# iPERDance/iPERCore

Measured on AMD Instinct MI355X. Metric: synthesized frames/sec at 512x512 (run_imitator), higher is better.
Workload: dtype f32; 1 GPU; run_imitator 512x512 single src/ref pair, 300-frame reference clip frame-sharded over 1 GPU(s), AttLWB-SPADE generator fp32 (BASELINE configs[1] at N = 1, configs[2] at N = 8); poses=imitate, image_size=512, frame_batch=300, frame_batch_requested=384, world_size=1, parallelism=frame-shard x1, batches_in_flight=1, weights=random-init (seeded) of the real architecture, 36,276,992 params

## Files before the change

include/lwg_hip.h:

```cpp
#ifndef LWG_HIP_H
#define LWG_HIP_H

#include <stddef.h>
#include <stdint.h>

#ifdef __cplusplus
extern "C" {
#endif

typedef void* lwg_stream_t;

#define LWG_ABI_VERSION 10
int lwg_abi_version(void);

#define LWG_MAX_TAPS 52
enum { LWG_EPI_NONE = 0, LWG_EPI_RESIDUAL = 1, LWG_EPI_SPADE = 2 };
enum { LWG_ACTIVATION_NONE = 0, LWG_ACTIVATION_RELU = 1, LWG_ACTIVATION_TANH = 2, LWG_ACTIVATION_SIGMOID = 3 };
#define LWG_ACTIVATION_RELU_MASK 5
enum { LWG_DT_F32 = 0, LWG_DT_BF16 = 1,
       LWG_DT_F32_Q4 = 2 };

typedef struct LwgConvArgs {
    const float* x0;
    const float* x1;
    int C0, C1;
    int B, H, W;
    int OH, OW;
    int M;
    int stride;
    int ntaps;
    int cshift;
    const float* w;
    int N;
    const float* bias;
    float* y;
    int YH, YW, YC, ycoff;
    int omul, ooy, oox;
    int epi;
    int act;
    const float* res;
    const float* xn;
    const float* mean;
    const float* rstd;
    int xdt;
    int ydt;
    signed char dy[LWG_MAX_TAPS];
    signed char dx[LWG_MAX_TAPS];
} LwgConvArgs;

int lwg_conv2d_nhwc_f32(const LwgConvArgs* args, lwg_stream_t stream);
size_t lwg_conv2d_ws_floats(const LwgConvArgs* args);
int lwg_conv2d_nhwc_f32_ws(const LwgConvArgs* args, float* ws, lwg_stream_t stream);
int lwg_conv_slice_count(const LwgConvArgs* args);

int lwg_conv2d_nhwc_bf16(const LwgConvArgs* args, lwg_stream_t stream);
int lwg_conv2d_winograd_f32(const LwgConvArgs* args, lwg_stream_t stream);
size_t lwg_conv2d_winograd_ws_floats(const LwgConvArgs* args);
int lwg_conv2d_winograd_f32_ws(const LwgConvArgs* args, float* ws, lwg_stream_t stream);
int lwg_conv2d_winograd_plan(const LwgConvArgs* args, int with_ws, long long* blocks, int* slices, int* nbv, int* workgroups);
int lwg_winograd_panel_f32(const float* wpanel, float* upk, int Cin, int N, const int* tap9, lwg_stream_t stream);
typedef struct LwgWinoDesc {
    const float* wpanel;
    float* upk;
    int Cin, N, first_block;
    int tap9[9];
} LwgWinoDesc;
int lwg_winograd_panels_f32(const LwgWinoDesc* descs_dev, int ndesc, int total_blocks, lwg_stream_t stream);
int lwg_conv2d_winograd4_f32(const LwgConvArgs* args, lwg_stream_t stream);
typedef struct LwgConvLists {
    const int* heavy;
    const int* light;
    const int* counts;
    const float* cal;
} LwgConvLists;
int lwg_conv2d_winograd4_list_f32(const LwgConvArgs* args, const LwgConvLists* lists, lwg_stream_t stream);
int lwg_conv2d_winograd4_list_applies(const LwgConvArgs* args);
int lwg_spade_skip_lists_f32(const float* T, int B, int ns, int h, int w, int d, int* marks, int* heavy, int* light, int* counts, lwg_stream_t stream);
int lwg_conv2d_winograd4_fine_f32(const LwgConvArgs* args, const LwgConvLists* lists, lwg_stream_t stream);
int lwg_spade_skip_fine_lists_f32(const float* T, int B, int ns, int h, int w, int d, int* marks, int* heavy, int* light, int* counts, int* fmarks,
                                  int* fheavy, int* flight, int* fcounts, lwg_stream_t stream);
int lwg_winograd4_panel_f32(const float* wpanel, float* upk, int Cin, int N, const int* tap9, lwg_stream_t stream);
int lwg_conv2d_nhwc_bf16_hr(const LwgConvArgs* args, lwg_stream_t stream);
int lwg_conv2d_winograd_bf16(const LwgConvArgs* args, lwg_stream_t stream);
int lwg_conv2d_nhwc_c8_bf16(const LwgConvArgs* args, lwg_stream_t stream);
int lwg_conv_transpose4_nhwc_bf16(const LwgConvArgs* args, lwg_stream_t stream);
int lwg_conv_transpose4_nhwc_f32(const LwgConvArgs* args, lwg_stream_t stream);
int lwg_conv_transpose4_is_one_grid(const LwgConvArgs* args);
int lwg_conv_transpose4_winograd_f32(const LwgConvArgs* args, lwg_stream_t stream);

int lwg_conv_transpose4_winograd24_f32(const LwgConvArgs* args, lwg_stream_t stream);

int lwg_conv2d_nhwc_f32_split(const LwgConvArgs* args, lwg_stream_t stream);

size_t lwg_conv2d_wgrad_ws_floats(int Ktot, int N, int M);
int lwg_conv2d_wgrad_nhwc_f32(const LwgConvArgs* args, const float* dy, float* dw, float* ws, lwg_stream_t stream);
int lwg_conv2d_wgrad_unpacked_f32(const LwgConvArgs* args, const float* dy, float* ws, float* dw, int D0, int D1, int KH, int KW,
                                  int transposed, const int* kidx, int cin, int nout, float* db, lwg_stream_t stream);
int lwg_colsum_nhwc_f32(const float* x, size_t rows, int C, float* out, float* ws, lwg_stream_t stream);
size_t lwg_conv2d_wgrad_winograd_ws_floats(const LwgConvArgs* args);
int lwg_conv2d_wgrad_winograd_f32(const LwgConvArgs* args, const float* dy, float* ws, float* dw, int cin, int nout, lwg_stream_t stream);

int lwg_act_bwd_f32(const float* dy, const float* y, size_t n, int act, float* out, lwg_stream_t stream);
int lwg_norm_fwd_nhwc_f32(const float* x, const float* mean, const float* rstd, const float* gamma, const float* beta, int gstride,
                          int B, int HW, int C, int act, float* y, lwg_stream_t stream);
int lwg_norm_bwd_nhwc_f32(const float* dy, const float* y, const float* x, const float* mean, const float* rstd,
                          const float* gamma, int gstride, int B, int HW, int C, int act, int nsplit, float* dx, float* dgamma,
                          float* dbeta, float* ws, lwg_stream_t stream);
int lwg_adam_step_f32(float* p, const float* g, float* m, float* v, size_t n, float lr, float beta1, float beta2, float eps, int t,
                      lwg_stream_t stream);
int lwg_adam_step_dev_f32(float* p, const float* g, float* m, float* v, size_t n, float lr, float beta1, float beta2, float eps,
                          int* t_dev, lwg_stream_t stream);
int lwg_pack_panel_f32(const float* w, int D0, int D1, int KH, int KW, int transposed, const int* kidx, int ntaps, int cin,
                       int cin_pad, int nout, int n_pad, float* out, lwg_stream_t stream);
int lwg_unpack_wgrad_f32(const float* dwk, int D0, int D1, int KH, int KW, int transposed, const int* kidx, int ntaps, int cin,
                         int cin_pad, int nout, int n_pad, float* dw, lwg_stream_t stream);
typedef struct LwgPackDesc {
    const float* w;
    float* out;
    int D1, KHW, transposed, ntaps, cin, cin_pad, nout, n_pad, Kp, first_block;
    int kidx[LWG_MAX_TAPS];
} LwgPackDesc;
int lwg_pack_panels_f32(const LwgPackDesc* descs_dev, int ndesc, int total_blocks, lwg_stream_t stream);
int lwg_maxpool2_fwd_nhwc_f32(const float* x, float* y, int B, int H, int W, int C, lwg_stream_t stream);
int lwg_maxpool2_bwd_nhwc_f32(const float* x, const float* dy, float* dx, int B, int H, int W, int C, lwg_stream_t stream);
int lwg_crop_resize_bilinear_f32(const float* x, const long long* box, float* y, float* valid, int N, int C, int H, int W, int OH, int OW,
                                 lwg_stream_t stream);
int lwg_crop_resize_bilinear_bwd_f32(const float* dy, const long long* box, float* dx, int N, int C, int H, int W, int OH, int OW, lwg_stream_t stream);
int lwg_prelu_f32(const float* x, const float* slope, const float* res, size_t rows, int C, float* y, lwg_stream_t stream);
int lwg_prelu_bwd_f32(const float* x, const float* slope, const float* dy, size_t rows, int C, float* dx, lwg_stream_t stream);

int lwg_instnorm_stats_nhwc_f32(const float* x, int B, int HW, int C, float eps, float* mean, float* rstd,
                                float* ws, int nsplit, lwg_stream_t stream);
int lwg_instnorm_stats_nhwc_bf16(const void* x, int B, int HW, int C, float eps, float* mean, float* rstd, float* ws, int nsplit,
                                 lwg_stream_t stream);
int lwg_instnorm_apply_nhwc_f32(const float* x, const float* mean, const float* rstd, const float* res,
                                float* y, int B, int HW, int C, int act, lwg_stream_t stream);

int lwg_flow_resize_f32(const float* T, int n, int S, int h, int w, float* out, lwg_stream_t stream);
int lwg_lwb_attention_f32(const float* q, const float* Ks, const float* Vs, const float* bk, const float* bv,
                          const float* T, float* out, int B, int ns, int h, int w, int C, int S,
                          int src_batched, lwg_stream_t stream);
int lwg_lwb_attention_bf16(const void* q, const void* Ks, const void* Vs, const float* bk, const float* bv, const float* T, void* out,
                           int B, int ns, int h, int w, int C, int S, int src_batched, lwg_stream_t stream);
int lwg_lwb_attention_x_records(int h, int w, int C, int element_size);
int lwg_lwb_attention_x_f32(const float* x, const float* Kq, const float* kappa, const float* Vs, const float* bv, const float* T,
                            float* out, float* stats, int B, int ns, int h, int w, int C, int src_batched, lwg_stream_t stream);
int lwg_lwb_attention_x_bf16(const void* x, const void* Kq, const float* kappa, const void* Vs, const float* bv, const float* T,
                             void* out, float* stats, int B, int ns, int h, int w, int C, int src_batched, lwg_stream_t stream);
size_t lwg_instnorm_finalize_ws_floats(int B, int C, int nrec);
int lwg_instnorm_finalize_f32(float* ws, int B, int C, int nrec, float eps, float* mean, float* rstd, lwg_stream_t stream);
int lwg_lwb_attention_bwd_f32(const float* q, const float* Ks, const float* Vs, const float* bk, const float* bv,
                              const float* T, const float* dout, float* dq, float* dKs, float* dVs, int B, int ns,
                              int h, int w, int C, int S, int src_batched, lwg_stream_t stream);
int lwg_lwb_attention_kv_f32(const float* q, const float* kv, const float* bk, const float* bv, const float* T, float* out,
                             int B, int ns, int h, int w, int C, int S, int src_batched, lwg_stream_t stream);
int lwg_lwb_attention_kv_bwd_f32(const float* q, const float* kv, const float* bk, const float* bv, const float* T,
                                 const float* dout, float* dq, float* dkv, int B, int ns, int h, int w, int C, int S,
                                 int src_batched, lwg_stream_t stream);
int lwg_lwb_fuse_f32(const float* tsf_x, const float* src_x, const float* gate, const float* T, float* out, int B, int ns,
                     int h, int w, int C, int S, int src_batched, float scale_w, float scale_o, lwg_stream_t stream);
int lwg_lwb_fuse_bf16(const void* tsf_x, const void* src_x, const void* gate, const float* T, void* out, int B, int ns, int h, int w,
                      int C, int S, int src_batched, float scale_w, float scale_o, lwg_stream_t stream);
int lwg_lwb_fuse_bwd_f32(const float* src_x, const float* gate, const float* T, const float* dout, float* d_tsf, float* d_src,
                         float* d_gate, int B, int ns, int h, int w, int C, int S, int src_batched, float scale_w, float scale_o,
                         lwg_stream_t stream);

size_t lwg_rasterize_ws_bytes(int B, int nf, int S);
int lwg_project_faces_f32(const float* verts, const float* cam, const int32_t* faces, int B, int nv, int nf,
                          float eye_dist, float* faces_v, float* f2pts, lwg_stream_t stream);
int lwg_rasterize_fim_wim_f32(const float* faces_v, int B, int nf, int S, float near, float far, int32_t* fim,
                              float* wim, void* ws, lwg_stream_t stream);
int lwg_texture_sample_f32(const int32_t* fim, const float* wim, const float* faces_v, const float* textures, int B, int nf,
                           int S, int T, int tex_batched, float eps, const float* bg_color3_host, float* rgb, lwg_stream_t stream);

int lwg_flow_compose_f32(const int32_t* fim, const float* wim, int B, int S, const float* map_fn, int nf,
                         const float* f_uvs2img, const float* uv_img4, int Hu, int Wu, const float* src_f2pts,
                         int ns, float* tsf_inputs, float* Tst, float* cond_nchw, float* Tuv, lwg_stream_t stream);
int lwg_bc_transform_f32(const float* f2pts, const int32_t* fim, const float* wim, int B, int S, int nf, float* T,
                         lwg_stream_t stream);
int lwg_encode_fim_f32(const int32_t* fim, const float* map_fn, int B, int S, int nf, int D, float* out,
                       lwg_stream_t stream);

size_t lwg_smpl_lbs_ws_floats(int B, int nv, int nj);
int lwg_smpl_lbs_f32(const float* pose, int pose_stride, const float* beta, int beta_stride, int nbeta,
                     const float* cam, int cam_stride, const float* v_template, const float* offsets, int off_batched,
                     const float* shapedirs, const float* posedirs, const float* J_regressor, const int32_t* parents,
                     const float* lbs_weights, const int32_t* links, int nlinks, int B, int nv, int nj, float* verts,
                     float* j3d, float* j2d, float* ws, lwg_stream_t stream);

int lwg_head_compose_f32(const float* x, const float* wpk, const float* bg, size_t bg_bstride, int B, int S, int C,
                         float* pred, float* mask, float* img, lwg_stream_t stream);
int lwg_head_compose_q4_f32(const float* x, const float* wpk, const float* bg, size_t bg_bstride, int B, int S, int C,
                            float* pred, float* mask, float* img, lwg_stream_t stream);
int lwg_thin_conv_f32(const float* x, const float* wpk, int B, int S, int C, int ks, float* y, lwg_stream_t stream);
int lwg_head_compose_bf16(const void* x, const void* wb, const float* bg, size_t bg_bstride, int B, int S, int C, float* pred,
                          float* mask, float* img, lwg_stream_t stream);
int lwg_up4_head_compose_bf16(const LwgConvArgs* args, const void* whead, const float* bg, size_t bg_bstride, float* pred, float* mask, float* img,
                              lwg_stream_t stream);
int lwg_frames_to_u8(const float* pred, int B, int S, int bgr, uint8_t* out, lwg_stream_t stream);
int lwg_nchw_to_nhwc_f32(const float* src, float* dst, int B, int C, int Cp, int P, lwg_stream_t stream);
int lwg_nhwc_to_nchw_f32(const float* src, float* dst, int B, int C, int Cs, int P, lwg_stream_t stream);

int lwg_morph_f32(const float* in, float* out, int n, int H, int W, int ks, int mode, float* ws, lwg_stream_t stream);
int lwg_canny_f32(const float* sil, int n, int H, int W, const float* gauss9, const float* sobelx9, float low, float high,
                  float* edges, float* ws, lwg_stream_t stream);
int lwg_boundary_fill_f32(const float* src, const float* confidant, const float* outpad, const float* edges, int n, int H,
                          int W, float* out, int32_t* top3, int32_t* ws, lwg_stream_t stream);
int lwg_grid_sample_nchw_f32(const float* img, size_t img_bstride, const float* grid, int n, int C, int H, int W, int Ho,
                             int Wo, float* out, lwg_stream_t stream);
int lwg_uv_merge_f32(const float* src_warp, const float* vis, int ns, int H, int W, float* out, lwg_stream_t stream);
int lwg_uv_merge_parts_f32(const float* uv_imgs, const float* vis, int n, int H, int W, float* out, lwg_stream_t stream);
int lwg_pack_inputs_f32(const float* a, int Ca, const float* b, int Cb, const float* mask, int n, int H, int W, int Cp,
                        float* out, lwg_stream_t stream);

int lwg_device_cu_count(void);

#ifdef __cplusplus
}
#endif
#endif
```

ipercore_amd/_lib.py:

```python
import ctypes
import os
import re

_HERE = os.path.dirname(os.path.abspath(__file__))
LIB_PATH = os.path.join(_HERE, "liblwg_hip.so")
HEADER_PATH = os.path.join(os.path.dirname(_HERE), "include", "lwg_hip.h")

LWG_MAX_TAPS = 52
EPI_NONE, EPI_RESIDUAL, EPI_SPADE = 0, 1, 2
ACT_NONE, ACT_RELU, ACT_TANH, ACT_SIGMOID, ACT_LRELU = 0, 1, 2, 3, 4
ACT_RELU_MASK = 5
DT_F32, DT_BF16, DT_F32_Q4 = 0, 1, 2

c_f = ctypes.c_void_p
c_i = ctypes.c_int


class LwgConvArgs(ctypes.Structure):
    _fields_ = [
        ("x0", c_f), ("x1", c_f),
        ("C0", c_i), ("C1", c_i),
        ("B", c_i), ("H", c_i), ("W", c_i),
        ("OH", c_i), ("OW", c_i),
        ("M", c_i), ("stride", c_i), ("ntaps", c_i), ("cshift", c_i),
        ("w", c_f), ("N", c_i), ("bias", c_f),
        ("y", c_f), ("YH", c_i), ("YW", c_i), ("YC", c_i), ("ycoff", c_i),
        ("omul", c_i), ("ooy", c_i), ("oox", c_i),
        ("epi", c_i), ("act", c_i),
        ("res", c_f), ("xn", c_f), ("mean", c_f), ("rstd", c_f),
        ("xdt", c_i), ("ydt", c_i),
        ("dy", ctypes.c_byte * LWG_MAX_TAPS), ("dx", ctypes.c_byte * LWG_MAX_TAPS),
    ]


class LwgWinoDesc(ctypes.Structure):
    _fields_ = [("wpanel", ctypes.c_void_p), ("upk", ctypes.c_void_p), ("Cin", c_i), ("N", c_i), ("first_block", c_i), ("tap9", c_i * 9)]


class LwgConvLists(ctypes.Structure):
    _fields_ = [("heavy", c_f), ("light", c_f), ("counts", c_f), ("cal", c_f)]


class LwgPackDesc(ctypes.Structure):
    _fields_ = [("w", c_f), ("out", c_f)] + [(n, c_i) for n in ("D1", "KHW", "transposed", "ntaps", "cin", "cin_pad", "nout", "n_pad", "Kp",
                                                               "first_block")] + [("kidx", c_i * LWG_MAX_TAPS)]


_SIGS = {
    "lwg_abi_version": (c_i, []),
    "lwg_device_cu_count": (c_i, []),
    "lwg_conv2d_nhwc_f32": (c_i, [ctypes.POINTER(LwgConvArgs), c_f]),
    "lwg_conv2d_ws_floats": (ctypes.c_size_t, [ctypes.POINTER(LwgConvArgs)]),
    "lwg_conv2d_nhwc_f32_ws": (c_i, [ctypes.POINTER(LwgConvArgs), c_f, c_f]),
    "lwg_conv2d_nhwc_bf16": (c_i, [ctypes.POINTER(LwgConvArgs), c_f]),
    "lwg_conv2d_winograd_f32": (c_i, [ctypes.POINTER(LwgConvArgs), c_f]),
    "lwg_conv2d_winograd_ws_floats": (ctypes.c_size_t, [ctypes.POINTER(LwgConvArgs)]),
    "lwg_conv2d_winograd_f32_ws": (c_i, [ctypes.POINTER(LwgConvArgs), c_f, c_f]),
    "lwg_conv2d_winograd_plan": (c_i, [ctypes.POINTER(LwgConvArgs), c_i, ctypes.POINTER(ctypes.c_longlong), ctypes.POINTER(c_i), ctypes.POINTER(c_i),
                                       ctypes.POINTER(c_i)]),
    "lwg_winograd_panel_f32": (c_i, [c_f, c_f, c_i, c_i, ctypes.POINTER(c_i), c_f]),
    "lwg_winograd_panels_f32": (c_i, [c_f, c_i, c_i, c_f]),
    "lwg_conv2d_winograd4_f32": (c_i, [ctypes.POINTER(LwgConvArgs), c_f]),
    "lwg_conv2d_winograd4_list_f32": (c_i, [ctypes.POINTER(LwgConvArgs), ctypes.POINTER(LwgConvLists), c_f]),
    "lwg_conv2d_winograd4_list_applies": (c_i, [ctypes.POINTER(LwgConvArgs)]),
    "lwg_spade_skip_lists_f32": (c_i, [c_f, c_i, c_i, c_i, c_i, c_i, c_f, c_f, c_f, c_f, c_f]),
    "lwg_conv2d_winograd4_fine_f32": (c_i, [ctypes.POINTER(LwgConvArgs), ctypes.POINTER(LwgConvLists), c_f]),
    "lwg_spade_skip_fine_lists_f32": (c_i, [c_f, c_i, c_i, c_i, c_i, c_i, c_f, c_f, c_f, c_f, c_f, c_f, c_f, c_f, c_f]),
    "lwg_winograd4_panel_f32": (c_i, [c_f, c_f, c_i, c_i, ctypes.POINTER(c_i), c_f]),
    "lwg_conv2d_nhwc_bf16_hr": (c_i, [ctypes.POINTER(LwgConvArgs), c_f]),
    "lwg_conv2d_winograd_bf16": (c_i, [ctypes.POINTER(LwgConvArgs), c_f]),
    "lwg_conv2d_nhwc_c8_bf16": (c_i, [ctypes.POINTER(LwgConvArgs), c_f]),
    "lwg_conv_transpose4_nhwc_bf16": (c_i, [ctypes.POINTER(LwgConvArgs), c_f]),
    "lwg_conv_transpose4_nhwc_f32": (c_i, [ctypes.POINTER(LwgConvArgs), c_f]),
    "lwg_conv_transpose4_winograd_f32": (c_i, [ctypes.POINTER(LwgConvArgs), c_f]),
    "lwg_conv_transpose4_winograd24_f32": (c_i, [ctypes.POINTER(LwgConvArgs), c_f]),
    "lwg_conv_transpose4_is_one_grid": (c_i, [ctypes.POINTER(LwgConvArgs)]),
    "lwg_conv_slice_count": (c_i, [ctypes.POINTER(LwgConvArgs)]),
    "lwg_conv2d_nhwc_f32_split": (c_i, [ctypes.POINTER(LwgConvArgs), c_f]),
    "lwg_conv2d_wgrad_ws_floats": (ctypes.c_size_t, [c_i, c_i, c_i]),
    "lwg_conv2d_wgrad_nhwc_f32": (c_i, [ctypes.POINTER(LwgConvArgs), c_f, c_f, c_f, c_f]),
    "lwg_conv2d_wgrad_unpacked_f32": (c_i, [ctypes.POINTER(LwgConvArgs), c_f, c_f, c_f] + [c_i] * 5 + [ctypes.POINTER(ctypes.c_int), c_i, c_i, c_f, c_f]),
    "lwg_colsum_nhwc_f32": (c_i, [c_f, ctypes.c_size_t, c_i, c_f, c_f, c_f]),
    "lwg_conv2d_wgrad_winograd_ws_floats": (ctypes.c_size_t, [ctypes.POINTER(LwgConvArgs)]),
    "lwg_conv2d_wgrad_winograd_f32": (c_i, [ctypes.POINTER(LwgConvArgs), c_f, c_f, c_f, c_i, c_i, c_f]),
    "lwg_act_bwd_f32": (c_i, [c_f, c_f, ctypes.c_size_t, c_i, c_f, c_f]),
    "lwg_norm_fwd_nhwc_f32": (c_i, [c_f, c_f, c_f, c_f, c_f, c_i, c_i, c_i, c_i, c_i, c_f, c_f]),
    "lwg_norm_bwd_nhwc_f32": (c_i, [c_f, c_f, c_f, c_f, c_f, c_f, c_i, c_i, c_i, c_i, c_i, c_i, c_f, c_f, c_f, c_f, c_f]),
    "lwg_adam_step_f32": (c_i, [c_f, c_f, c_f, c_f, ctypes.c_size_t, ctypes.c_float, ctypes.c_float, ctypes.c_float, ctypes.c_float, c_i, c_f]),
    "lwg_adam_step_dev_f32": (c_i, [c_f, c_f, c_f, c_f, ctypes.c_size_t, ctypes.c_float, ctypes.c_float, ctypes.c_float, ctypes.c_float, c_f, c_f]),
    "lwg_pack_panel_f32": (c_i, [c_f] + [c_i] * 5 + [ctypes.POINTER(ctypes.c_int)] + [c_i] * 5 + [c_f, c_f]),
    "lwg_pack_panels_f32": (c_i, [c_f, c_i, c_i, c_f]),
    "lwg_unpack_wgrad_f32": (c_i, [c_f] + [c_i] * 5 + [ctypes.POINTER(ctypes.c_int)] + [c_i] * 5 + [c_f, c_f]),
    "lwg_maxpool2_fwd_nhwc_f32": (c_i, [c_f, c_f, c_i, c_i, c_i, c_i, c_f]),
    "lwg_maxpool2_bwd_nhwc_f32": (c_i, [c_f, c_f, c_f, c_i, c_i, c_i, c_i, c_f]),
    "lwg_crop_resize_bilinear_f32": (c_i, [c_f, c_f, c_f, c_f, c_i, c_i, c_i, c_i, c_i, c_i, c_f]),
    "lwg_crop_resize_bilinear_bwd_f32": (c_i, [c_f, c_f, c_f, c_i, c_i, c_i, c_i, c_i, c_i, c_f]),
    "lwg_prelu_f32": (c_i, [c_f, c_f, c_f, ctypes.c_size_t, c_i, c_f, c_f]),
    "lwg_prelu_bwd_f32": (c_i, [c_f, c_f, c_f, ctypes.c_size_t, c_i, c_f, c_f]),
    "lwg_instnorm_stats_nhwc_f32": (c_i, [c_f, c_i, c_i, c_i, ctypes.c_float, c_f, c_f, c_f, c_i, c_f]),
    "lwg_instnorm_apply_nhwc_f32": (c_i, [c_f, c_f, c_f, c_f, c_f, c_i, c_i, c_i, c_i, c_f]),
    "lwg_lwb_attention_f32": (c_i, [c_f, c_f, c_f, c_f, c_f, c_f, c_f, c_i, c_i, c_i, c_i, c_i, c_i, c_i, c_f]),
    "lwg_lwb_attention_bf16": (c_i, [c_f, c_f, c_f, c_f, c_f, c_f, c_f, c_i, c_i, c_i, c_i, c_i, c_i, c_i, c_f]),
    "lwg_instnorm_stats_nhwc_bf16": (c_i, [c_f, c_i, c_i, c_i, ctypes.c_float, c_f, c_f, c_f, c_i, c_f]),
    "lwg_head_compose_bf16": (c_i, [c_f, c_f, c_f, ctypes.c_size_t, c_i, c_i, c_i, c_f, c_f, c_f, c_f]),
    "lwg_up4_head_compose_bf16": (c_i, [ctypes.POINTER(LwgConvArgs), c_f, c_f, ctypes.c_size_t, c_f, c_f, c_f, c_f]),
    "lwg_flow_resize_f32": (c_i, [c_f, c_i, c_i, c_i, c_i, c_f, c_f]),
    "lwg_lwb_fuse_f32": (c_i, [c_f] * 5 + [c_i] * 7 + [ctypes.c_float, ctypes.c_float, c_f]),
    "lwg_lwb_fuse_bf16": (c_i, [c_f] * 5 + [c_i] * 7 + [ctypes.c_float, ctypes.c_float, c_f]),
    "lwg_lwb_fuse_bwd_f32": (c_i, [c_f] * 7 + [c_i] * 7 + [ctypes.c_float, ctypes.c_float, c_f]),
    "lwg_lwb_attention_x_f32": (c_i, [c_f] * 8 + [c_i] * 6 + [c_f]),
    "lwg_lwb_attention_x_bf16": (c_i, [c_f] * 8 + [c_i] * 6 + [c_f]),
    "lwg_lwb_attention_x_records": (c_i, [c_i, c_i, c_i, c_i]),
    "lwg_instnorm_finalize_ws_floats": (ctypes.c_size_t, [c_i, c_i, c_i]),
    "lwg_instnorm_finalize_f32": (c_i, [c_f, c_i, c_i, c_i, ctypes.c_float, c_f, c_f, c_f]),
    "lwg_lwb_attention_bwd_f32": (c_i, [c_f] * 10 + [c_i] * 7 + [c_f]),
    "lwg_lwb_attention_kv_f32": (c_i, [c_f] * 6 + [c_i] * 7 + [c_f]),
    "lwg_lwb_attention_kv_bwd_f32": (c_i, [c_f] * 8 + [c_i] * 7 + [c_f]),
    "lwg_rasterize_ws_bytes": (ctypes.c_size_t, [c_i, c_i, c_i]),
    "lwg_project_faces_f32": (c_i, [c_f, c_f, c_f, c_i, c_i, c_i, ctypes.c_float, c_f, c_f, c_f]),
    "lwg_rasterize_fim_wim_f32": (c_i, [c_f, c_i, c_i, c_i, ctypes.c_float, ctypes.c_float, c_f, c_f, c_f, c_f]),
    "lwg_texture_sample_f32": (c_i, [c_f, c_f, c_f, c_f, c_i, c_i, c_i, c_i, c_i, ctypes.c_float, ctypes.POINTER(ctypes.c_float), c_f, c_f]),
    "lwg_flow_compose_f32": (c_i, [c_f, c_f, c_i, c_i, c_f, c_i, c_f, c_f, c_i, c_i, c_f, c_i, c_f, c_f, c_f, c_f, c_f]),
    "lwg_bc_transform_f32": (c_i, [c_f, c_f, c_f, c_i, c_i, c_i, c_f, c_f]),
    "lwg_encode_fim_f32": (c_i, [c_f, c_f, c_i, c_i, c_i, c_i, c_f, c_f]),
    "lwg_smpl_lbs_ws_floats": (ctypes.c_size_t, [c_i, c_i, c_i]),
    "lwg_smpl_lbs_f32": (c_i, [c_f, c_i, c_f, c_i, c_i, c_f, c_i, c_f, c_f, c_i, c_f, c_f, c_f, c_f, c_f, c_f, c_i, c_i, c_i,
                               c_i, c_f, c_f, c_f, c_f, c_f]),
    "lwg_head_compose_f32": (c_i, [c_f, c_f, c_f, ctypes.c_size_t, c_i, c_i, c_i, c_f, c_f, c_f, c_f]),
    "lwg_head_compose_q4_f32": (c_i, [c_f, c_f, c_f, ctypes.c_size_t, c_i, c_i, c_i, c_f, c_f, c_f, c_f]),
    "lwg_thin_conv_f32": (c_i, [c_f, c_f, c_i, c_i, c_i, c_i, c_f, c_f]),
    "lwg_nchw_to_nhwc_f32": (c_i, [c_f, c_f, c_i, c_i, c_i, c_i, c_f]),
    "lwg_nhwc_to_nchw_f32": (c_i, [c_f, c_f, c_i, c_i, c_i, c_i, c_f]),
    "lwg_frames_to_u8": (c_i, [c_f, c_i, c_i, c_i, c_f, c_f]),
    "lwg_morph_f32": (c_i, [c_f, c_f, c_i, c_i, c_i, c_i, c_i, c_f, c_f]),
    "lwg_canny_f32": (c_i, [c_f, c_i, c_i, c_i, ctypes.POINTER(ctypes.c_float), ctypes.POINTER(ctypes.c_float),
                            ctypes.c_float, ctypes.c_float, c_f, c_f, c_f]),
    "lwg_boundary_fill_f32": (c_i, [c_f, c_f, c_f, c_f, c_i, c_i, c_i, c_f, c_f, c_f, c_f]),
    "lwg_grid_sample_nchw_f32": (c_i, [c_f, ctypes.c_size_t, c_f, c_i, c_i, c_i, c_i, c_i, c_i, c_f, c_f]),
    "lwg_uv_merge_f32": (c_i, [c_f, c_f, c_i, c_i, c_i, c_f, c_f]),
    "lwg_uv_merge_parts_f32": (c_i, [c_f, c_f, c_i, c_i, c_i, c_f, c_f]),
    "lwg_pack_inputs_f32": (c_i, [c_f, c_i, c_f, c_i, c_f, c_i, c_i, c_i, c_i, c_f, c_f]),
}

_lib = None


def header_symbols():
    with open(HEADER_PATH) as fp:
        src = re.sub(r"/\*.*?\*/", "", fp.read(), flags=re.S)
    return sorted(set(re.findall(r"\b(lwg_[a-z0-9_]+)\s*\(", src)))


def lib():
    global _lib
    if _lib is None:
        if not os.path.exists(LIB_PATH):
            raise RuntimeError(
                f"{LIB_PATH} not found: the HIP kernels are not built (run `python -c 'import __graft_entry__ as g; "
                "g.build()'` or `make -C ipercore_amd/csrc`).  There is no CPU fallback.")
        import torch
        handle = ctypes.CDLL(LIB_PATH)
        for name, (res, args) in _SIGS.items():
            fn = getattr(handle, name)
            fn.restype = res
            fn.argtypes = args
        if handle.lwg_abi_version() != 10:
            raise RuntimeError("liblwg_hip.so ABI version mismatch")
        _lib = handle
    return _lib


def check(err, what):
    if err != 0:
        raise RuntimeError(f"{what} failed with hipError_t {err}")
```

ipercore_amd/csrc/lwb_attn_x.hip:

```cpp
#include "lwg_common.h"
#include "lwg_conv_args.h"
#include "lwg_lwb_taps.h"

typedef unsigned int uintx4 __attribute__((ext_vector_type(4)));

template <typename ST> struct AttnXTraits;
template <> struct AttnXTraits<float> {
    static constexpr int CPL = 4;
    __device__ static __forceinline__ void unpack(const uintx4 v, float (&f)[4]) {
#pragma unroll
        for (int k = 0; k < 4; ++k) {
            const unsigned u = v[k];
            f[k] = __builtin_bit_cast(float, u);
        }
    }
    __device__ static __forceinline__ uintx4 pack(const float (&f)[4]) {
        uintx4 v;
#pragma unroll
        for (int k = 0; k < 4; ++k) v[k] = __builtin_bit_cast(unsigned, f[k]);
        return v;
    }
};
template <> struct AttnXTraits<__bf16> {
    static constexpr int CPL = 8;
    __device__ static __forceinline__ void unpack(const uintx4 v, float (&f)[8]) {
#pragma unroll
        for (int k = 0; k < 4; ++k) {
            f[2 * k] = __builtin_bit_cast(float, v[k] << 16);
            f[2 * k + 1] = __builtin_bit_cast(float, v[k] & 0xffff0000u);
        }
    }
    __device__ static __forceinline__ uintx4 pack(const float (&f)[8]) {
        typedef __bf16 bf16x2 __attribute__((ext_vector_type(2)));
        uintx4 v;
#pragma unroll
        for (int k = 0; k < 4; ++k) {
            bf16x2 p;
            p[0] = (__bf16)f[2 * k];
            p[1] = (__bf16)f[2 * k + 1];
            v[k] = __builtin_bit_cast(unsigned, p);
        }
        return v;
    }
};

template <typename ST, int LPP, bool STATS, int NSU, int PW, int OCC, bool PIPE = false>
__global__ __launch_bounds__(256 * PW, PW == 1 ? OCC : 1) void lwg_lwb_attnx_kernel(const ST* __restrict__ x, const ST* __restrict__ Kq,
                                                                 const float* __restrict__ kappa, const ST* __restrict__ Vs,
                                                                 const float* __restrict__ bv, const float* __restrict__ T,
                                                                 ST* __restrict__ out, float* __restrict__ stats, int B, int ns, int h, int w,
                                                                 int src_batched) {
    using TR = AttnXTraits<ST>;
    constexpr int CPL = TR::CPL;
    constexpr int C = CPL * LPP;
    constexpr int PPW = 64 / LPP;
    constexpr int PPP = 4 * PPW;
    constexpr int NPASS = 64 / PPP;
    constexpr int NIT = NPASS / PW;
    static_assert(NPASS % PW == 0, "PW must divide the tile's pass count");
    constexpr int NT = NSU > 0 ? NSU : 1;
    constexpr unsigned ROWB = (unsigned)C * sizeof(ST);
    const int lane = threadIdx.x & 63, wid = threadIdx.x >> 6;
    const int wq = wid & 3, pl = wid >> 2;
    const int cl = lane % LPP, pg = lane / LPP;
    const int tiles_x = (w + 7) >> 3;
    int tile, b;
    if (LWG_ATTNX_INTERLEAVE) {
        const int xcd = blockIdx.x & 7;
        const long idx = blockIdx.x >> 3;
        const long grp = idx / B;
        tile = (int)(grp * 8 + xcd);
        b = (int)(idx - grp * B);
        if (tile >= tiles_x * ((h + 7) >> 3)) return;
    } else {
        const long L = lwg_xcd_remap(blockIdx.x, gridDim.x);
        tile = (int)(L / B);
        b = (int)(L - (long)tile * B);
    }
    const int ty = tile / tiles_x, tx = tile - ty * tiles_x;
    const int hw = h * w;
    const unsigned nsrc = (unsigned)(src_batched ? B * ns : ns);
    __amdgpu_buffer_rsrc_t rK = __builtin_amdgcn_make_buffer_rsrc(const_cast<ST*>(Kq), 0, (int)(nsrc * (unsigned)hw * ROWB), 0x00020000);
    __amdgpu_buffer_rsrc_t rV = __builtin_amdgcn_make_buffer_rsrc(const_cast<ST*>(Vs), 0, (int)(nsrc * (unsigned)hw * ROWB), 0x00020000);
    __amdgpu_buffer_rsrc_t rA = __builtin_amdgcn_make_buffer_rsrc(const_cast<float*>(kappa), 0, (int)(nsrc * (unsigned)hw * 4u), 0x00020000);
    const float inv_sqrt_c = 1.0f / sqrtf((float)C);
    constexpr bool BV_REG = CPL == 4 || LWG_ATTNX_BVREG16;
    float bvr[CPL];
    if (BV_REG) {
#pragma unroll
        for (int k = 0; k < CPL; ++k) bvr[k] = bv[CPL * cl + k];
    }
    const float2* Tb = reinterpret_cast<const float2*>(T) + (size_t)b * ns * hw;

    auto pixel_of = [&](int pass, int& yc, int& xc) -> bool {
        const int p = pass * PPP + wq * PPW + pg;
        const int y = ty * 8 + (p >> 3), xx = tx * 8 + (p & 7);
        const bool live = y < h && xx < w;
        yc = live ? y : ty * 8;
        xc = live ? xx : tx * 8;
        return live;
    };
    extern __shared__ __attribute__((aligned(16))) char smem_ax[];
    char* xs = smem_ax;
    float2* Tl = reinterpret_cast<float2*>(smem_ax + NPASS * 4096);
    {
        __amdgpu_buffer_rsrc_t rX = __builtin_amdgcn_make_buffer_rsrc(const_cast<ST*>(x) + (size_t)b * hw * C, 0, (int)((unsigned)hw * ROWB), 0x00020000);
#pragma unroll
        for (int it = 0; it < NIT; ++it) {
            const int pass = it * PW + pl;
            int yc, xc;
            pixel_of(pass, yc, xc);
            const unsigned voff = (unsigned)(yc * w + xc) * ROWB + (unsigned)(CPL * cl) * (unsigned)sizeof(ST);
            __builtin_amdgcn_raw_ptr_buffer_load_lds(rX, (__attribute__((address_space(3))) void*)(xs + (pass * 4 + wq) * 1024), 16, (int)voff, 0, 0, 0);
        }
        for (int i = threadIdx.x; i < ns * 64; i += 256 * PW) {
            const int s = i >> 6, p = i & 63;
            const int y = ty * 8 + (p >> 3), xx = tx * 8 + (p & 7);
            const bool in = y < h && xx < w;
            Tl[i] = Tb[(size_t)s * hw + (size_t)(in ? y : ty * 8) * w + (in ? xx : tx * 8)];
        }
        asm volatile("s_waitcnt vmcnt(0)" ::: "memory");
        __syncthreads();
    }
    auto x_row = [&](int pass) -> uintx4 { return *reinterpret_cast<const uintx4*>(xs + ((pass * 4 + wq) * 64 + lane) * 16); };

    float shift[CPL], s1[CPL], s2[CPL];
    if (STATS) {
        TR::unpack(*reinterpret_cast<const uintx4*>(xs + cl * 16), shift);
#pragma unroll
        for (int k = 0; k < CPL; ++k) s1[k] = s2[k] = 0.f;
    }
    int nlive = 0;
    auto stats_add = [&](const float (&xv)[CPL]) {
        ++nlive;
        if (PW == 1) {
#pragma unroll
            for (int k = 0; k < CPL; ++k) {
                const float d = xv[k] - shift[k];
                s1[k] += d;
                s2[k] = __builtin_fmaf(d, d, s2[k]);
            }
        }
    };
    auto taps_of = [&](const float2 t, float (&wt)[4], int& tx0, int& ty0) { lwb_taps_of(t, w, h, wt, tx0, ty0); };
    auto fold = [&](const float (&ka)[CPL], const float (&va)[CPL], float kap, const float (&xv)[CPL], float& mrun, float& lrun, float (&o)[CPL]) {
        float dot = 0.f;
#pragma unroll
        for (int k = 0; k < CPL; ++k) dot = __builtin_fmaf(ka[k], xv[k], dot);
#pragma unroll
        for (int off = LPP >> 1; off > 0; off >>= 1) dot += __shfl_xor(dot, off, 64);
        const float logit = (dot + kap) * inv_sqrt_c;
        const float mnew = fmaxf(mrun, logit);
        const float corr = expf(mrun - mnew);
        const float pr = expf(logit - mnew);
        lrun = __builtin_fmaf(lrun, corr, pr);
#pragma unroll
        for (int k = 0; k < CPL; ++k) o[k] = __builtin_fmaf(o[k], corr, pr * va[k]);
        mrun = mnew;
    };
    auto finish = [&](long gp, float lrun, const float (&o)[CPL]) {
        const float invl = 1.f / lrun;
        float r[CPL];
        if (!BV_REG) {
#pragma unroll
            for (int k = 0; k < CPL; k += 4) {
                const floatx4 b4 = *reinterpret_cast<const floatx4*>(bv + CPL * cl + k);
#pragma unroll
                for (int j = 0; j < 4; ++j) bvr[k + j] = b4[j];
            }
        }
#pragma unroll
        for (int k = 0; k < CPL; ++k) r[k] = __builtin_fmaf(o[k], invl, bvr[k]);
        *reinterpret_cast<uintx4*>(out + gp * C + CPL * cl) = TR::pack(r);
    };

    if constexpr (PIPE) {
        static_assert(NSU == 2 && PW == 1 && (NIT % 2) == 0, "the pipelined form is the ns = 2 frame-batch form");
        bool mine = false;
#pragma unroll 1
        for (int it = 0; it < NIT; ++it) {
            int yc, xc;
            const bool live = pixel_of(it, yc, xc);
            const int ptile = it * PPP + wq * PPW + pg;
#pragma unroll
            for (int s = 0; s < 2; ++s) {
                const float2 t = Tl[s * 64 + ptile];
                float wt[4];
                int tx0, ty0;
                taps_of(t, wt, tx0, ty0);
                mine |= live && lwb_tap_in_image(tx0, ty0, w, h);
            }
        }
        if (__syncthreads_or(mine ? 1 : 0) == 0) {
#pragma unroll 1
            for (int it = 0; it < NIT; ++it) {
                int yc, xc;
                const bool live = pixel_of(it, yc, xc);
                float xv[CPL];
                TR::unpack(x_row(it), xv);
                if (live) {
                    if (STATS) stats_add(xv);
                    float o[CPL];
#pragma unroll
                    for (int k = 0; k < CPL; ++k) o[k] = 0.f;
                    finish(((long)b * h + yc) * w + xc, 2.f, o);
                }
            }
        } else {
            struct Taps { uintx4 kr[2][4], vr[2][4]; float ar[2][4], wt[2][4]; };
            auto issue = [&](int pass, Taps& g) {
                int yc, xc;
                const bool live = pixel_of(pass, yc, xc);
                const int ptile = pass * PPP + wq * PPW + pg;
#pragma unroll
                for (int s = 0; s < 2; ++s) {
                    int tx0, ty0;
                    taps_of(Tl[s * 64 + ptile], g.wt[s], tx0, ty0);
                    const unsigned pbase = (unsigned)(src_batched ? b * ns + s : s) * (unsigned)hw;
#pragma unroll
                    for (int tp = 0; tp < 4; ++tp) {
                        const int tyy = ty0 + (tp >> 1), txx = tx0 + (tp & 1);
                        const bool ok = live && tyy >= 0 && tyy < h && txx >= 0 && txx < w;
                        const unsigned pix = pbase + (unsigned)(tyy * w + txx);
                        const unsigned voff = ok ? pix * ROWB + (unsigned)(CPL * cl) * (unsigned)sizeof(ST) : 0xC0000000u;
                        g.kr[s][tp] = __builtin_bit_cast(uintx4, __builtin_amdgcn_raw_buffer_load_b128(rK, (int)voff, 0, 0));
                        g.vr[s][tp] = __builtin_bit_cast(uintx4, __builtin_amdgcn_raw_buffer_load_b128(rV, (int)voff, 0, 0));
                        g.ar[s][tp] = __builtin_bit_cast(float, __builtin_amdgcn_raw_buffer_load_b32(rA, ok ? (int)(pix * 4u) : (int)0xC0000000u, 0, 0));
                    }
                }
            };
            auto consume = [&](int pass, const Taps& g) {
                int yc, xc;
                const bool live = pixel_of(pass, yc, xc);
                float xv[CPL];
                TR::unpack(x_row(pass), xv);
                if (STATS && live) stats_add(xv);
                float mrun = -INFINITY, lrun = 0.f;
                float o[CPL];
#pragma unroll
                for (int k = 0; k < CPL; ++k) o[k] = 0.f;
#pragma unroll
                for (int s = 0; s < 2; ++s) {
                    float ka[CPL], va[CPL], kap = 0.f;
#pragma unroll
                    for (int k = 0; k < CPL; ++k) ka[k] = va[k] = 0.f;
#pragma unroll
                    for (int tp = 0; tp < 4; ++tp) {
                        float k8[CPL], v8[CPL];
                        TR::unpack(g.kr[s][tp], k8);
                        TR::unpack(g.vr[s][tp], v8);
#pragma unroll
                        for (int k = 0; k < CPL; ++k) {
                            ka[k] = __builtin_fmaf(k8[k], g.wt[s][tp], ka[k]);
                            va[k] = __builtin_fmaf(v8[k], g.wt[s][tp], va[k]);
                        }
                        kap = __builtin_fmaf(g.ar[s][tp], g.wt[s][tp], kap);
                    }
                    fold(ka, va, kap, xv, mrun, lrun, o);
                }
                if (live) finish(((long)b * h + yc) * w + xc, lrun, o);
            };
            Taps g0, g1;
            issue(0, g0);
#pragma unroll 1
            for (int it = 0; it < NIT; it += 2) {
                issue(it + 1, g1);
                consume(it, g0);
                issue(it + 2 < NIT ? it + 2 : it + 1, g0);
                consume(it + 1, g1);
            }
        }
    } else {
#pragma unroll 1
    for (int it = 0; it < NIT; ++it) {
        const int pass = it * PW + pl;
        int yc, xc;
        const bool live = pixel_of(pass, yc, xc);
        const long gp = ((long)b * h + yc) * w + xc;
        const int ptile = pass * PPP + wq * PPW + pg;
        float xv[CPL];
        TR::unpack(x_row(pass), xv);
        if (STATS && live) stats_add(xv);
        float mrun = -INFINITY, lrun = 0.f;
        float o[CPL];
#pragma unroll
        for (int k = 0; k < CPL; ++k) o[k] = 0.f;

        auto source = [&](int s, const float2 t) {
            float wt[4];
            int tx0, ty0;
            taps_of(t, wt, tx0, ty0);
            const bool any_tap = live && lwb_tap_in_image(tx0, ty0, w, h);
            float ka[CPL], va[CPL], kap = 0.f;
#pragma unroll
            for (int k = 0; k < CPL; ++k) ka[k] = va[k] = 0.f;
            if (__builtin_amdgcn_ballot_w64(any_tap) != 0ull) {
                const unsigned sidx = (unsigned)(src_batched ? b * ns + s : s);
                const unsigned pbase = sidx * (unsigned)hw;
                uintx4 kr[4], vr[4];
                float ar[4];
#pragma unroll
                for (int tp = 0; tp < 4; ++tp) {
                    const int tyy = ty0 + (tp >> 1), txx = tx0 + (tp & 1);
                    const bool ok = live && tyy >= 0 && tyy < h && txx >= 0 && txx < w;
                    const unsigned pix = pbase + (unsigned)(tyy * w + txx);
                    const unsigned voff = ok ? pix * ROWB + (unsigned)(CPL * cl) * (unsigned)sizeof(ST) : 0xC0000000u;
                    kr[tp] = __builtin_bit_cast(uintx4, __builtin_amdgcn_raw_buffer_load_b128(rK, (int)voff, 0, 0));
                    vr[tp] = __builtin_bit_cast(uintx4, __builtin_amdgcn_raw_buffer_load_b128(rV, (int)voff, 0, 0));
                    ar[tp] = __builtin_bit_cast(float, __builtin_amdgcn_raw_buffer_load_b32(rA, ok ? (int)(pix * 4u) : (int)0xC0000000u, 0, 0));
                }
#pragma unroll
                for (int tp = 0; tp < 4; ++tp) {
                    float k8[CPL], v8[CPL];
                    TR::unpack(kr[tp], k8);
                    TR::unpack(vr[tp], v8);
#pragma unroll
                    for (int k = 0; k < CPL; ++k) {
                        ka[k] = __builtin_fmaf(k8[k], wt[tp], ka[k]);
                        va[k] = __builtin_fmaf(v8[k], wt[tp], va[k]);
                    }
                    kap = __builtin_fmaf(ar[tp], wt[tp], kap);
                }
            }
            fold(ka, va, kap, xv, mrun, lrun, o);
        };
        if (NSU > 0) {
#pragma unroll
            for (int s = 0; s < NT; ++s) source(s, Tl[s * 64 + ptile]);
        } else {
#pragma unroll 1
            for (int s = 0; s < ns; ++s) source(s, Tl[s * 64 + ptile]);
        }
        if (live) finish(gp, lrun, o);
    }
    }

    if (STATS) {
        if (PW > 1) {
            __shared__ float acc[4][64][2 * CPL];
            if (pl == 0) {
#pragma unroll
                for (int k = 0; k < 2 * CPL; ++k) acc[wq][lane][k] = 0.f;
            }
            __syncthreads();
#pragma unroll 1
            for (int p = 0; p < NPASS; ++p) {
                if (pl == p % PW) {
                    int yc, xc;
                    if (pixel_of(p, yc, xc)) {
                        float xv[CPL];
                        TR::unpack(x_row(p), xv);
#pragma unroll
                        for (int k = 0; k < CPL; ++k) {
                            const float d = xv[k] - shift[k];
                            acc[wq][lane][k] += d;
                            acc[wq][lane][CPL + k] = __builtin_fmaf(d, d, acc[wq][lane][CPL + k]);
                        }
                    }
                }
                __syncthreads();
            }
            if (pl == 0) {
#pragma unroll
                for (int k = 0; k < CPL; ++k) {
                    s1[k] = acc[wq][lane][k];
                    s2[k] = acc[wq][lane][CPL + k];
                }
            }
        }
        __syncthreads();
        float (*sh)[2][C] = reinterpret_cast<float (*)[2][C]>(smem_ax);
        float* shn = reinterpret_cast<float*>(smem_ax + 4 * 2 * C * sizeof(float));
        float fn = (float)nlive;
#pragma unroll
        for (int off = LPP; off < 64; off <<= 1) {
#pragma unroll
            for (int k = 0; k < CPL; ++k) {
                s1[k] += __shfl_xor(s1[k], off, 64);
                s2[k] += __shfl_xor(s2[k], off, 64);
            }
            fn += __shfl_xor(fn, off, 64);
        }
        if (pg == 0) {
            if (pl == 0) {
#pragma unroll
                for (int k = 0; k < CPL; ++k) {
                    sh[wq][0][CPL * cl + k] = s1[k];
                    sh[wq][1][CPL * cl + k] = s2[k];
                }
            }
            if (cl == 0) shn[wid] = fn;
        }
        __syncthreads();
        if (wid == 0 && pg == 0) {
            float tn = 0.f;
#pragma unroll
            for (int k = 0; k < 4 * PW; ++k) tn += shn[k];
            const int nrec = tiles_x * ((h + 7) >> 3);
#pragma unroll
            for (int k = 0; k < CPL; ++k) {
                const int c = CPL * cl + k;
                const float t1 = ((sh[0][0][c] + sh[1][0][c]) + sh[2][0][c]) + sh[3][0][c];
                const float t2 = ((sh[0][1][c] + sh[1][1][c]) + sh[2][1][c]) + sh[3][1][c];
                const float mean = shift[k] + t1 / tn;
                const float m2 = t2 - t1 * t1 / tn;
                float* rec = stats + (((size_t)b * nrec + tile) * C + c) * 3;
                rec[0] = tn;
                rec[1] = mean;
                rec[2] = m2 > 0.f ? m2 : 0.f;
            }
        }
    }
}

extern "C" int lwg_lwb_attention_x_records(int h, int w, int C, int esz) {
    if (h <= 0 || w <= 0 || C <= 0 || (esz != 2 && esz != 4)) return 0;
    const int lpp = C / (16 / esz);
    if (lpp < 8 || lpp > 64 || (lpp & (lpp - 1)) != 0) return 0;
    return ((w + 7) >> 3) * ((h + 7) >> 3);
}

template <typename ST>
static int lwg_attnx_launch(const ST* x, const ST* Kq, const float* kappa, const ST* Vs, const float* bv, const float* T, ST* out, float* stats,
                            int B, int ns, int h, int w, int C, int src_batched, hipStream_t stream) {
    if (!x || !Kq || !kappa || !Vs || !bv || !T || !out || B <= 0 || ns <= 0 || ns > 64 || h <= 0 || w <= 0) return (int)hipErrorInvalidValue;
    const unsigned long long nsrc = (unsigned long long)(src_batched ? B * ns : ns);
    if (nsrc * (unsigned long long)h * w * (unsigned long long)C * sizeof(ST) >= 0xC0000000ull) return (int)hipErrorInvalidValue;
    const long tiles = (long)((w + 7) >> 3) * ((h + 7) >> 3);
    constexpr int CPL = AttnXTraits<ST>::CPL;
    const int npass = (C / CPL) / 4;
    const dim3 grid((unsigned)((LWG_ATTNX_INTERLEAVE ? (tiles + 7) / 8 * 8 : tiles) * B));
    const bool wide = LWG_ATTNX_WIDE && tiles * B < 512 && npass >= 4;
#define LWG_ATTNX_GO(LPP, ST_, NSU, PW)                                                                                              \
    {                                                                                                                                \
             \
        constexpr bool pipe = LWG_ATTNX_PIPE && CPL == 4 && (LPP) == 64 && (NSU) == 2 && (PW) == 1;                                  \
        auto kern = lwg_lwb_attnx_kernel<ST, LPP, ST_, NSU, PW, (pipe ? 2 : CPL == 4 ? LWG_ATTNX_OCC : LWG_ATTNX_OCC16), pipe>;        \
        const size_t lds = (size_t)((LPP) / 4) * 4096 + (size_t)ns * 512;                         \
        static unsigned long long lds_ok = 0;                                                                                        \
        if (lds > 65536) {                                                                                                           \
            const hipError_t e = lwg_allow_dynamic_lds(reinterpret_cast<const void*>(kern), lds, lds_ok);                            \
            if (e != hipSuccess) return (int)e;                                                                                      \
        }                                                                                                                            \
        hipLaunchKernelGGL(kern, grid, dim3(256 * PW), lds, stream, x, Kq, kappa, Vs, bv, T, out, stats, B, ns, h, w, src_batched);   \
    }
#define LWG_ATTNX_PW(LPP, ST_, NSU)                                                                                                  \
    {                                                                                                                                \
        if constexpr ((LPP) / 4 >= 4) {                                                                                              \
            if (wide) LWG_ATTNX_GO(LPP, ST_, NSU, 4) else LWG_ATTNX_GO(LPP, ST_, NSU, 1)                                             \
        } else {                                                                                                                     \
            LWG_ATTNX_GO(LPP, ST_, NSU, 1)                                                                                           \
        }                                                                                                                            \
    }
#define LWG_ATTNX_LAUNCH(LPP)                                                                                                        \
    if (stats) { if (LWG_ATTNX_NSU2 && ns == 2) LWG_ATTNX_PW(LPP, true, 2) else LWG_ATTNX_PW(LPP, true, 0) }                         \
    else { if (LWG_ATTNX_NSU2 && ns == 2) LWG_ATTNX_PW(LPP, false, 2) else LWG_ATTNX_PW(LPP, false, 0) }
    switch (C / CPL) {
        case 8: LWG_ATTNX_LAUNCH(8) break;
        case 16: LWG_ATTNX_LAUNCH(16) break;
        case 32: LWG_ATTNX_LAUNCH(32) break;
        case 64: if constexpr (CPL == 4) { LWG_ATTNX_LAUNCH(64) break; }
                 return (int)hipErrorInvalidValue;
        default: return (int)hipErrorInvalidValue;
    }
#undef LWG_ATTNX_LAUNCH
#undef LWG_ATTNX_PW
#undef LWG_ATTNX_GO
    return (int)hipGetLastError();
}

extern "C" int lwg_lwb_attention_x_f32(const float* x, const float* Kq, const float* kappa, const float* Vs, const float* bv, const float* T,
                                       float* out, float* stats, int B, int ns, int h, int w, int C, int src_batched, lwg_stream_t stream_) {
    if (C != 32 && C != 64 && C != 128 && C != 256) return (int)hipErrorInvalidValue;
    return lwg_attnx_launch<float>(x, Kq, kappa, Vs, bv, T, out, stats, B, ns, h, w, C, src_batched, reinterpret_cast<hipStream_t>(stream_));
}

extern "C" int lwg_lwb_attention_x_bf16(const void* x, const void* Kq, const float* kappa, const void* Vs, const float* bv, const float* T,
                                        void* out, float* stats, int B, int ns, int h, int w, int C, int src_batched, lwg_stream_t stream_) {
    if (C != 64 && C != 128 && C != 256) return (int)hipErrorInvalidValue;
    return lwg_attnx_launch<__bf16>(static_cast<const __bf16*>(x), static_cast<const __bf16*>(Kq), kappa, static_cast<const __bf16*>(Vs), bv, T,
                                    static_cast<__bf16*>(out), stats, B, ns, h, w, C, src_batched, reinterpret_cast<hipStream_t>(stream_));
}

__global__ __launch_bounds__(1024) void lwg_in_stats_merge_seg(const float* __restrict__ ws, int C, int nrec, int nseg, float eps,
                                                              float* __restrict__ part, float* __restrict__ mean, float* __restrict__ rstd) {
    const int lane = threadIdx.x & 63, wid = threadIdx.x >> 6;
    const int c = blockIdx.x * 64 + lane, b = blockIdx.y, seg = blockIdx.z;
    const bool cok = c < C;
    const float* base = ws + ((size_t)b * nrec * C + (cok ? c : 0)) * 3;
    const float r = base[1];
    const int per = (nrec + nseg - 1) / nseg;
    const int r0 = seg * per, r1 = min(nrec, r0 + per);
    float sa = 0.f, ss = 0.f, sq = 0.f;
    if (cok) {
        for (int i = r0 + wid; i < r1; i += 16) {
            const float* o = base + (size_t)i * C * 3;
            const float n = o[0], d = o[1] - r;
            sa += n;
            ss = __builtin_fmaf(n, d, ss);
            sq += __builtin_fmaf(n * d, d, o[2]);
        }
    }
    __shared__ float sh[16][3][64];
    sh[wid][0][lane] = sa;
    sh[wid][1][lane] = ss;
    sh[wid][2][lane] = sq;
    __syncthreads();
    if (wid == 0 && cok) {
        float ta = 0.f, ts = 0.f, tq = 0.f;
#pragma unroll
        for (int k = 0; k < 16; ++k) { ta += sh[k][0][lane]; ts += sh[k][1][lane]; tq += sh[k][2][lane]; }
        if (nseg == 1) {
            const float m2 = tq - ts * ts / ta;
            mean[(size_t)b * C + c] = r + ts / ta;
            rstd[(size_t)b * C + c] = 1.0f / sqrtf((m2 > 0.f ? m2 : 0.f) / ta + eps);
        } else {
            float* o = part + (((size_t)b * nseg + seg) * C + c) * 3;
            o[0] = ta; o[1] = ts; o[2] = tq;
        }
    }
}

__global__ __launch_bounds__(256) void lwg_in_stats_merge_fin(const float* __restrict__ ws, const float* __restrict__ part, int BC, int C, int nrec,
                                                             int nseg, float eps, float* __restrict__ mean, float* __restrict__ rstd) {
    const int i = blockIdx.x * 256 + threadIdx.x;
    if (i >= BC) return;
    const int b = i / C, c = i - b * C;
    const float r = ws[((size_t)b * nrec * C + c) * 3 + 1];
    float ta = 0.f, ts = 0.f, tq = 0.f;
    for (int s = 0; s < nseg; ++s) {
        const float* o = part + (((size_t)b * nseg + s) * C + c) * 3;
        ta += o[0]; ts += o[1]; tq += o[2];
    }
    const float m2 = tq - ts * ts / ta;
    mean[i] = r + ts / ta;
    rstd[i] = 1.0f / sqrtf((m2 > 0.f ? m2 : 0.f) / ta + eps);
}

extern "C" size_t lwg_instnorm_finalize_ws_floats(int B, int C, int nrec) {
    if (B <= 0 || C <= 0 || nrec <= 0) return 0;
    const size_t nseg = nrec > 512 ? (size_t)(nrec + 255) / 256 : 0;
    return (size_t)B * nrec * C * 3 + (size_t)B * nseg * C * 3;
}
extern "C" int lwg_instnorm_finalize_f32(float* ws, int B, int C, int nrec, float eps, float* mean, float* rstd, lwg_stream_t stream_) {
    if (!ws || !mean || !rstd || B <= 0 || C <= 0 || nrec <= 0 || B > 65535) return (int)hipErrorInvalidValue;
    hipStream_t stream = reinterpret_cast<hipStream_t>(stream_);
    const int nseg = nrec > 512 ? (nrec + 255) / 256 : 1;
    if (nseg > 65535) return (int)hipErrorInvalidValue;
    float* part = ws + (size_t)B * nrec * C * 3;
    hipLaunchKernelGGL(lwg_in_stats_merge_seg, dim3((C + 63) / 64, B, nseg), dim3(1024), 0, stream, ws, C, nrec, nseg, eps, part, mean, rstd);
    if (nseg > 1)
        hipLaunchKernelGGL(lwg_in_stats_merge_fin, dim3((B * C + 255) / 256), dim3(256), 0, stream, ws, part, B * C, C, nrec, nseg, eps, mean, rstd);
    return (int)hipGetLastError();
}
```

ipercore_amd/csrc/lwg_conv_wino.h:

```cpp
#pragma once
#include <stddef.h>
#include "lwg_conv_args.h"

#ifdef __HIPCC__
#define CW_FN __host__ __device__ __forceinline__
#else
#define CW_FN static inline
#endif
#ifdef __HIP_DEVICE_COMPILE__
#define CW_UNIFORM(v) __builtin_amdgcn_readfirstlane(v)
#else
#define CW_UNIFORM(v) (v)
#endif
#define CW_OOB 0xC0000000u
#define CW_KS 8
#define CW_NB 64
struct CwGrid { int bx, by, tiles, total; };
CW_FN CwGrid cw_grid(int B, int H, int W, int N, int ex, int ey, int nbv) {
    const int bx = (W + ex - 1) / ex, by = (H + ey - 1) / ey, tiles = bx * by * B;
    return CwGrid{bx, by, tiles, tiles * (N / nbv)};
}
CW_FN long long cw_total_blocks(int B, int H, int W, int N, int ex, int ey, int nbv) {
    return (long long)((W + ex - 1) / ex) * ((H + ey - 1) / ey) * B * (N / nbv);
}

enum { CW_COLMAJOR = 0, CW_CHUNK = 1, CW_XCD = 2 };
struct CwOrder { int kind, nwg, wg, ncb, tiles, total, xg, xr; };

CW_FN int cw4_order_kind(int xcd_sw, int chunk_sw, bool sm, unsigned nwg, int ncb, int Cin, int N, int tiles, int total) {
    const bool xcd = xcd_sw && !sm && (nwg & 7u) == 0 && (ncb == 4 || ncb == 8 || (ncb == 2 && (Cin >= 192 || xcd_sw == 2))) && (int)nwg < total && tiles >= (int)nwg / ncb;
    return xcd ? CW_XCD : chunk_sw == 2 || (chunk_sw == 1 && 144u * (unsigned)Cin * (unsigned)N <= (5u << 20)) ? CW_CHUNK : CW_COLMAJOR;
}
CW_FN CwOrder cw_order(int kind, unsigned nwg, unsigned wg, int ncb, const CwGrid& g) {
    return CwOrder{kind, (int)nwg, (int)wg, ncb, g.tiles, g.total, (int)nwg / ncb, (int)(((wg & 7u) / (unsigned)ncb) * (nwg >> 3) + (wg >> 3))};
}
CW_FN bool cw_has_block(const CwOrder& o, int id) {
    return o.kind == CW_XCD ? (id / o.nwg) * o.xg + o.xr < o.tiles : id < o.total;
}
CW_FN void cw_block(const CwOrder& o, int id, int& cb, int& t) {
    if (o.kind == CW_XCD) {
        cb = (int)((unsigned)o.wg & 7u) & (o.ncb - 1);
        t = CW_UNIFORM((id / o.nwg) * o.xg + o.xr);
    } else if (o.kind == CW_CHUNK) {
        const int G = o.nwg, per = G * o.ncb;
        const int ch = CW_UNIFORM(id / per);
        const int r = id - ch * per, base = ch * G;
        const int nt = o.tiles - base < G ? o.tiles - base : G;
        cb = CW_UNIFORM(r / nt);
        t = CW_UNIFORM(base + r - cb * nt);
    } else {
        cb = CW_UNIFORM(id / o.tiles);
        t = CW_UNIFORM(id - cb * o.tiles);
    }
}
CW_FN int cw_image(const CwGrid& g, int t) { return t / (g.bx * g.by); }
CW_FN void cw_corner(const CwGrid& g, int t_in_image, int ex, int ey, int& x0, int& y0) { x0 = (t_in_image % g.bx) * ex, y0 = (t_in_image / g.bx) * ey; }
CW_FN int cw_n0(int cb, int nbv) { return cb * nbv; }
CW_FN int cw4_n0_spade_small(int cb) { return (cb >> 1) * 64 + (cb & 1) * 16; }
CW_FN int cw_halo_pixel(int i, int hw, int nel, int lgp, int x0, int y0, int H, int W) {
    const int pix = i >> lgp, hy = pix / hw, hx = pix - hy * hw;
    const int gy = y0 - 1 + hy, gx = x0 - 1 + hx;
    return i < nel && gy >= 0 && gy < H && gx >= 0 && gx < W ? gy * W + gx : -1;
}
CW_FN unsigned cw_halo_pixel_voff(int lin, int i, int lgp, int C, int ebytes) {
    return lin >= 0 ? (unsigned)(lin * C + (16 / ebytes) * (i & ((1 << lgp) - 1))) * (unsigned)ebytes : CW_OOB;
}
CW_FN unsigned cw_halo_voff(int i, int hw, int nel, int lgp, int x0, int y0, int H, int W, int C, int ebytes) {
    return cw_halo_pixel_voff(cw_halo_pixel(i, hw, nel, lgp, x0, y0, H, W), i, lgp, C, ebytes);
}
CW_FN bool cw_stage_second(int c, int C0, bool two) { return two && c >= C0; }
CW_FN unsigned cw_stage_soff(int c, int C0, bool two, int ebytes) { return (unsigned)(cw_stage_second(c, C0, two) ? c - C0 : c) * (unsigned)ebytes; }
CW_FN unsigned cw4_out_voff(int ox, int oy, int H, int W, int YC, int chan) {
    return ox < W && oy < H ? (unsigned)((oy * W + ox) * YC + chan) * 4u : CW_OOB;
}
CW_FN unsigned cw4_out_group(unsigned vo, int h, bool grouped) { return vo + (grouped ? 128u * (unsigned)h : 0u); }

struct CwWindow { int x0, y0, x1, y1; };
CW_FN CwWindow cw_block_window(int x0, int y0, int ex, int ey, int d, int H, int W) {
    return CwWindow{x0 - d > 0 ? x0 - d : 0, y0 - d > 0 ? y0 - d : 0, x0 + ex + d < W ? x0 + ex + d : W, y0 + ey + d < H ? y0 + ey + d : H};
}
CW_FN void cw_list_entry(int e, int ncb, int& slot, int& cb) { slot = e / ncb, cb = e - slot * ncb; }
CW_FN int cw_list_first_light(int wg, int nwg, int nhe) { return wg >= nhe ? wg : wg + (nhe - wg + nwg - 1) / nwg * nwg; }
CW_FN void cw4_light_elem(int tid, int it, int nth, int nq, int& px, int& py, int& q4) {
    const int e = it * nth + tid, p = e / nq;
    q4 = e - p * nq, px = p & 31, py = p >> 5;
}

#define CW4F_SX 16
#define CW4F_SY 8
#define CW4F_NSX (32 / CW4F_SX)
#define CW4F_NS (CW4F_NSX * (16 / CW4F_SY))
#define CW4F_HW (CW4F_SX + 2)
#define CW4F_HH (CW4F_SY + 2)
#define CW4F_NEL (CW4F_HW * CW4F_HH * 2)
#define CW4F_ROUNDS ((CW4F_NEL + 63) / 64)
CW_FN int cw4f_slot_of_patch(int pty, int ptx) { return (pty / (CW4F_SY / 4)) * CW4F_NSX + ptx / (CW4F_SX / 4); }
CW_FN void cw4f_patch_in_slot(int pty, int ptx, int& ly, int& lx) { ly = pty % (CW4F_SY / 4), lx = ptx % (CW4F_SX / 4); }
CW_FN void cw4f_corner(const CwGrid& g, int u, int& b, int& x0, int& y0) {
    const int t = u / CW4F_NS, s = u - t * CW4F_NS;
    b = cw_image(g, t);
    cw_corner(g, t - b * g.bx * g.by, 32, 16, x0, y0);
    x0 += (s % CW4F_NSX) * CW4F_SX, y0 += (s / CW4F_NSX) * CW4F_SY;
}
CW_FN bool cw4f_in_image(int x0, int y0, int H, int W) { return x0 < W && y0 < H; }
CW_FN int cw4f_in_image_total(int B, int H, int W) { return B * ((W + CW4F_SX - 1) / CW4F_SX) * ((H + CW4F_SY - 1) / CW4F_SY); }
CW_FN int cw4f_groups(int nh) { return (nh + CW4F_NS - 1) / CW4F_NS; }
CW_FN int cw4f_slot_index(int grp, int k, int nh) { return grp * CW4F_NS + k < nh ? grp * CW4F_NS + k : -1; }
CW_FN unsigned cw4f_reached(int x, int y, int x0, int y0, int d) {
    unsigned m = 0;
    for (int s = 0; s < CW4F_NS; ++s) {
        const int sx = x0 + (s % CW4F_NSX) * CW4F_SX, sy = y0 + (s / CW4F_NSX) * CW4F_SY;
        m |= (x >= sx - d && x < sx + CW4F_SX + d && y >= sy - d && y < sy + CW4F_SY + d ? 1u : 0u) << s;
    }
    return m;
}
CW_FN void cw4f_halo_elem(int i, int& slot, int& j) {
    const int wave = (i >> 6) & 7, k = i >> 9, per = CW4F_ROUNDS / 3, wr = 3 * wave + k;
    slot = wave / per, j = (wr - slot * CW4F_ROUNDS) * 64 + (i & 63);
}
CW_FN void cw4f_halo_place(int j, int& hy, int& hx, int& hq) {
    const int pix = j >> 1;
    hq = j & 1, hy = pix / CW4F_HW, hx = pix - hy * CW4F_HW;
}
CW_FN unsigned cw4f_halo_voff(bool present, int j, int x0, int y0, int H, int W, int C) {
    int hy, hx, hq;
    cw4f_halo_place(j, hy, hx, hq);
    const int gy = y0 - 1 + hy, gx = x0 - 1 + hx;
    return present && j < CW4F_NEL && gy >= 0 && gy < H && gx >= 0 && gx < W ? (unsigned)((gy * W + gx) * C + 4 * hq) * 4u : CW_OOB;
}
CW_FN void cw4f_light_pixel(int& px, int& py) {
    const int p = py * 32 + px;
    py = p / CW4F_SX, px = p - py * CW4F_SX;
}

#define CW_NO_OUT_BUFFER (-1ll)
CW_FN bool cw_contract_ok(const LwgConvArgs& a, unsigned long long pair_bytes, long long out_slack) {
    if (!a.x0 || !a.w || !a.y || a.M <= 0 || a.ntaps != 9 || a.stride != 1 || a.omul != 1 || a.C0 <= 0 || (a.C0 % CW_KS) != 0 || a.C1 < 0 ||
        (a.C1 % CW_KS) != 0 || ((a.C0 + a.C1) % (2 * CW_KS)) != 0 || (a.C1 > 0 && !a.x1) || a.N <= 0 || (a.N % CW_NB) != 0 || a.OH != a.H ||
        a.OW != a.W || a.YH != a.H || a.YW != a.W || a.xdt != LWG_DT_F32 || a.ydt != LWG_DT_F32 || (long long)a.M != (long long)a.B * a.H * a.W ||
        a.ycoff < 0 || (a.ycoff % 4) != 0 || (a.YC % 4) != 0 || (a.act == LWG_ACTIVATION_RELU_MASK && a.epi != LWG_EPI_RESIDUAL))
        return false;
    if (a.epi == LWG_EPI_SPADE) {
        if (!a.xn || !a.mean || !a.rstd || !a.bias || a.YC * 2 != a.N || a.ycoff != 0) return false;
    } else {
        if (a.ycoff + a.N > a.YC) return false;
        if (a.epi != LWG_EPI_NONE && (a.epi != LWG_EPI_RESIDUAL || !a.res)) return false;
    }
    const unsigned long long cmax = (unsigned long long)(a.C0 > a.C1 ? a.C0 : a.C1);
    if ((unsigned long long)a.H * a.W * cmax * 4ull >= (unsigned long long)CW_OOB || pair_bytes * (a.C0 + a.C1) * a.N >= 0xffffffffull) return false;
    if (out_slack >= 0 && (unsigned long long)a.H * a.W * a.YC * 4ull + (unsigned long long)out_slack >= (unsigned long long)CW_OOB) return false;
    return true;
}
CW_FN bool cw_contract_calib_ok(const LwgConvArgs& a) {
    return (unsigned long long)a.H * a.W * (unsigned long long)(a.epi == LWG_EPI_SPADE ? a.N : a.YC) * 4ull + 256ull < (unsigned long long)CW_OOB;
}
CW_FN bool cwb_contract_ok(const LwgConvArgs& a) {
    if (!a.x0 || !a.w || !a.y || a.B <= 0 || a.H <= 0 || a.W <= 0 || a.C0 <= 0 || a.C1 < 0 || a.N <= 0 || a.xdt != LWG_DT_BF16 || a.ydt != LWG_DT_BF16 ||
        a.ntaps != 9 || a.stride != 1 || a.omul != 1 || a.ooy != 0 || a.oox != 0 || a.OH != a.H || a.OW != a.W || a.YH != a.H || a.YW != a.W ||
        (long long)a.M != (long long)a.B * a.H * a.W)
        return false;
    for (int t = 0; t < 9; ++t)
        if (a.dy[t] != t / 3 - 1 || a.dx[t] != t % 3 - 1) return false;
    const int Cin = a.C0 + a.C1;
    if (a.N % 64 != 0 || Cin % 64 != 0 || (a.YC & 7) != 0 || (a.ycoff & 7) != 0 || a.ycoff < 0 || (a.C1 != 0 && (a.C0 % 64 != 0 || !a.x1))) return false;
    if (a.act != LWG_ACTIVATION_NONE && a.act != LWG_ACTIVATION_RELU && a.act != LWG_ACTIVATION_TANH && a.act != LWG_ACTIVATION_SIGMOID) return false;
    if ((unsigned long long)a.H * a.W * (unsigned long long)(a.C0 > a.C1 ? a.C0 : a.C1) * 2ull >= (unsigned long long)CW_OOB ||
        32ull * (unsigned long long)Cin * (unsigned long long)a.N >= (unsigned long long)CW_OOB || cw_total_blocks(a.B, a.H, a.W, a.N, 16, 16, 64) >= 0x7fffffffll)
        return false;
    if (a.epi == LWG_EPI_SPADE) return a.xn && a.mean && a.rstd && a.bias && a.YC * 2 == a.N && a.ycoff == 0;
    return a.ycoff + a.N <= a.YC && (a.epi == LWG_EPI_NONE || (a.epi == LWG_EPI_RESIDUAL && a.res));
}

struct LwgWinoTaps { int t[9]; };
CW_FN bool cw_panel_args_ok(const float* wpanel, const float* upk, int Cin, int N, const int* tap9, LwgWinoTaps& taps) {
    if (!wpanel || !upk || !tap9 || Cin <= 0 || (Cin % 32) != 0 || N <= 0) return false;
    for (int i = 0; i < 9; ++i) {
        if (tap9[i] < 0 || tap9[i] > 8) return false;
        taps.t[i] = tap9[i];
    }
    return true;
}

#ifdef __HIPCC__
#include "lwg_common.h"

template <int V> struct IntC { static constexpr int value = V; };
template <int POLICY = 0>
__device__ __forceinline__ floatx4 cw_buf_load(__amdgpu_buffer_rsrc_t r, unsigned voff, unsigned soff) {
    return __builtin_bit_cast(floatx4, __builtin_amdgcn_raw_buffer_load_b128(r, (int)voff, (int)soff, POLICY));
}
__device__ __forceinline__ __amdgpu_buffer_rsrc_t cw_image_rsrc(const void* x, int b, int H, int W, int C, unsigned ebytes) {
    const unsigned img = (unsigned)(H * W);
    return __builtin_amdgcn_make_buffer_rsrc(const_cast<char*>(static_cast<const char*>(x)) + (size_t)b * img * C * ebytes, 0, (int)(img * (unsigned)C * ebytes), 0x00020000);
}

template <int NQ, bool TWO>
struct CwBlock {
    int b, x0, y0, n0;
    __amdgpu_buffer_rsrc_t rx0, rx1;
    unsigned voff0[NQ], voff1[NQ];

    __device__ __forceinline__ void locate(const LwgConvArgs& a, const CwGrid& g, int t, int ex, int ey, int n) {
        b = __builtin_amdgcn_readfirstlane(cw_image(g, t));
        cw_corner(g, t - b * g.bx * g.by, ex, ey, x0, y0);
        n0 = n;
        rx0 = cw_image_rsrc(a.x0, b, a.H, a.W, a.C0, 4u);
        if constexpr (TWO) rx1 = cw_image_rsrc(a.x1, b, a.H, a.W, a.C1, 4u);
    }
    __device__ __forceinline__ void halo(const LwgConvArgs& a, int tid, int nth, int hw, int nel) {
#pragma unroll
        for (int k = 0; k < NQ; ++k) {
            voff0[k] = cw_halo_voff(tid + nth * k, hw, nel, 1, x0, y0, a.H, a.W, a.C0, 4);
            if constexpr (TWO) voff1[k] = cw_halo_voff(tid + nth * k, hw, nel, 1, x0, y0, a.H, a.W, a.C1, 4);
        }
    }
    template <int POLICY = 0>
    __device__ __forceinline__ floatx4 rld1(const LwgConvArgs& a, int c, int k) const {
        if constexpr (!TWO) {
            return cw_buf_load<POLICY>(rx0, voff0[k], cw_stage_soff(c, a.C0, false, 4));
        } else {
            const bool second = cw_stage_second(c, a.C0, true);
            const __amdgpu_buffer_rsrc_t r = second ? rx1 : rx0;
            const unsigned v = second ? voff1[k] : voff0[k];
            return cw_buf_load<POLICY>(r, v, cw_stage_soff(c, a.C0, true, 4));
        }
    }
};
__device__ __forceinline__ void cw_rst1(float* dst, int plane, floatx4 v) {
#pragma unroll
    for (int k = 0; k < 4; ++k) dst[k * plane] = v[k];
}

template <void (*KERNEL)(const LwgConvArgs)>
static inline int cw_launch(dim3 grid, unsigned threads, size_t lds, hipStream_t stream, const LwgConvArgs& a) {
    static unsigned long long done = 0ull;
    if (hipError_t e = lwg_allow_dynamic_lds(reinterpret_cast<const void*>(KERNEL), lds, done); e != hipSuccess) return (int)e;
    hipLaunchKernelGGL(KERNEL, grid, dim3(threads), lds, stream, a);
    return (int)hipGetLastError();
}
template <void (*KERNEL)(const LwgConvArgs, const LwgConvLists)>
static inline int cw_launch_lists(dim3 grid, unsigned threads, size_t lds, hipStream_t stream, const LwgConvArgs& a, const LwgConvLists& l) {
    static unsigned long long done = 0ull;
    if (hipError_t e = lwg_allow_dynamic_lds(reinterpret_cast<const void*>(KERNEL), lds, done); e != hipSuccess) return (int)e;
    hipLaunchKernelGGL(KERNEL, grid, dim3(threads), lds, stream, a, l);
    return (int)hipGetLastError();
}
static inline dim3 cw_persistent_grid(long long total, int cus) { return dim3((unsigned)(LWG_WINO_PERSIST && total > cus ? cus : total)); }
#endif
```

ipercore_amd/csrc/spade_skip.hip:

```cpp
#include <hip/hip_runtime.h>
#include "lwg_common.h"
#include "lwg_conv_wino.h"
#include "lwg_lwb_taps.h"

#define SK_EX 32
#define SK_EY 16

__global__ __launch_bounds__(256) void lwg_spade_skip_mark_kernel(const float2* __restrict__ T, int B, int ns, int h, int w, int d, int* __restrict__ marks) {
    const CwGrid g = cw_grid(B, h, w, CW_NB, SK_EX, SK_EY, CW_NB);
    const int t = blockIdx.x, b = cw_image(g, t);
    int x0, y0;
    cw_corner(g, t - b * g.bx * g.by, SK_EX, SK_EY, x0, y0);
    const CwWindow win = cw_block_window(x0, y0, SK_EX, SK_EY, d, h, w);
    const int ww = win.x1 - win.x0, n = ww * (win.y1 - win.y0);
    bool mine = false;
    for (int s = 0; s < ns; ++s) {
        const float2* Ts = T + ((size_t)b * ns + s) * h * w;
        for (int i = threadIdx.x; i < n; i += 256) {
            const int yy = i / ww, y = win.y0 + yy, x = win.x0 + (i - yy * ww);
            float wt[4];
            int tx0, ty0;
            lwb_taps_of(Ts[(size_t)y * w + x], w, h, wt, tx0, ty0);
            mine |= lwb_tap_in_image(tx0, ty0, w, h);
        }
    }
    const int any = __syncthreads_or(mine ? 1 : 0);
    if (threadIdx.x == 0) marks[t] = any ? 1 : 0;
}

__global__ __launch_bounds__(1024) void lwg_spade_skip_scan_kernel(const int* __restrict__ marks, int n, int* __restrict__ heavy, int* __restrict__ light,
                                                                   int* __restrict__ counts) {
    __shared__ int part[1024];
    const int tid = threadIdx.x, per = (n + 1023) / 1024;
    const int i0 = tid * per < n ? tid * per : n, i1 = i0 + per < n ? i0 + per : n;
    int c = 0;
    for (int i = i0; i < i1; ++i) c += marks[i] != 0;
    part[tid] = c;
    __syncthreads();
    for (int off = 1; off < 1024; off <<= 1) {
        const int v = tid >= off ? part[tid - off] : 0;
        __syncthreads();
        part[tid] += v;
        __syncthreads();
    }
    int hv = part[tid] - c;
    for (int i = i0; i < i1; ++i) {
        if (marks[i] != 0) heavy[hv++] = i;
        else light[i - hv] = i;
    }
    if (tid == 1023) {
        counts[0] = part[1023];
        counts[1] = n - part[1023];
    }
}

__global__ __launch_bounds__(256) void lwg_spade_skip_mark_fine_kernel(const float2* __restrict__ T, int B, int ns, int h, int w, int d, int* __restrict__ marks,
                                                                       int* __restrict__ fmarks) {
    const CwGrid g = cw_grid(B, h, w, CW_NB, SK_EX, SK_EY, CW_NB);
    const int t = blockIdx.x, b = cw_image(g, t);
    int x0, y0;
    cw_corner(g, t - b * g.bx * g.by, SK_EX, SK_EY, x0, y0);
    const CwWindow win = cw_block_window(x0, y0, SK_EX, SK_EY, d, h, w);
    const int ww = win.x1 - win.x0, n = ww * (win.y1 - win.y0);
    unsigned mine = 0;
    for (int s = 0; s < ns; ++s) {
        const float2* Ts = T + ((size_t)b * ns + s) * h * w;
        for (int i = threadIdx.x; i < n; i += 256) {
            const int yy = i / ww, y = win.y0 + yy, x = win.x0 + (i - yy * ww);
            float wt[4];
            int tx0, ty0;
            lwb_taps_of(Ts[(size_t)y * w + x], w, h, wt, tx0, ty0);
            if (lwb_tap_in_image(tx0, ty0, w, h)) mine |= (1u << CW4F_NS) | cw4f_reached(x, y, x0, y0, d);
        }
    }
    unsigned all = 0;
    for (int s = 0; s <= CW4F_NS; ++s) all |= __syncthreads_or((int)((mine >> s) & 1u)) ? 1u << s : 0u;
    if (threadIdx.x < CW4F_NS) {
        const int s = threadIdx.x;
        const bool in = cw4f_in_image(x0 + (s % CW4F_NSX) * CW4F_SX, y0 + (s / CW4F_NSX) * CW4F_SY, h, w);
        fmarks[CW4F_NS * t + s] = in ? (int)((all >> s) & 1u) : 2;
    } else if (threadIdx.x == CW4F_NS) {
        marks[t] = (int)((all >> CW4F_NS) & 1u);
    }
}

struct SkScanJob { const int* marks; int n; int* heavy; int* light; int* counts; };
template <typename F>
__device__ __forceinline__ void sk_for_marks(const int* __restrict__ marks, int i0, int i1, bool vec, F f) {
    int i = i0;
    if (vec)
        for (; i + 4 <= i1; i += 4) {
            const int4 m = *reinterpret_cast<const int4*>(marks + i);
            f(i, m.x), f(i + 1, m.y), f(i + 2, m.z), f(i + 3, m.w);
        }
    for (; i < i1; ++i) f(i, marks[i]);
}
__global__ __launch_bounds__(1024) void lwg_spade_skip_scan2_kernel(SkScanJob j0, SkScanJob j1) {
    __shared__ int ph[1024], pl[1024];
    const SkScanJob j = blockIdx.x == 0 ? j0 : j1;
    const int tid = threadIdx.x, n = j.n, per = ((n + 1023) / 1024 + 3) & ~3;
    const int i0 = tid * per < n ? tid * per : n, i1 = i0 + per < n ? i0 + per : n;
    const bool vec = (reinterpret_cast<size_t>(j.marks) & 15) == 0;
    int ch = 0, cl = 0;
    sk_for_marks(j.marks, i0, i1, vec, [&](int, int m) { ch += m == 1, cl += m == 0; });
    ph[tid] = ch, pl[tid] = cl;
    __syncthreads();
    for (int off = 1; off < 1024; off <<= 1) {
        const int vh = tid >= off ? ph[tid - off] : 0, vl = tid >= off ? pl[tid - off] : 0;
        __syncthreads();
        ph[tid] += vh, pl[tid] += vl;
        __syncthreads();
    }
    int hv = ph[tid] - ch, lt = pl[tid] - cl;
    sk_for_marks(j.marks, i0, i1, vec, [&](int i, int m) {
        if (m == 1) j.heavy[hv++] = i;
        else if (m == 0) j.light[lt++] = i;
    });
    if (tid == 1023) {
        j.counts[0] = ph[1023];
        j.counts[1] = pl[1023];
    }
}

extern "C" int lwg_spade_skip_fine_lists_f32(const float* T, int B, int ns, int h, int w, int d, int* marks, int* heavy, int* light, int* counts,
                                             int* fmarks, int* fheavy, int* flight, int* fcounts, lwg_stream_t stream_) {
    if (!T || !marks || !heavy || !light || !counts || !fmarks || !fheavy || !flight || !fcounts || B <= 0 || ns <= 0 || h <= 0 || w <= 0 || d < 0 || d > 64)
        return (int)hipErrorInvalidValue;
    const long long tiles = cw_total_blocks(B, h, w, CW_NB, SK_EX, SK_EY, CW_NB);
    if (tiles * CW4F_NS >= (1ll << 30) || (long long)h * w >= (1ll << 30)) return (int)hipErrorInvalidValue;
    hipStream_t stream = reinterpret_cast<hipStream_t>(stream_);
    hipLaunchKernelGGL(lwg_spade_skip_mark_fine_kernel, dim3((unsigned)tiles), dim3(256), 0, stream, reinterpret_cast<const float2*>(T), B, ns, h, w, d, marks, fmarks);
    hipLaunchKernelGGL(lwg_spade_skip_scan2_kernel, dim3(2), dim3(1024), 0, stream, SkScanJob{marks, (int)tiles, heavy, light, counts},
                       SkScanJob{fmarks, (int)tiles * CW4F_NS, fheavy, flight, fcounts});
    return (int)hipGetLastError();
}

extern "C" int lwg_spade_skip_lists_f32(const float* T, int B, int ns, int h, int w, int d, int* marks, int* heavy, int* light, int* counts,
                                        lwg_stream_t stream_) {
    if (!T || !marks || !heavy || !light || !counts || B <= 0 || ns <= 0 || h <= 0 || w <= 0 || d < 0 || d > 64) return (int)hipErrorInvalidValue;
    const long long tiles = cw_total_blocks(B, h, w, CW_NB, SK_EX, SK_EY, CW_NB);
    if (tiles >= (1ll << 30) || (long long)h * w >= (1ll << 30)) return (int)hipErrorInvalidValue;
    hipStream_t stream = reinterpret_cast<hipStream_t>(stream_);
    hipLaunchKernelGGL(lwg_spade_skip_mark_kernel, dim3((unsigned)tiles), dim3(256), 0, stream, reinterpret_cast<const float2*>(T), B, ns, h, w, d, marks);
    hipLaunchKernelGGL(lwg_spade_skip_scan_kernel, dim3(1), dim3(1024), 0, stream, marks, (int)tiles, heavy, light, counts);
    return (int)hipGetLastError();
}
```

ipercore_amd/networks/generator.py:

```python
import math

import torch
import torch.nn as nn

from .. import ops
from . import packing
from .params import generator_param_shapes


class _Node(nn.Module):

    def __init__(self):
        super().__init__()


class ParamTree(nn.Module):
    def __init__(self, shapes):
        super().__init__()
        self._shapes = dict(shapes)
        for name, shape in shapes.items():
            parts = name.split(".")
            node = self
            for p in parts[:-1]:
                if not hasattr(node, p):
                    node.add_module(p, _Node())
                node = getattr(node, p)
            node.register_parameter(parts[-1], nn.Parameter(torch.empty(*shape)))
        self.reset_parameters()

    @torch.no_grad()
    def reset_parameters(self):
        named = dict(self.named_parameters())
        for name, p in named.items():
            if name.endswith(".weight"):
                fan_in = p.shape[1] * p.shape[2] * p.shape[3]
                bound = 1.0 / math.sqrt(fan_in)
                p.uniform_(-bound, bound)
                b = named.get(name[:-len("weight")] + "bias")
                if b is not None:
                    b.uniform_(-bound, bound)


class _Packed:

    def __init__(self, gen):
        sd = {k: v for k, v in gen.named_parameters()}
        dev = next(gen.parameters()).device
        self.device = dev
        self.version = _param_version(gen)
        nf, n_res, n_down = gen.num_filters, gen.n_res_block, len(gen.num_filters)
        P = packing

        def conv(name, stride=1, pad=None, cin_pad=None, n_pad=None):
            return P.spec_to(P.pack_conv(sd[name + ".weight"], sd.get(name + ".bias"), stride, pad, cin_pad, n_pad), dev)

        def convT(name, n_pad=None):
            return [P.spec_to(s, dev) for s in P.pack_conv_transpose(sd[name + ".weight"], sd.get(name + ".bias"), n_pad)]

        def site(p):
            Wq = sd[p + ".fq.weight"].detach()[:, :, 0, 0].double()
            Wk = sd[p + ".fk.weight"].detach()[:, :, 0, 0].double()
            bq = sd[p + ".fq.bias"].detach().double()
            Wkq = (Wq.t() @ Wk).float()[:, :, None, None].contiguous()
            wkap = (Wk.t() @ bq).float()[None, :, None, None].contiguous()
            d = {
                "fkq": P.spec_to(P.pack_conv(Wkq, None, 1, 0), dev),
                "fkap": P.spec_to(P.pack_conv(wkap, None, 1, 0, None, 64), dev),
                "fv": P.spec_to(P.pack_conv(sd[p + ".fv.weight"], None, 1, 0), dev),
                "bv": sd[p + ".fv.bias"].detach().float().contiguous(),
                "shared": conv(p + ".spade.mlp_shared.0"),
                "gb": P.spec_to(P.pack_spade_gamma_beta(sd[p + ".spade.mlp_gamma.weight"], sd[p + ".spade.mlp_gamma.bias"],
                                                        sd[p + ".spade.mlp_beta.weight"], sd[p + ".spade.mlp_beta.bias"]), dev),
            }
            return d

        cin_pad = 8
        self.tsf_enc = [conv(f"tsf_net_enc.layers.{i}.0", stride=2, cin_pad=cin_pad if i == 0 else None) for i in range(n_down)]
        self.src_enc = [conv(f"src_net.encoders.layers.{i}.0", stride=2, cin_pad=cin_pad if i == 0 else None) for i in range(n_down)]
        self.src_res = [(conv(f"src_net.res_blocks.{i}.main.0"), conv(f"src_net.res_blocks.{i}.main.2")) for i in range(n_res)]
        self.src_dec = [convT(f"src_net.decoders.layers.{i}.0") for i in range(n_down)]
        self.src_head = P.pack_head(sd["src_net.img_reg.0.weight"], sd["src_net.att_reg.0.weight"]).to(dev)
        self.res = [(conv(f"res_blocks.{i}.main.0"), conv(f"res_blocks.{i}.main.2")) for i in range(n_res)]
        if gen.lwb_kind == "att":
            pass
        elif gen.lwb_kind in ("sg_add", "sg_avg"):
            site = lambda p: {"g0": conv(p + ".gate_conv.0"), "g2": conv(p + ".gate_conv.2")}
        else:
            site = lambda p: {}
        self.enc_sites = [site(f"enc_attlwbs.{i}") for i in range(n_down)]
        self.res_sites = [site(f"res_attlwbs.{i}") for i in range(n_res)]
        self.upconvs = [convT(f"tsf_net_dec.upconvs.{i}.0") for i in range(n_down)]
        self.skippers = [conv(f"tsf_net_dec.skippers.{i}.0") for i in range(n_down - 1)]
        self.head = P.pack_head(sd["tsf_img_reg.0.weight"], sd["tsf_att_reg.0.weight"]).to(dev)
        self.head16 = P.pack_head_bf16(sd["tsf_img_reg.0.weight"], sd["tsf_att_reg.0.weight"]).to(dev) if nf[0] == 64 else None
        self.bg = pack_bg_layers(sd, gen.bg_filters, n_res, dev) if gen.has_bg else None


def pack_bg_layers(sd, bgf, n_res, dev):
    P = packing

    def conv(name, stride=1, pad=None, cin_pad=None, n_pad=None):
        return P.spec_to(P.pack_conv(sd[name + ".weight"], sd.get(name + ".bias"), stride, pad, cin_pad, n_pad), dev)

    def convT(name, n_pad=None):
        return [P.spec_to(s, dev) for s in P.pack_conv_transpose(sd[name + ".weight"], sd.get(name + ".bias"), n_pad)]
    i = 0
    layers = [("conv", conv(f"bg_net.main.{i}", stride=1, pad=3, cin_pad=4))]
    i += 3
    for d in range(1, len(bgf)):
        layers.append(("conv", conv(f"bg_net.main.{i}", stride=2)))
        i += 3
    for _ in range(n_res):
        layers.append(("res", (conv(f"bg_net.main.{i}.main.0"), conv(f"bg_net.main.{i}.main.3"))))
        i += 1
    for d in range(len(bgf) - 1, 0, -1):
        layers.append(("convT", convT(f"bg_net.main.{i}")))
        i += 3
    layers.append(("out", conv(f"bg_net.main.{i}", stride=1, pad=3, n_pad=64)))
    return layers


def run_bg_layers(layers, bg4):
    scratch = _Scratch()
    x = bg4

    def norm(t, act, res=None):
        B, h, w, C = t.shape
        mean, rstd = t.new_empty(B, C), t.new_empty(B, C)
        nsplit = max(1, min(64, (h * w) // 64))
        ops.instnorm_stats(t, mean, rstd, scratch.get(B * C * nsplit * 3, t.device), eps=1e-5, nsplit=nsplit)
        return ops.instnorm_apply(t, mean, rstd, torch.empty_like(t), act=act, res=res)

    for kind, spec in layers:
        B, H, W, _ = x.shape
        if kind == "conv":
            y = ops.conv2d(x, spec, x.new_empty(B, H // spec.stride, W // spec.stride, spec.N))
            x = norm(y, ops.ACT_RELU)
        elif kind == "res":
            h = norm(ops.conv2d(x, spec[0], torch.empty_like(x)), ops.ACT_RELU)
            x = norm(ops.conv2d(h, spec[1], torch.empty_like(x)), ops.ACT_NONE, res=x)
        elif kind == "convT":
            y = x.new_empty(B, 2 * H, 2 * W, spec[0].N)
            x = norm(ops.conv_transpose2d(x, spec, y, act=ops.ACT_NONE), ops.ACT_RELU)
        else:
            y = ops.conv2d(x, spec, x.new_empty(B, H, W, spec.N), act=ops.ACT_TANH)
            return ops.nhwc_to_nchw(y, channels=3)


def _skip_lists(lists, cal):
    return (lists, cal) if isinstance(lists, ops.SkipLists) else tuple(lists) + (cal,)


def spade_calibration(st, x):
    _, h, w, C = x.shape
    cal = st.setdefault("cal", {})
    if (h, w) not in cal:
        hook, ops.CONV_HOOK = ops.CONV_HOOK, None
        try:
            z = x.new_zeros(1, h, w, C)
            T = x.new_full((1, 1, h, w, 2), -2.0)
            att = ops.lwb_attention_x(z, z, x.new_zeros(1, h, w), z, st["bv"], T, torch.empty_like(z))
            actv = ops.conv2d(att, st["shared"], x.new_empty(1, h, w, st["shared"].N), act=ops.ACT_RELU)
            gb = ops.conv2d(actv, st["gb"], x.new_empty(1, h, w, st["gb"].N))
        finally:
            ops.CONV_HOOK = hook
        cal[(h, w)] = (actv, gb)
    return cal[(h, w)]


def _param_version(gen):
    return tuple((p.data_ptr(), p._version) for p in gen.parameters())


class SourceFeatures:

    def __init__(self, enc, res, kv, ns, batched=False):
        self.enc, self.res, self.kv, self.ns, self.batched = enc, res, kv, ns, batched


class AttentionLWBGenerator(nn.Module):
    has_bg = True
    lwb_kind = "att"

    def __init__(self, cfg, temporal=False):
        super().__init__()
        self._name = _get(cfg, "name", "AttLWB-SPADE")
        tsf = _get(cfg, "TSFNet")
        sid = _get(cfg, "SIDNet")
        self.num_filters = [int(c) for c in _get(tsf, "num_filters")]
        self.n_res_block = int(_get(tsf, "n_res_block"))
        if [int(c) for c in _get(sid, "num_filters")] != self.num_filters or int(_get(sid, "n_res_block")) != self.n_res_block:
            raise ValueError("SIDNet and TSFNet must share num_filters / n_res_block (the LWB sites pair them up)")
        for c in self.num_filters:
            if c not in (64, 128, 256):
                raise ValueError(f"num_filters entries must be in {{64,128,256}} for the HIP kernels, got {c}")
        self.cond_nc = int(_get(tsf, "cond_nc"))
        self.temporal = temporal
        self.bg_filters, bg_cond = None, 4
        if self.has_bg:
            bgc = _get(cfg, "BGNet")
            self.bg_filters = [int(c) for c in _get(bgc, "num_filters")]
            bg_cond = int(_get(bgc, "cond_nc"))
        shapes = generator_param_shapes(self.num_filters, self.n_res_block, self.bg_filters or (), cond_nc=self.cond_nc,
                                        bg_cond_nc=bg_cond, with_bg=self.has_bg,
                                        lwb={"att": "att", "add": "plain", "avg": "plain"}.get(self.lwb_kind, "softgate"))
        tree = ParamTree(shapes)
        for name, child in tree.named_children():
            self.add_module(name, child)
        self._packed = None
        self.conv_precision = "winograd"

    def packed(self):
        if self._packed is None or self._packed.version != _param_version(self):
            self._packed = _Packed(self)
        return self._packed

    def _check(self, *tensors):
        if torch.is_grad_enabled() and any(p.requires_grad for p in self.parameters()) and self.training:
            raise NotImplementedError("these methods are the no_grad inference engine: call under torch.no_grad() / .eval(), or train "
                                      "through ipercore_amd.networks.training.TrainableGenerator (trainers.LWGTrainer; all five LWB generators)")
        for t in tensors:
            if t is not None and not t.is_cuda:
                raise RuntimeError("ipercore_amd generator runs on the MI355X only: got a CPU tensor (no fallback)")

    @staticmethod
    def _check_square(t):
        if t.shape[-1] != t.shape[-2]:
            raise ValueError(f"square images only (got {t.shape[-2]} x {t.shape[-1]}): the reference's image_size is one number and the "
                             "attention blocks' flow fields are resized to square feature maps")

    @torch.no_grad()
    def _encode_sources_impl(self, src8, batched=False, ns=None):
        pk = self.packed()
        x = src8
        adt = self._act_dtype()
        enc, res = [], []
        for i, spec in enumerate(pk.src_enc):
            n, H, W, _ = x.shape
            y = x.new_empty(n, H // 2, W // 2, spec.N, dtype=adt)
            x = ops.conv2d(x, spec, y, act=ops.ACT_RELU)
            enc.append(x)
        for c0, c1 in pk.src_res:
            h = ops.conv2d(x, c0, torch.empty_like(x), act=ops.ACT_RELU)
            x = ops.conv2d(h, c1, torch.empty_like(x), epi=ops.EPI_RESIDUAL, res=x)
            res.append(x)
        return SourceFeatures(enc, res, self._project_sources(pk, enc, res), ns if ns is not None else src8.shape[0], batched)

    def _project_sources(self, pk, enc, res):
        kv = []
        for feats, sites in ((enc, pk.enc_sites), (res, pk.res_sites)):
            for f, st in zip(feats, sites):
                if self.lwb_kind == "att":
                    n, h, w, _ = f.shape
                    with ops.conv_precision("fp32" if self.conv_precision in ("bf16", "bf16_winograd") else self.conv_precision):
                        kap = ops.conv2d(f.float(), st["fkap"], f.new_empty(n, h, w, 64, dtype=torch.float32))[..., 0].contiguous()
                    kv.append((ops.conv2d(f, st["fkq"], torch.empty_like(f)), ops.conv2d(f, st["fv"], torch.empty_like(f)), kap))
                else:
                    kv.append((f, None, None))
        return kv

    def _attlwb(self, st, tsf_x, kv, Tst, batched, scratch):
        B, h, w, C = tsf_x.shape
        if self.lwb_kind != "att":
            ns = Tst.shape[1]
            Tst = scratch.flow(Tst, h, w)
            if self.lwb_kind == "add":
                return ops.lwb_fuse(tsf_x, kv[0], Tst, torch.empty_like(tsf_x), src_batched=batched)
            if self.lwb_kind == "avg":
                return ops.lwb_fuse(tsf_x, kv[0], Tst, torch.empty_like(tsf_x), scale_o=1.0 / (ns + 1), src_batched=batched)
            g = ops.conv2d(tsf_x, st["g0"], torch.empty_like(tsf_x), act=ops.ACT_RELU)
            g = ops.conv2d(g, st["g2"], torch.empty_like(tsf_x), act=ops.ACT_SIGMOID)
            return ops.lwb_fuse(tsf_x, kv[0], Tst, torch.empty_like(tsf_x), gate=g,
                                scale_w=1.0 if self.lwb_kind == "sg_add" else 1.0 / ns, src_batched=batched)
        mean = tsf_x.new_empty(B, C, dtype=torch.float32)
        rstd = tsf_x.new_empty(B, C, dtype=torch.float32)
        nrec = ops.attn_records(h, w, C, tsf_x.dtype)
        ws = scratch.get(ops.instnorm_finalize_ws(B, C, nrec), tsf_x.device)
        flow = scratch.flow(Tst, h, w)
        if tuple(flow.shape[2:4]) != (h, w):
            raise NotImplementedError("the attention block takes flows resized to its feature size: non-square feature maps are not built "
                                      "(image_size is one number throughout the reference)")
        att = ops.lwb_attention_x(tsf_x, kv[0], kv[2], kv[1], st["bv"], flow, torch.empty_like(tsf_x), stats=ws,
                                  src_batched=batched)
        ops.instnorm_finalize(ws, B, C, nrec, mean, rstd, eps=1e-5)
        actv, out = tsf_x.new_empty(B, h, w, st["shared"].N), torch.empty_like(tsf_x)
        l1 = l5 = None
        if ops.conv2d_lists_apply(att, st["shared"], actv, act=ops.ACT_RELU):
            l1 = _skip_lists(scratch.lists(flow, ops.SPADE_SKIP_D[0]), spade_calibration(st, tsf_x)[0])
        if ops.conv2d_lists_apply(actv, st["gb"], out, epi=ops.EPI_SPADE, xn=tsf_x, mean=mean, rstd=rstd):
            l5 = _skip_lists(scratch.lists(flow, ops.SPADE_SKIP_D[1]), spade_calibration(st, tsf_x)[1])
        ops.conv2d(att, st["shared"], actv, act=ops.ACT_RELU, **({} if l1 is None else {"lists": l1}))
        return ops.conv2d(actv, st["gb"], out, epi=ops.EPI_SPADE, xn=tsf_x, mean=mean, rstd=rstd, **({} if l5 is None else {"lists": l5}))

    @staticmethod
    def _upconv(x, specs, act, q4=False):
        B, H, W, _ = x.shape
        if q4:
            return ops.conv_transpose2d(x, specs, x.new_empty(B, specs[0].N // 4, 2 * H, 2 * W, 4), act=act, q4=True)
        y = x.new_empty(B, 2 * H, 2 * W, specs[0].N)
        return ops.conv_transpose2d(x, specs, y, act=act)

    @torch.no_grad()
    def _run_tsf_impl(self, tsf8, feats, Tst, bg=None, want_pred=True, want_mask=True, want_img=False):
        pk = self.packed()
        scratch = _Scratch()
        n_down = len(pk.tsf_enc)
        x = tsf8
        adt = self._act_dtype()
        if feats.kv[0][0].dtype != adt:
            raise RuntimeError(f"source features are {feats.kv[0][0].dtype} but the generator runs in {self.conv_precision} mode: "
                               "rebuild them (Imitator.set_source / forward_src) after changing conv_precision")
        enc = []
        site = 0
        for i, spec in enumerate(pk.tsf_enc):
            B, H, W, _ = x.shape
            x = ops.conv2d(x, spec, x.new_empty(B, H // 2, W // 2, spec.N, dtype=adt), act=ops.ACT_RELU)
            x = self._attlwb(pk.enc_sites[i], x, feats.kv[site], Tst, feats.batched, scratch)
            site += 1
            enc.append(x)
        for i, (c0, c1) in enumerate(pk.res):
            h = ops.conv2d(x, c0, torch.empty_like(x), act=ops.ACT_RELU)
            x = ops.conv2d(h, c1, torch.empty_like(x), epi=ops.EPI_RESIDUAL, res=x)
            x = self._attlwb(pk.res_sites[i], x, feats.kv[site], Tst, feats.batched, scratch)
            site += 1
        q4 = adt == torch.float32 and self.conv_precision in ("fp32", "winograd", "winograd2x2")
        for i in range(n_down):
            if i == n_down - 1 and pk.head16 is not None and ops.up4_head_eligible(x, pk.upconvs[i], ops.ACT_RELU):
                return ops.up4_head_compose_bf16(x, pk.upconvs[i], pk.head16, bg, want_pred=want_pred and bg is not None, want_mask=want_mask,
                                                 want_img=want_img)
            x = self._upconv(x, pk.upconvs[i], ops.ACT_RELU, q4=q4 and i == n_down - 1)
            if i != n_down - 1:
                skip = enc[n_down - 2 - i]
                sp = pk.skippers[i]
                x = ops.conv2d(skip, sp, x.new_empty(x.shape[0], x.shape[1], x.shape[2], sp.N), x1=x, act=ops.ACT_RELU)
        head = pk.head
        if x.dtype == torch.bfloat16:
            if pk.head16 is not None:
                head = pk.head16
            else:
                x = x.float()
        return ops.head_compose(x, head, bg, want_pred=want_pred and bg is not None, want_mask=want_mask, want_img=want_img, q4=q4)

    def _act_dtype(self):
        return torch.bfloat16 if self.conv_precision in ("bf16", "bf16_winograd") else torch.float32

    @torch.no_grad()
    def _run_bg_impl(self, bg4):
        return run_bg_layers(self.packed().bg, bg4)

    @torch.no_grad()
    def _run_src_decode_impl(self, x):
        pk = self.packed()
        for specs in pk.src_dec:
            x = self._upconv(x, specs, ops.ACT_RELU)
        _, mask, img = ops.head_compose(x.float(), pk.src_head, None, want_pred=False, want_mask=True, want_img=True)
        return img, mask

    def encode_sources(self, *a, **k):
        with ops.conv_precision(self.conv_precision):
            return self._encode_sources_impl(*a, **k)

    def run_tsf(self, *a, **k):
        with ops.conv_precision(self.conv_precision):
            return self._run_tsf_impl(*a, **k)

    def run_bg(self, *a, **k):
        with ops.conv_precision("fp32" if self.conv_precision in ("bf16", "bf16_winograd") else self.conv_precision):
            return self._run_bg_impl(*a, **k)

    def run_src_decode(self, *a, **k):
        with ops.conv_precision(self.conv_precision):
            return self._run_src_decode_impl(*a, **k)

    @torch.no_grad()
    def forward_bg(self, bg_inputs):
        if not self.has_bg:
            raise AttributeError("this generator has no background network")
        self._check(bg_inputs)
        bs, ns, c, h, w = bg_inputs.shape
        x = ops.nchw_to_nhwc(bg_inputs.reshape(bs * ns, c, h, w).contiguous().float(), c_pad=4)
        return self.run_bg(x).view(bs, ns, 3, h, w)

    @torch.no_grad()
    def forward_src(self, src_inputs, only_enc=True):
        self._check(src_inputs)
        self._check_square(src_inputs)
        bs, ns, c, h, w = src_inputs.shape
        src8 = ops.nchw_to_nhwc(src_inputs.reshape(bs * ns, c, h, w).contiguous().float(), c_pad=8)
        feats = self.encode_sources(src8, batched=bs > 1, ns=ns)
        enc = _FeatList(ops.nhwc_to_nchw(t.float()) for t in feats.enc)
        res = _FeatList(ops.nhwc_to_nchw(t.float()) for t in feats.res)
        enc.lwg_cache = res.lwg_cache = feats
        if only_enc:
            return enc, res
        img, mask = self.run_src_decode(feats.res[-1])
        return enc, res, img.view(bs, ns, 3, h, w), mask.view(bs, ns, 1, h, w)

    def _features_from_api(self, src_enc_outs, src_res_outs, bs):
        cache = getattr(src_enc_outs, "lwg_cache", None)
        if cache is not None and getattr(src_res_outs, "lwg_cache", None) is cache:
            return cache
        pk = self.packed()
        adt = self._act_dtype()
        enc = [ops.nchw_to_nhwc(t.contiguous().float()).to(adt) for t in src_enc_outs]
        res = [ops.nchw_to_nhwc(t.contiguous().float()).to(adt) for t in src_res_outs]
        n = enc[0].shape[0]
        return SourceFeatures(enc, res, self._project_sources(pk, enc, res), n // bs, batched=bs > 1)

    @torch.no_grad()
    def forward_tsf(self, tsf_inputs, src_enc_outs, src_res_outs, Tst, temp_enc_outs=None, temp_res_outs=None, Ttt=None):
        self._check(tsf_inputs, Tst)
        self._check_square(tsf_inputs)
        bs = tsf_inputs.shape[0]
        feats = self._features_from_api(src_enc_outs, src_res_outs, bs)
        T = Tst.contiguous().float()
        if temp_enc_outs is not None and Ttt is not None and self.lwb_kind == "att":
            if bs != 1:
                raise NotImplementedError("temporal attention runs one clip per process (bs = 1), as Imitator.inference does")
            tfe = self._features_from_api(temp_enc_outs, temp_res_outs, bs)
            feats = SourceFeatures(feats.enc, feats.res, [tuple(torch.cat([a, ta], dim=0) for a, ta in zip(site, tsite))
                                                          for site, tsite in zip(feats.kv, tfe.kv)],
                                   feats.ns + Ttt.shape[1], batched=False)
            T = torch.cat([T, Ttt.contiguous().float()], dim=1).contiguous()
        tsf8 = ops.nchw_to_nhwc(tsf_inputs.contiguous().float(), c_pad=8)
        _, mask, img = self.run_tsf(tsf8, feats, T, bg=None, want_pred=False, want_mask=True, want_img=True)
        return img, mask

    @torch.no_grad()
    def _forward_streams(self, src_inputs, tsf_inputs, Tst, only_tsf):
        bs, nt = Tst.shape[0], Tst.shape[1]
        if only_tsf:
            enc, res = self.forward_src(src_inputs, only_enc=True)
            src_imgs = src_masks = None
        else:
            enc, res, src_imgs, src_masks = self.forward_src(src_inputs, only_enc=False)
        imgs, masks = [], []
        for t in range(nt):
            if t != 0 and self.temporal:
                raise NotImplementedError("multi-step temporal training forward (Ttt inside forward()) is not built; "
                                          "temporal INFERENCE goes through Imitator(temporal=True) / forward_tsf(temp_*)")
            img, mask = self.forward_tsf(tsf_inputs[:, t], enc, res, Tst[:, t].contiguous())
            imgs.append(img)
            masks.append(mask)
        return src_imgs, src_masks, torch.stack(imgs, dim=1), torch.stack(masks, dim=1)

    @torch.no_grad()
    def forward(self, bg_inputs, src_inputs, tsf_inputs, Tst, Ttt=None, only_tsf=True):
        bg_img = self.forward_bg(bg_inputs)
        src_imgs, src_masks, imgs, masks = self._forward_streams(src_inputs, tsf_inputs, Tst, only_tsf)
        if only_tsf:
            return bg_img, imgs, masks
        return bg_img, src_imgs, src_masks, imgs, masks


class AttentionLWBFrontGenerator(AttentionLWBGenerator):
    has_bg = False

    @torch.no_grad()
    def forward(self, src_inputs, tsf_inputs, Tst, Ttt=None, only_tsf=True):
        src_imgs, src_masks, imgs, masks = self._forward_streams(src_inputs, tsf_inputs, Tst, only_tsf)
        if only_tsf:
            return imgs, masks
        return src_imgs, src_masks, imgs, masks


class AddLWBGenerator(AttentionLWBGenerator):
    lwb_kind = "add"


class AvgLWBGenerator(AttentionLWBGenerator):
    lwb_kind = "avg"


class SoftGateAddLWBGenerator(AttentionLWBGenerator):
    lwb_kind = "sg_add"


class SoftGateAvgLWBGenerator(AttentionLWBGenerator):
    lwb_kind = "sg_avg"


class _FeatList(list):
    """A list that can carry the engine's cache as an attribute (plain lists cannot)."""


class _Scratch:
    def __init__(self):
        self.buf = None
        self.flows = {}

    def flow(self, Tst, h, w):
        if Tst.shape[2] == h and Tst.shape[3] == w:
            return Tst
        if h != w:
            return Tst
        key = (h, w, Tst.data_ptr())
        if key not in self.flows:
            self.flows[key] = ops.flow_resize(Tst, h, w)
        return self.flows[key]

    def lists(self, flow, d):
        key = ("lists", flow.shape[2], flow.shape[3], d, flow.data_ptr())
        if key not in self.flows:
            self.flows[key] = ops.spade_skip_lists(flow, d)
        return self.flows[key]

    def get(self, n, device):
        if self.buf is None or self.buf.numel() < n or self.buf.device != device:
            self.buf = torch.empty(max(n, 1 << 16), device=device, dtype=torch.float32)
        return self.buf


def _get(cfg, key, default=None):
    if isinstance(cfg, dict):
        if key in cfg:
            return cfg[key]
    elif hasattr(cfg, key):
        return getattr(cfg, key)
    if default is not None:
        return default
    raise KeyError(key)


class _ConcatPacked:

    def __init__(self, gen):
        sd = {k: v for k, v in gen.named_parameters()}
        dev = next(gen.parameters()).device
        self.version = _param_version(gen)
        P = packing
        nf, n_down = gen.num_filters, len(gen.num_filters)

        def conv(name, stride=1, pad=None, cin_pad=None):
            return P.spec_to(P.pack_conv(sd[name + ".weight"], sd.get(name + ".bias"), stride, pad, cin_pad, None), dev)
        self.enc = [conv(f"tsf_net.encoders.layers.{i}.0", stride=2, cin_pad=gen.cin_pad if i == 0 else None) for i in range(n_down)]
        self.res = [(conv(f"tsf_net.res_blocks.{i}.main.0"), conv(f"tsf_net.res_blocks.{i}.main.2")) for i in range(gen.n_res_block)]
        self.dec = [[P.spec_to(sp, dev) for sp in P.pack_conv_transpose(sd[f"tsf_net.decoders.layers.{i}.0.weight"],
                                                                       sd[f"tsf_net.decoders.layers.{i}.0.bias"], None)] for i in range(n_down)]
        self.head = P.pack_head(sd["tsf_net.img_reg.0.weight"], sd["tsf_net.att_reg.0.weight"]).to(dev)
        self.bg = pack_bg_layers(sd, gen.bg_filters, gen.bg_n_res_block, dev)


class InputConcatGenerator(nn.Module):
    has_bg = True

    def __init__(self, cfg, temporal=False):
        super().__init__()
        self._name = _get(cfg, "name", "InputConcat")
        tsf, bgc = _get(cfg, "TSFNet"), _get(cfg, "BGNet")
        self.num_filters = [int(c) for c in _get(tsf, "num_filters")]
        self.n_res_block = int(_get(tsf, "n_res_block"))
        self.cond_nc = int(_get(tsf, "cond_nc"))
        self.num_source = int(_get(tsf, "num_source", 4)) if self._uses_sources() else None
        self.bg_filters = [int(c) for c in _get(bgc, "num_filters")]
        self.bg_n_res_block = int(_get(bgc, "n_res_block"))
        self.temporal = temporal
        if self.num_filters[0] != 64 or any(c not in (64, 128, 256) for c in self.num_filters):
            raise ValueError(f"num_filters must start with 64 and stay in {{64,128,256}} for the HIP kernels, got {self.num_filters}")
        self.cin_pad = 8 if self.cond_nc <= 8 else (16 if self.cond_nc <= 16 else (self.cond_nc + 31) // 32 * 32)
        from .params import concat_generator_param_shapes
        tree = ParamTree(concat_generator_param_shapes(self.num_filters, self.n_res_block, self.bg_filters, self.cond_nc,
                                                        int(_get(bgc, "cond_nc", 4)), self.bg_n_res_block))
        for name, child in tree.named_children():
            self.add_module(name, child)
        self._packed = None

    def _uses_sources(self):
        return True

    def packed(self):
        if self._packed is None or self._packed.version != _param_version(self):
            self._packed = _ConcatPacked(self)
        return self._packed

    @staticmethod
    def _check(*tensors):
        for t in tensors:
            if t is not None and not t.is_cuda:
                raise RuntimeError("ipercore_amd generator runs on the MI355X only: got a CPU tensor (no fallback)")

    @torch.no_grad()
    def forward_bg(self, bg_inputs):
        self._check(bg_inputs)
        bs, ns, c, h, w = bg_inputs.shape
        x = ops.nchw_to_nhwc(bg_inputs.reshape(bs * ns, c, h, w).contiguous().float(), c_pad=4)
        return run_bg_layers(self.packed().bg, x).view(bs, ns, 3, h, w)

    def forward_src(self, src_inputs, only_enc=True):
        bs, ns, _, h, w = src_inputs.shape
        need = self.num_source
        if ns > need:
            src_inputs = src_inputs[:, 0:need]
        elif ns < need:
            src_inputs = torch.cat([src_inputs, torch.stack([src_inputs[:, s % ns] for s in range(need - ns)], dim=1)], dim=1)
        enc = src_inputs.reshape(bs, -1, h, w)
        return (enc, enc) if only_enc else (enc, enc, None, None)

    @torch.no_grad()
    def _autoencode(self, inputs):
        self._check(inputs)
        pk = self.packed()
        x = ops.nchw_to_nhwc(inputs.contiguous().float(), c_pad=self.cin_pad)
        for spec in pk.enc:
            n, H, W, _ = x.shape
            x = ops.conv2d(x, spec, x.new_empty(n, H // 2, W // 2, spec.N), act=ops.ACT_RELU)
        for c0, c1 in pk.res:
            t = ops.conv2d(x, c0, torch.empty_like(x), act=ops.ACT_RELU)
            x = ops.conv2d(t, c1, torch.empty_like(x), epi=ops.EPI_RESIDUAL, res=x)
        for specs in pk.dec:
            n, H, W, _ = x.shape
            x = ops.conv_transpose2d(x, specs, x.new_empty(n, 2 * H, 2 * W, specs[0].N), act=ops.ACT_RELU)
        _, mask, img = ops.head_compose(x, pk.head, None, want_pred=False, want_mask=True, want_img=True)
        return img, mask

    @torch.no_grad()
    def forward_tsf(self, tsf_inputs, src_enc_outs, src_res_outs=None, Tst=None, temp_enc_outs=None, temp_res_outs=None, Ttt=None):
        return self._autoencode(torch.cat([src_enc_outs, tsf_inputs[:, -3:]], dim=1))

    @torch.no_grad()
    def forward(self, bg_inputs, src_inputs, tsf_inputs, Tst=None, Ttt=None, only_tsf=True):
        bg_img = self.forward_bg(bg_inputs)
        enc, _ = self.forward_src(src_inputs, only_enc=True)
        outs = [self.forward_tsf(tsf_inputs[:, t], enc) for t in range(tsf_inputs.shape[1])]
        return bg_img, torch.stack([o[0] for o in outs], dim=1), torch.stack([o[1] for o in outs], dim=1)


class TextureWarpingGenerator(InputConcatGenerator):

    def __init__(self, cfg, temporal=False):
        super().__init__(cfg, temporal)
        self._name = _get(cfg, "name", "TextureWarping")

    def _uses_sources(self):
        return False

    def forward_src(self, src_inputs, only_enc=True):
        bs, ns, _, h, w = src_inputs.shape
        enc = src_inputs.reshape(bs, -1, h, w)
        return (enc, enc) if only_enc else (enc, enc, None, None)

    @torch.no_grad()
    def forward_tsf(self, tsf_inputs, src_enc_outs=None, src_res_outs=None, Tst=None, temp_enc_outs=None, temp_res_outs=None, Ttt=None):
        return self._autoencode(tsf_inputs)

    @torch.no_grad()
    def forward(self, bg_inputs, src_inputs, tsf_inputs, Tst=None, Ttt=None, only_tsf=True):
        bg_img = self.forward_bg(bg_inputs)
        bs, nt, c, h, w = tsf_inputs.shape
        img, mask = self._autoencode(tsf_inputs.reshape(bs * nt, c, h, w))
        return bg_img, img.view(bs, nt, 3, h, w), mask.view(bs, nt, 1, h, w)
```

ipercore_amd/ops.py:

```python
import ctypes

import torch

from . import _lib
from ._lib import ACT_LRELU, ACT_NONE, ACT_RELU, ACT_RELU_MASK, ACT_SIGMOID, ACT_TANH, EPI_NONE, EPI_RESIDUAL, EPI_SPADE

EYE_DIST = 2.7320508075688776


def _ptr(t, dtype=torch.float32):
    if t is None:
        return None
    if not t.is_cuda:
        raise RuntimeError("ipercore_amd ops need CUDA (HIP) tensors: the MI355X path has no CPU fallback")
    if t.dtype != dtype:
        raise TypeError(f"expected {dtype}, got {t.dtype}")
    if not t.is_contiguous():
        raise ValueError("tensor must be contiguous")
    return t.data_ptr()


CONV_PRECISION = "fp32"


class conv_precision(object):

    def __init__(self, mode):
        assert mode in ("fp32", "bf16", "bf16_winograd", "split", "winograd", "winograd2x2")
        self.mode = mode

    def __enter__(self):
        global CONV_PRECISION, _MODE_WINO4
        self.prev = CONV_PRECISION, _MODE_WINO4
        CONV_PRECISION, _MODE_WINO4 = ("winograd", False) if self.mode == "winograd2x2" else (self.mode, True)

    def __exit__(self, *exc):
        global CONV_PRECISION, _MODE_WINO4
        CONV_PRECISION, _MODE_WINO4 = self.prev


_MODE_WINO4 = True


CONV_HOOK = None


def _stream():
    return torch.cuda.current_stream().cuda_stream


class ConvSpec:
    __slots__ = ("w", "bias", "N", "Cin", "ntaps", "dy", "dx", "stride", "cshift", "omul", "ooy", "oox", "algo_kn", "_panels")

    def __init__(self, w, bias, N, Cin, taps, stride=1, omul=1, ooy=0, oox=0, algo_kn=None):
        self.w, self.bias, self.N, self.Cin = w, bias, int(N), int(Cin)
        self.algo_kn = int(algo_kn) if algo_kn is not None else len(taps) * int(Cin) * int(N)
        self.ntaps = len(taps)
        self.dy = [int(t[0]) for t in taps]
        self.dx = [int(t[1]) for t in taps]
        self.stride, self.omul, self.ooy, self.oox = stride, omul, ooy, oox
        self._panels = {}
        self.cshift = 0
        if self.Cin % 32 != 0:
            q = self.Cin // 4
            assert q in (1, 2, 4), "small-Cin path handles Cin in {4, 8, 16}"
            self.cshift = q.bit_length() - 1


def _derived(specs, key, build, bias=False):
    specs = specs if isinstance(specs, (list, tuple)) else (specs,)
    src = [s.w for s in specs] + ([specs[0].bias] if bias else [])
    hit = specs[0]._panels.get(key)
    if hit is None or len(hit[0]) != len(src) or any(a is not b for a, b in zip(hit[0], src)):
        hit = specs[0]._panels[key] = (src, build())
    return hit[1]


def _tap_order9(spec):
    order = [0] * 9
    for t in range(spec.ntaps):
        order[3 * (spec.dy[t] + 1) + spec.dx[t] + 1] = t
    return order


def _spade_columns(N, blk, device):
    j = torch.arange(N, device=device)
    ch, beta = blk * (j // (2 * blk)) + j % blk, (j % (2 * blk)) // blk
    return 64 * (ch // 32) + (ch % 32) + 32 * beta


def _w16v2(spec):
    def build():
        K4, N, _ = spec.w.shape
        cin, nt = spec.Cin, spec.ntaps
        assert cin % 64 == 0 and K4 * 4 == nt * cin, (cin, nt, K4)
        wk = spec.w.permute(0, 2, 1).reshape(cin // 64, 2, nt, 32, N)
        wk = wk.permute(0, 2, 1, 3, 4).reshape(cin // 64 * nt, 64, N)
        rows = wk.permute(0, 2, 1).reshape(cin // 64 * nt, N, 8, 8)
        n = torch.arange(N, device=spec.w.device)
        slot = torch.arange(8, device=spec.w.device)
        src = slot[None, :] ^ ((n[:, None] >> 1) & 7)
        rows = torch.gather(rows, 2, src[None, :, :, None].expand(rows.shape[0], N, 8, 8))
        return rows.reshape(cin // 64 * nt, N, 64).contiguous().to(torch.bfloat16)
    return _derived(spec, "w16v2", build)


def _hr_eligible(spec, x0, y, out_hw):
    if not BF16_HR or spec.stride != 1 or spec.ntaps not in (9, 4) or spec.N % 64 != 0 or spec.Cin % 64 != 0:
        return False
    if any(abs(d) > 1 for d in spec.dy) or any(abs(d) > 1 for d in spec.dx):
        return False
    OH, OW = ((y.shape[1], y.shape[2]) if spec.omul == 1 else (y.shape[1] // spec.omul, y.shape[2] // spec.omul)) if out_hw is None else out_hw
    return (OH, OW) == (x0.shape[1], x0.shape[2])


def _hr_tap_order(spec):
    return sorted(range(spec.ntaps), key=lambda t: (spec.dy[t], spec.dx[t]))


def _w16hr(spec, spade):
    def build():
        K4, N, _ = spec.w.shape
        cin, nt = spec.Cin, spec.ntaps
        wk = spec.w.permute(0, 2, 1).reshape(cin // 64, 2, nt, 32, N).permute(0, 2, 1, 3, 4).reshape(cin // 64, nt, 64, N)
        wk = wk[:, _hr_tap_order(spec)].reshape(cin // 64 * nt, 64, N)
        bias = spec.bias
        if spade:
            old = _spade_columns(N, 16, spec.w.device)
            wk = wk[:, :, old]
            bias = None if bias is None else bias[old].contiguous()
        return wk.reshape(cin // 64 * nt, 4, 16, N).permute(0, 1, 3, 2).contiguous().to(torch.bfloat16), bias
    return _derived(spec, ("w16hr", bool(spade)), build, bias=True)


BF16_WINO_MIN_CIN = 64
_WINO_G = ((1.0, 0.0, 0.0), (0.5, 0.5, 0.5), (0.5, -0.5, 0.5), (0.0, 0.0, 1.0))


def _bf16_wino_eligible(spec, x0, y, x1, epi, act, out_hw, ycoff=0):
    if spec.ntaps != 9 or spec.stride != 1 or spec.omul != 1 or spec.N % 64 != 0 or spec.Cin % 64 != 0 or spec.Cin < BF16_WINO_MIN_CIN:
        return False
    if (y.shape[1], y.shape[2]) != (x0.shape[1], x0.shape[2]) or (out_hw is not None and tuple(out_hw) != (x0.shape[1], x0.shape[2])):
        return False
    if sorted(zip(spec.dy, spec.dx)) != _WINO_TAPS or epi not in (EPI_NONE, EPI_RESIDUAL, EPI_SPADE):
        return False
    if act not in (ACT_NONE, ACT_RELU, ACT_TANH, ACT_SIGMOID) or y.dtype != torch.bfloat16:
        return False
    if x1 is not None and (x1.dtype != torch.bfloat16 or x0.shape[3] % 64 != 0):
        return False
    if epi == EPI_SPADE:
        return y.shape[3] * 2 == spec.N and ycoff == 0
    return y.shape[3] % 8 == 0 and ycoff % 8 == 0 and ycoff + spec.N <= y.shape[3]


def wwino16_index(ks, p, n, e, N):
    return ((ks * 16 + p) * N + n) * 16 + e


def wwino16_spade_column(j):
    return 4 * (j // 8) + j % 4, (j % 8) // 4


def _wwino16(spec, spade):
    def build():
        K4, N, _ = spec.w.shape
        cin, nt = spec.Cin, spec.ntaps
        assert nt == 9 and cin % 64 == 0 and N % 64 == 0 and K4 * 4 == nt * cin, (cin, nt, K4, N)
        dev = spec.w.device
        wk = spec.w.permute(0, 2, 1).reshape(cin // 32, nt, 32, N).permute(1, 0, 2, 3).reshape(nt, cin, N)
        w33 = wk[_tap_order9(spec)].reshape(3, 3, cin, N).to(torch.float64)
        G = torch.tensor(_WINO_G, dtype=torch.float64, device=dev)
        U = torch.einsum("ar,rscn,bs->abcn", G, w33, G)
        bias = spec.bias
        if spade:
            old = _spade_columns(N, 4, dev)
            U = U[:, :, :, old]
            bias = None if bias is None else bias[old].contiguous()
        return U.reshape(16, cin // 16, 16, N).permute(1, 0, 3, 2).contiguous().to(torch.bfloat16), bias
    return _derived(spec, ("wwino16", bool(spade)), build, bias=True)


BF16_HR = True
BF16_PW = True
BF16_C8 = True


def _pw_eligible(spec, x0, y, x1, epi, out_hw):
    if not BF16_PW or spec.ntaps != 1 or spec.stride != 1 or spec.omul != 1 or x1 is not None or epi != EPI_NONE:
        return False
    if spec.dy[0] != 0 or spec.dx[0] != 0 or spec.N != spec.Cin or spec.N not in (64, 128, 256):
        return False
    OH, OW = (y.shape[1], y.shape[2]) if out_hw is None else out_hw
    return (OH, OW) == (x0.shape[1], x0.shape[2])


def _w16c8(spec):
    def build():
        K4, N, _ = spec.w.shape
        nks = (spec.ntaps + 1) // 2
        wk = spec.w.permute(0, 2, 1).reshape(K4 * 4, N)
        if wk.shape[0] < nks * 16:
            wk = torch.cat([wk, wk.new_zeros(nks * 16 - wk.shape[0], N)], dim=0)
        return wk[:nks * 16].reshape(nks, 16, N).permute(0, 2, 1).contiguous().to(torch.bfloat16)
    return _derived(spec, "w16c8", build)


def _w16x3(spec):
    def build():
        K4, N, _ = spec.w.shape
        wk = spec.w.permute(0, 2, 1).reshape(K4 * 4, N)
        hi = wk.to(torch.bfloat16)
        r1 = wk - hi.float()
        mid = r1.to(torch.bfloat16)
        lo = (r1 - mid.float()).to(torch.bfloat16)
        return torch.stack([hi, mid, lo]).view(3, K4 // 2, 8, N).permute(0, 1, 3, 2).contiguous()
    return _derived(spec, "w16x3", build)


_WINO_TAPS = sorted((dy, dx) for dy in (-1, 0, 1) for dx in (-1, 0, 1))


def _wino_eligible(spec, x0, y, x1, epi, act, out_hw, q4, ycoff=0):
    if q4 or x0.dtype != torch.float32 or y.dtype != torch.float32 or epi not in (EPI_NONE, EPI_RESIDUAL, EPI_SPADE) or \
            (act == ACT_RELU_MASK and epi != EPI_RESIDUAL):
        return False
    if x1 is not None and (x1.dtype != torch.float32 or x0.shape[3] % 8 != 0 or x1.shape[3] % 8 != 0):
        return False
    if spec.ntaps != 9 or spec.stride != 1 or spec.omul != 1 or spec.Cin % 32 != 0 or spec.N % 64 != 0:
        return False
    if epi == EPI_SPADE and (y.shape[3] * 2 != spec.N or ycoff != 0):
        return False
    if sorted(zip(spec.dy, spec.dx)) != _WINO_TAPS:
        return False
    hw = (y.shape[1], y.shape[2]) if out_hw is None else tuple(out_hw)
    return hw == (x0.shape[1], x0.shape[2]) == (y.shape[1], y.shape[2])


WINO_MIN_GRID = 128
WINO_SPLITK = True


def _wino_plan(a, spec, y, splitk):
    if not splitk:
        return 0
    blocks, slices, nbv = ctypes.c_longlong(0), ctypes.c_int(0), ctypes.c_int(0)
    if _lib.lib().lwg_conv2d_winograd_plan(a, 1 if WINO_SPLITK else 0, ctypes.byref(blocks), ctypes.byref(slices), ctypes.byref(nbv), None) != 0:
        return None
    units32 = blocks.value * (nbv.value // 32)
    return slices.value * a.M * spec.N if units32 >= WINO_MIN_GRID else None


def _wwino(spec):
    def build():
        cin, N, tap9 = _wino_panel_source(spec)
        if PANEL_CACHE is not None:
            U = PANEL_CACHE.winograd(spec, list(tap9))
            if U is not None:
                return U
        U = torch.empty(16, cin // 8, 2, N, 4, device=spec.w.device, dtype=torch.float32)
        _lib.check(_lib.lib().lwg_winograd_panel_f32(_ptr(spec.w), _ptr(U), cin, N, tap9, _stream()), "lwg_winograd_panel_f32")
        return U
    return _derived(spec, "wwino", build)


def _wino_panel_source(spec):
    K4, N, _ = spec.w.shape
    cin, nt = spec.Cin, spec.ntaps
    assert nt == 9 and cin % 32 == 0 and K4 * 4 == nt * cin, (cin, nt, K4)
    if not spec.w.is_cuda:
        raise RuntimeError("ipercore_amd ops need CUDA (HIP) tensors: the MI355X path has no CPU fallback")
    return cin, N, (ctypes.c_int * 9)(*_tap_order9(spec))


WINO4 = True
WINO4_MIN_CIN = 64


def _wino4_use(spec, splitk):
    return WINO4 and _MODE_WINO4 and not splitk and spec.Cin >= WINO4_MIN_CIN


def _wwino4(spec):
    def build():
        cin, N, tap9 = _wino_panel_source(spec)
        U = torch.empty(4, cin // 8, 4, 2, 9 * N, device=spec.w.device, dtype=torch.float32)
        _lib.check(_lib.lib().lwg_winograd4_panel_f32(_ptr(spec.w), _ptr(U), cin, N, tap9, _stream()), "lwg_winograd4_panel_f32")
        return U
    return _derived(spec, "wwino4", build)


SPADE_SKIP = True
SPADE_SKIP_D = (1, 5)


SPADE_SKIP_FINE = True

_LISTS_APPLY = {}


class SkipLists(tuple):
    fine = None


def spade_skip_fine_apply(x0):
    return SPADE_SKIP_FINE


def spade_skip_lists(flow, d):
    B, ns, h, w, two = flow.shape
    assert two == 2 and flow.dtype == torch.float32
    tiles = B * ((h + 15) // 16) * ((w + 31) // 32)
    buf = torch.empty(15 * tiles + 4, device=flow.device, dtype=torch.int32)
    fmarks, fheavy, flight = buf[:4 * tiles], buf[4 * tiles:8 * tiles], buf[8 * tiles:12 * tiles]
    bb = buf[12 * tiles:]
    marks, heavy, light, counts, fcounts = bb[:tiles], bb[tiles:2 * tiles], bb[2 * tiles:3 * tiles], bb[3 * tiles:3 * tiles + 2], bb[3 * tiles + 2:]
    i32 = torch.int32
    _lib.check(_lib.lib().lwg_spade_skip_fine_lists_f32(_ptr(flow), B, ns, h, w, int(d), _ptr(marks, i32), _ptr(heavy, i32), _ptr(light, i32),
                                                        _ptr(counts, i32), _ptr(fmarks, i32), _ptr(fheavy, i32), _ptr(flight, i32), _ptr(fcounts, i32),
                                                        _stream()), "lwg_spade_skip_fine_lists_f32")
    out = SkipLists((heavy, light, counts))
    out.fine = (fheavy, flight, fcounts)
    return out


def conv2d_lists_apply(x0, spec, y, epi=EPI_NONE, act=ACT_NONE, xn=None, mean=None, rstd=None):
    if not SPADE_SKIP or CONV_PRECISION != "winograd" or not x0.is_cuda or x0.dtype != torch.float32 or not _wino4_use(spec, False) or \
            not _wino_eligible(spec, x0, y, None, epi, act, None, False):
        return False
    key = (x0.shape, y.shape, spec.Cin, spec.N, epi, act)
    if key not in _LISTS_APPLY:
        a = conv_args(x0, spec, y, None, epi, act, None, xn, mean, rstd)
        a.w = _ptr(_wwino4(spec))
        _LISTS_APPLY[key] = bool(_lib.lib().lwg_conv2d_winograd4_list_applies(a))
    return _LISTS_APPLY[key]


def conv_args(x0, spec, y, x1=None, epi=EPI_NONE, act=ACT_NONE, res=None, xn=None, mean=None, rstd=None,
              out_hw=None, ycoff=0, q4=False):
    B, H, W, C0 = x0.shape
    C1 = 0 if x1 is None else x1.shape[3]
    assert C0 + C1 == spec.Cin, (C0, C1, spec.Cin)
    if q4:
        YB, YCq, YH, YW, four = y.shape
        assert four == 4 and y.dtype == torch.float32 and x0.dtype == torch.float32 and epi == EPI_NONE and y.is_contiguous()
        YC = 4 * YCq
    else:
        YB, YH, YW, YC = y.shape
    if out_hw is None:
        OH, OW = (YH, YW) if spec.omul == 1 else (YH // spec.omul, YW // spec.omul)
    else:
        OH, OW = out_hw
    a = _lib.LwgConvArgs()
    xdt, ydt = x0.dtype, y.dtype
    a.xdt = _lib.DT_BF16 if xdt == torch.bfloat16 else _lib.DT_F32
    a.ydt = _lib.DT_F32_Q4 if q4 else (_lib.DT_BF16 if ydt == torch.bfloat16 else _lib.DT_F32)
    a.x0, a.x1 = _ptr(x0, xdt), _ptr(x1, xdt)
    a.C0, a.C1 = C0, C1
    a.B, a.H, a.W = B, H, W
    a.OH, a.OW, a.M = OH, OW, B * OH * OW
    a.stride, a.ntaps, a.cshift = spec.stride, spec.ntaps, spec.cshift
    a.w, a.N, a.bias = _ptr(spec.w), spec.N, _ptr(spec.bias)
    a.y, a.YH, a.YW, a.YC, a.ycoff = _ptr(y, ydt), YH, YW, YC, ycoff
    a.omul, a.ooy, a.oox = spec.omul, spec.ooy, spec.oox
    a.epi, a.act = epi, act
    a.res, a.xn, a.mean, a.rstd = _ptr(res, ydt), _ptr(xn, ydt), _ptr(mean), _ptr(rstd)
    for i in range(spec.ntaps):
        a.dy[i] = spec.dy[i]
        a.dx[i] = spec.dx[i]
    return a


def _hook_end(a, spec, epi, kind, slices=True, extra=0):
    n = (max(1, int(_lib.lib().lwg_conv_slice_count(a))) if slices else 1) + extra
    CONV_HOOK(False, a.M, spec, epi, {"kernels": n, "kind": kind})


def conv2d(x0, spec, y, x1=None, epi=EPI_NONE, act=ACT_NONE, res=None, xn=None, mean=None, rstd=None,
           out_hw=None, ycoff=0, splitk=False, q4=False, lists=None):
    a = conv_args(x0, spec, y, x1, epi, act, res, xn, mean, rstd, out_hw, ycoff, q4)
    if q4 and (splitk or CONV_PRECISION not in ("fp32", "winograd") or x0.dtype != torch.float32):
        raise ValueError("channel-quad-plane outputs: fp32 activations on the fp32 MFMA path, no split-K")
    if CONV_HOOK is not None:
        CONV_HOOK(True, a.M, spec, epi, None)
    if lists is not None and not (x0.dtype == torch.float32 and y.dtype == torch.float32 and CONV_PRECISION == "winograd" and _wino4_use(spec, splitk)):
        raise ValueError("lists: the F(4x4, 3x3) launches of the \"winograd\" mode only (conv2d_lists_apply)")
    kind, sliced, extra = "direct", True, 0
    if x0.dtype == torch.bfloat16:
        kind = "bf16"
        if y.dtype != torch.bfloat16 or spec.Cin % 64 != 0:
            raise ValueError("bf16 convolutions need bf16 outputs and Cin % 64 == 0")
        if CONV_PRECISION == "bf16_winograd" and _bf16_wino_eligible(spec, x0, y, x1, epi, act, out_hw, ycoff):
            kind, sliced = "bf16_winograd", False
            panel, bias = _wwino16(spec, epi == EPI_SPADE)
            a.w, a.bias = _ptr(panel, torch.bfloat16), _ptr(bias)
            for i, (dy, dx) in enumerate(_WINO_TAPS):
                a.dy[i], a.dx[i] = dy, dx
            _lib.check(_lib.lib().lwg_conv2d_winograd_bf16(a, _stream()), "lwg_conv2d_winograd_bf16")
        elif _hr_eligible(spec, x0, y, out_hw) or _pw_eligible(spec, x0, y, x1, epi, out_hw):
            panel, bias = _w16hr(spec, epi == EPI_SPADE)
            a.w, a.bias = _ptr(panel, torch.bfloat16), _ptr(bias)
            for i, t in enumerate(_hr_tap_order(spec)):
                a.dy[i], a.dx[i] = spec.dy[t], spec.dx[t]
            _lib.check(_lib.lib().lwg_conv2d_nhwc_bf16_hr(a, _stream()), "lwg_conv2d_nhwc_bf16_hr")
        else:
            a.w = _ptr(_w16v2(spec), torch.bfloat16)
            _lib.check(_lib.lib().lwg_conv2d_nhwc_bf16(a, _stream()), "lwg_conv2d_nhwc_bf16")
    elif y.dtype == torch.bfloat16:
        if BF16_C8 and spec.Cin == 8 and spec.N == 64 and spec.ntaps <= 10 and x1 is None and epi == EPI_NONE and spec.omul == 1:
            a.w = _ptr(_w16c8(spec), torch.bfloat16)
            _lib.check(_lib.lib().lwg_conv2d_nhwc_c8_bf16(a, _stream()), "lwg_conv2d_nhwc_c8_bf16")
        else:
            _lib.check(_lib.lib().lwg_conv2d_nhwc_f32(a, _stream()), "lwg_conv2d_nhwc_f32")
    elif CONV_PRECISION == "winograd" and _wino_eligible(spec, x0, y, x1, epi, act, out_hw, q4, ycoff) and \
            (nws := _wino_plan(a, spec, y, splitk)) is not None:
        kind, sliced = "winograd", False
        if _wino4_use(spec, splitk):
            a.w = _ptr(_wwino4(spec))
            kind = "winograd4"
            if lists is not None:
                i32 = torch.int32
                fine = len(lists) == 2 and isinstance(lists[0], SkipLists)
                if fine:
                    sl, cal = lists
                    fine = sl.fine is not None and spade_skip_fine_apply(x0)
                    lists = tuple(sl.fine if fine else sl) + (cal,)
                ld = _lib.LwgConvLists(_ptr(lists[0], i32), _ptr(lists[1], i32), _ptr(lists[2], i32), _ptr(lists[3]))
                if fine:
                    _lib.check(_lib.lib().lwg_conv2d_winograd4_fine_f32(a, ctypes.byref(ld), _stream()), "lwg_conv2d_winograd4_fine_f32")
                else:
                    _lib.check(_lib.lib().lwg_conv2d_winograd4_list_f32(a, ctypes.byref(ld), _stream()), "lwg_conv2d_winograd4_list_f32")
            else:
                _lib.check(_lib.lib().lwg_conv2d_winograd4_f32(a, _stream()), "lwg_conv2d_winograd4_f32")
        elif nws:
            a.w = _ptr(_wwino(spec))
            ws, extra = torch.empty(nws, device=x0.device, dtype=torch.float32), 1
            _lib.check(_lib.lib().lwg_conv2d_winograd_f32_ws(a, _ptr(ws), _stream()), "lwg_conv2d_winograd_f32_ws")
        else:
            a.w = _ptr(_wwino(spec))
            _lib.check(_lib.lib().lwg_conv2d_winograd_f32(a, _stream()), "lwg_conv2d_winograd_f32")
    elif CONV_PRECISION == "split" and spec.Cin % 32 == 0:
        a.w = _ptr(_w16x3(spec), torch.bfloat16)
        kind = "split"
        _lib.check(_lib.lib().lwg_conv2d_nhwc_f32_split(a, _stream()), "lwg_conv2d_nhwc_f32_split")
    else:
        nws = _lib.lib().lwg_conv2d_ws_floats(a) if splitk else 0
        if nws:
            ws = torch.empty(nws, device=x0.device, dtype=torch.float32)
            _lib.check(_lib.lib().lwg_conv2d_nhwc_f32_ws(a, _ptr(ws), _stream()), "lwg_conv2d_nhwc_f32_ws")
        else:
            _lib.check(_lib.lib().lwg_conv2d_nhwc_f32(a, _stream()), "lwg_conv2d_nhwc_f32")
    if CONV_HOOK is not None:
        _hook_end(a, spec, epi, kind, sliced, extra)
    return y


WINO_UP4 = True
F32_UP4 = True
BF16_UP4 = True


def _parity_specs_ok(specs):
    s0 = specs[0]
    return (len(specs) == 4 and all(s.ntaps == 4 and s.omul == 2 and s.stride == 1 and (s.ooy, s.oox) == (i >> 1, i & 1) and s.N == s0.N and s.Cin == s0.Cin
                                    and [(dy - (i >> 1), dx - (i & 1)) for dy, dx in zip(s.dy, s.dx)] == list(zip(s0.dy, s0.dx)) for i, s in enumerate(specs)))


def _wwino_t(specs):
    def build():
        Cin, N = specs[0].Cin, specs[0].N
        G = torch.tensor([[1.0, 0.0], [1.0, 1.0], [0.0, 1.0]], dtype=torch.float64, device=specs[0].w.device)
        parts = []
        for par, g in enumerate(_parity_subkernels(specs)):
            u = torch.einsum("ar,rqcn,bq->abcn", G, g, G)
            if par >> 1:
                u[0] = -u[0]
            if par & 1:
                u[:, 0] = -u[:, 0]
            parts.append(u.reshape(9, Cin, N))
        U9 = torch.stack(parts).float()
        U = torch.cat([U9[:, 0:4].permute(0, 2, 3, 1).reshape(4, Cin, 4 * N), U9[:, 4:8].permute(0, 2, 3, 1).reshape(4, Cin, 4 * N), U9[:, 8]], dim=2)
        return U.view(4, Cin // 8, 4, 2, 9 * N).contiguous()
    return _derived(specs, "wwino_t", build)


def _parity_subkernels(specs):
    Cin, N = specs[0].Cin, specs[0].N
    out = []
    for par, sp in enumerate(specs):
        py, px = par >> 1, par & 1
        W = sp.w.double().permute(0, 2, 1).reshape(4 * Cin, N)
        W = W.view(Cin // 32, 4, 32, N).permute(1, 0, 2, 3).reshape(4, Cin, N)
        g = torch.zeros(2, 2, Cin, N, dtype=torch.float64, device=W.device)
        for t, (dy, dx) in enumerate(zip(sp.dy, sp.dx)):
            g[dy - (py - 1), dx - (px - 1)] = W[t]
        out.append(g)
    return out


_G_X24 = ((1.0, 0.0), (0.5, 0.5), (-1.0 / 6.0, 1.0 / 6.0), (-8.0 / 3.0, -4.0 / 3.0), (0.0, 0.5))


def _wwino_t24(specs):
    def build():
        Cin, N = specs[0].Cin, specs[0].N
        Gy = torch.tensor([[1.0, 0.0], [1.0, 1.0], [0.0, 1.0]], dtype=torch.float64, device=specs[0].w.device)
        Gx = torch.tensor(_G_X24, dtype=torch.float64, device=specs[0].w.device)
        parts = []
        for par, g in enumerate(_parity_subkernels(specs)):
            u = torch.einsum("ar,rqcn,bq->abcn", Gy, g, Gx)
            if par >> 1:
                u[0] = -u[0]
            parts.append(torch.cat([u[:, :3].reshape(9, Cin, N), u[:, 3:].reshape(6, Cin, N)]))
        U15 = torch.stack(parts).float()
        quad = lambda lo, hi: U15[:, lo:hi].permute(0, 2, 3, 1).reshape(4, Cin, (hi - lo) * N)
        U = torch.cat([quad(0, 4), quad(4, 8), U15[:, 8], quad(9, 13), U15[:, 13], U15[:, 14]], dim=2)
        return U.view(4, Cin // 8, 4, 2, 15 * N).contiguous()
    return _derived(specs, "wwino_t24", build)


WINO_UP4_24 = True
WINO_UP4_24_MIN_HW = 64 * 64


def _up4_24(x):
    return WINO_UP4_24 and x.shape[1] * x.shape[2] >= WINO_UP4_24_MIN_HW


class _FusedTransposeSpec(object):

    def __init__(self, s0, panel):
        self.N, self.Cin, self.ntaps, self.stride, self.omul = 4 * s0.N, s0.Cin, 16, 1, 2
        self.algo_kn, self.w = 4 * s0.algo_kn, panel


def _fused_transpose_launch(a, s0, panel, entry, kind, sliced=True, extra=(), kernels=None):
    a.w = _ptr(panel, panel.dtype)
    if CONV_HOOK is not None:
        whole = _FusedTransposeSpec(s0, panel)
        CONV_HOOK(True, a.M, whole, EPI_NONE, None)
    _lib.check(getattr(_lib.lib(), entry)(a, *extra, _stream()), entry)
    if CONV_HOOK is not None:
        if kernels is None:
            _hook_end(a, whole, EPI_NONE, kind, sliced)
        else:
            CONV_HOOK(False, a.M, whole, EPI_NONE, {"kernels": kernels, "kind": kind})


def _w16up(specs):
    return _derived(specs, "w16up", lambda: torch.stack([_w16hr(s, False)[0] for s in specs]).contiguous())


def _w32up(specs):
    return _derived(specs, "w32up", lambda: torch.stack([s.w.reshape(-1) for s in specs]).contiguous())


def conv_transpose2d(x, specs, y, act=ACT_NONE, splitk=False, out_hw=None, q4=False):
    s0 = specs[0]
    if (BF16_UP4 and BF16_HR and x.dtype == torch.bfloat16 and y.dtype == torch.bfloat16 and len(specs) == 4 and s0.Cin in (64, 128)
            and s0.N % 64 == 0 and all(s.ntaps == 4 and s.omul == 2 and (s.ooy, s.oox) == (i >> 1, i & 1) for i, s in enumerate(specs))):
        _fused_transpose_launch(conv_args(x, s0, y, act=act), s0, _w16up(specs), "lwg_conv_transpose4_nhwc_bf16", "up4")
        return y
    if (WINO_UP4 and CONV_PRECISION == "winograd" and not splitk and out_hw is None and x.is_cuda and x.dtype == torch.float32 and y.dtype == torch.float32
            and s0.Cin % 32 == 0 and s0.N % 32 == 0 and _parity_specs_ok(specs)):
        a = conv_args(x, s0, y, act=act, q4=q4)
        if _up4_24(x):
            _fused_transpose_launch(a, s0, _wwino_t24(specs), "lwg_conv_transpose4_winograd24_f32", "winograd_up4", False)
        else:
            _fused_transpose_launch(a, s0, _wwino_t(specs), "lwg_conv_transpose4_winograd_f32", "winograd_up4", False)
        return y
    if (F32_UP4 and x.is_cuda and x.dtype == torch.float32 and y.dtype == torch.float32 and CONV_PRECISION in ("fp32", "winograd") and s0.Cin % 32 == 0
            and _parity_specs_ok(specs)):
        a = conv_args(x, s0, y, act=act, q4=q4)
        if _lib.lib().lwg_conv_transpose4_is_one_grid(a):
            _fused_transpose_launch(a, s0, _w32up(specs), "lwg_conv_transpose4_nhwc_f32", "up4")
            return y
    for s in specs:
        conv2d(x, s, y, act=act, splitk=splitk, out_hw=None if out_hw is None else out_hw(s), q4=q4)
    return y


def instnorm_stats(x, mean, rstd, ws, eps=1e-5, nsplit=None):
    B, H, W, C = x.shape
    HW = H * W
    if nsplit is None:
        nsplit = max(1, min(64, HW // 64))
    assert ws.numel() >= B * C * nsplit * 3
    if x.dtype == torch.bfloat16:
        _lib.check(_lib.lib().lwg_instnorm_stats_nhwc_bf16(_ptr(x, torch.bfloat16), B, HW, C, eps, _ptr(mean), _ptr(rstd), _ptr(ws), nsplit,
                                                            _stream()), "lwg_instnorm_stats_nhwc_bf16")
        return
    _lib.check(_lib.lib().lwg_instnorm_stats_nhwc_f32(_ptr(x), B, HW, C, eps, _ptr(mean), _ptr(rstd), _ptr(ws), nsplit,
                                                       _stream()), "lwg_instnorm_stats_nhwc_f32")


def instnorm_apply(x, mean, rstd, y, act=ACT_NONE, res=None):
    B, H, W, C = x.shape
    _lib.check(_lib.lib().lwg_instnorm_apply_nhwc_f32(_ptr(x), _ptr(mean), _ptr(rstd), _ptr(res), _ptr(y), B, H * W, C, act,
                                                       _stream()), "lwg_instnorm_apply_nhwc_f32")
    return y


def flow_resize(T, h, w):
    B, ns, S = T.shape[0], T.shape[1], T.shape[2]
    T = T.contiguous()
    out = torch.empty(B, ns, h, w, 2, device=T.device, dtype=torch.float32)
    _lib.check(_lib.lib().lwg_flow_resize_f32(_ptr(T), B * ns, S, h, w, _ptr(out), _stream()), "lwg_flow_resize_f32")
    return out


def lwb_attention(q, Ks, Vs, bk, bv, T, out, src_batched=False):
    B, h, w, C = q.shape
    ns = T.shape[1]
    S = T.shape[2]
    assert T.shape[0] == B and Ks.shape[0] == (B * ns if src_batched else ns) and tuple(Ks.shape[1:]) == (h, w, C)
    if q.dtype == torch.bfloat16:
        bf = torch.bfloat16
        _lib.check(_lib.lib().lwg_lwb_attention_bf16(_ptr(q, bf), _ptr(Ks, bf), _ptr(Vs, bf), _ptr(bk), _ptr(bv), _ptr(T), _ptr(out, bf), B, ns, h,
                                                      w, C, S, 1 if src_batched else 0, _stream()), "lwg_lwb_attention_bf16")
        return out
    _lib.check(_lib.lib().lwg_lwb_attention_f32(_ptr(q), _ptr(Ks), _ptr(Vs), _ptr(bk), _ptr(bv), _ptr(T), _ptr(out), B, ns, h,
                                                 w, C, S, 1 if src_batched else 0, _stream()), "lwg_lwb_attention_f32")
    return out


def attn_records(h, w, C, dtype=torch.float32):
    n = _lib.lib().lwg_lwb_attention_x_records(int(h), int(w), int(C), 2 if dtype == torch.bfloat16 else 4)
    if n <= 0:
        raise ValueError(f"lwb_attention_x: unsupported (h, w, C, dtype) = {(h, w, C, dtype)}")
    return n


def lwb_attention_x(x, Kq, kappa, Vs, bv, T, out, stats=None, src_batched=False):
    B, h, w, C = x.shape
    ns = T.shape[1]
    nsrc = B * ns if src_batched else ns
    assert tuple(T.shape) == (B, ns, h, w, 2), (tuple(T.shape), (B, ns, h, w, 2))
    assert tuple(Kq.shape) == (nsrc, h, w, C) and tuple(Vs.shape) == (nsrc, h, w, C) and tuple(kappa.shape) == (nsrc, h, w)
    assert Kq.dtype == x.dtype and Vs.dtype == x.dtype and out.dtype == x.dtype and kappa.dtype == torch.float32
    assert stats is None or stats.numel() >= B * attn_records(h, w, C, x.dtype) * C * 3
    if x.dtype == torch.bfloat16:
        bf = torch.bfloat16
        _lib.check(_lib.lib().lwg_lwb_attention_x_bf16(_ptr(x, bf), _ptr(Kq, bf), _ptr(kappa), _ptr(Vs, bf), _ptr(bv), _ptr(T), _ptr(out, bf),
                                                        _ptr(stats), B, ns, h, w, C, 1 if src_batched else 0, _stream()), "lwg_lwb_attention_x_bf16")
        return out
    _lib.check(_lib.lib().lwg_lwb_attention_x_f32(_ptr(x), _ptr(Kq), _ptr(kappa), _ptr(Vs), _ptr(bv), _ptr(T), _ptr(out), _ptr(stats), B, ns, h, w,
                                                   C, 1 if src_batched else 0, _stream()), "lwg_lwb_attention_x_f32")
    return out


def instnorm_finalize_ws(B, C, nrec):
    return int(_lib.lib().lwg_instnorm_finalize_ws_floats(int(B), int(C), int(nrec)))


def instnorm_finalize(ws, B, C, nrec, mean, rstd, eps=1e-5):
    assert ws.numel() >= instnorm_finalize_ws(B, C, nrec)
    _lib.check(_lib.lib().lwg_instnorm_finalize_f32(_ptr(ws), B, C, nrec, float(eps), _ptr(mean), _ptr(rstd), _stream()), "lwg_instnorm_finalize_f32")


def lwb_fuse(tsf_x, src_x, T, out, gate=None, scale_w=1.0, scale_o=1.0, src_batched=False):
    B, h, w, C = tsf_x.shape
    ns, S = T.shape[1], T.shape[2]
    assert T.shape[0] == B and src_x.shape[0] == (B * ns if src_batched else ns) and tuple(src_x.shape[1:]) == (h, w, C)
    assert src_x.dtype == tsf_x.dtype and out.dtype == tsf_x.dtype and (gate is None or gate.dtype == tsf_x.dtype)
    assert T.dtype == torch.float32
    if tsf_x.dtype == torch.bfloat16:
        bf = torch.bfloat16
        _lib.check(_lib.lib().lwg_lwb_fuse_bf16(_ptr(tsf_x, bf), _ptr(src_x, bf), _ptr(gate, bf), _ptr(T), _ptr(out, bf), B, ns, h, w, C, S,
                                                1 if src_batched else 0, float(scale_w), float(scale_o), _stream()), "lwg_lwb_fuse_bf16")
        return out
    _lib.check(_lib.lib().lwg_lwb_fuse_f32(_ptr(tsf_x), _ptr(src_x), _ptr(gate), _ptr(T), _ptr(out), B, ns, h, w, C, S,
                                           1 if src_batched else 0, float(scale_w), float(scale_o), _stream()), "lwg_lwb_fuse_f32")
    return out


def lwb_fuse_bwd(src_x, gate, T, dout, src_batched=False, scale_w=1.0, scale_o=1.0):
    B, h, w, C = dout.shape
    ns, S = T.shape[1], T.shape[2]
    assert T.shape[0] == B and src_x.shape[0] == (B * ns if src_batched else ns) and tuple(src_x.shape[1:]) == (h, w, C)
    assert gate is None or gate.shape == dout.shape
    dout = dout.contiguous()
    d_tsf = torch.empty_like(dout)
    d_src = torch.zeros_like(src_x)
    d_gate = None if gate is None else torch.empty_like(dout)
    _lib.check(_lib.lib().lwg_lwb_fuse_bwd_f32(_ptr(src_x), _ptr(gate), _ptr(T), _ptr(dout), _ptr(d_tsf), _ptr(d_src), _ptr(d_gate), B, ns, h, w, C,
                                               S, 1 if src_batched else 0, float(scale_w), float(scale_o), _stream()), "lwg_lwb_fuse_bwd_f32")
    return d_tsf, d_src, d_gate


def lwb_attention_bwd(q, Ks, Vs, bk, bv, T, dout, src_batched=False):
    B, h, w, C = q.shape
    ns, S = T.shape[1], T.shape[2]
    dout = dout.contiguous()
    dq = torch.empty_like(q)
    dKs = torch.zeros_like(Ks)
    dVs = torch.zeros_like(Vs)
    _lib.check(_lib.lib().lwg_lwb_attention_bwd_f32(_ptr(q), _ptr(Ks), _ptr(Vs), _ptr(bk), _ptr(bv), _ptr(T), _ptr(dout), _ptr(dq),
                                                     _ptr(dKs), _ptr(dVs), B, ns, h, w, C, S, 1 if src_batched else 0, _stream()),
               "lwg_lwb_attention_bwd_f32")
    return dq, dKs, dVs


def lwb_attention_kv(q, kv, bk, bv, T, out, src_batched=False):
    B, h, w, C = q.shape
    ns, S = T.shape[1], T.shape[2]
    assert T.shape[0] == B and kv.shape[0] == (B * ns if src_batched else ns) and tuple(kv.shape[1:]) == (h, w, 2 * C)
    _lib.check(_lib.lib().lwg_lwb_attention_kv_f32(_ptr(q), _ptr(kv), _ptr(bk), _ptr(bv), _ptr(T), _ptr(out), B, ns, h, w, C, S,
                                                    1 if src_batched else 0, _stream()), "lwg_lwb_attention_kv_f32")
    return out


def lwb_attention_kv_bwd(q, kv, bk, bv, T, dout, src_batched=False):
    B, h, w, C = q.shape
    ns, S = T.shape[1], T.shape[2]
    dout = dout.contiguous()
    dq = torch.empty_like(q)
    dkv = torch.zeros_like(kv)
    _lib.check(_lib.lib().lwg_lwb_attention_kv_bwd_f32(_ptr(q), _ptr(kv), _ptr(bk), _ptr(bv), _ptr(T), _ptr(dout), _ptr(dq), _ptr(dkv),
                                                        B, ns, h, w, C, S, 1 if src_batched else 0, _stream()), "lwg_lwb_attention_kv_bwd_f32")
    return dq, dkv


def project_faces(verts, cam, faces, want_faces_v=True, want_f2pts=True):
    B, nv, _ = verts.shape
    nf = faces.shape[0]
    fv = torch.empty(B, nf, 3, 3, device=verts.device, dtype=torch.float32) if want_faces_v else None
    f2 = torch.empty(B, nf, 3, 2, device=verts.device, dtype=torch.float32) if want_f2pts else None
    cam = cam.contiguous()
    _lib.check(_lib.lib().lwg_project_faces_f32(_ptr(verts), _ptr(cam), _ptr(faces, torch.int32), B, nv, nf, EYE_DIST, _ptr(fv),
                                                 _ptr(f2), _stream()), "lwg_project_faces_f32")
    return fv, f2


def rasterize_fim_wim(faces_v, image_size, near=0.1, far=100.0):
    B, nf = faces_v.shape[0], faces_v.shape[1]
    S = int(image_size)
    dev = faces_v.device
    fim = torch.empty(B, S, S, device=dev, dtype=torch.int32)
    wim = torch.empty(B, S, S, 3, device=dev, dtype=torch.float32)
    ws = torch.empty(_lib.lib().lwg_rasterize_ws_bytes(B, nf, S), device=dev, dtype=torch.uint8)
    _lib.check(_lib.lib().lwg_rasterize_fim_wim_f32(_ptr(faces_v), B, nf, S, near, far, _ptr(fim, torch.int32), _ptr(wim),
                                                     ws.data_ptr(), _stream()), "lwg_rasterize_fim_wim_f32")
    return fim, wim


def texture_sample(fim, wim, faces_v, textures, eps=1e-3, background_color=(0.0, 0.0, 0.0)):
    B, S = fim.shape[0], fim.shape[1]
    nf, T = faces_v.shape[1], textures.shape[2]
    assert textures.shape[0] in (1, B) and textures.shape[1] == nf
    rgb = torch.empty(B, S, S, 3, device=fim.device, dtype=torch.float32)
    bg = (ctypes.c_float * 3)(*[float(c) for c in background_color])
    _lib.check(_lib.lib().lwg_texture_sample_f32(_ptr(fim, torch.int32), _ptr(wim), _ptr(faces_v.contiguous()), _ptr(textures.contiguous()), B, nf,
                                                 S, T, 1 if textures.shape[0] == B and B > 1 else (1 if textures.shape[0] == B else 0),
                                                 float(eps), bg, _ptr(rgb), _stream()), "lwg_texture_sample_f32")
    return rgb


def flow_compose(fim, wim, map_fn, f_uvs2img, uv_img4, src_f2pts, want_cond=False, want_tuv=False):
    B, S, _ = fim.shape
    nf = f_uvs2img.shape[0]
    ns = src_f2pts.shape[0]
    dev = fim.device
    tsf = torch.empty(B, S, S, 8, device=dev, dtype=torch.float32)
    Tst = torch.empty(B, ns, S, S, 2, device=dev, dtype=torch.float32)
    cond = torch.empty(B, 3, S, S, device=dev, dtype=torch.float32) if want_cond else None
    tuv = torch.empty(B, S, S, 2, device=dev, dtype=torch.float32) if want_tuv else None
    Hu, Wu = uv_img4.shape[0], uv_img4.shape[1]
    _lib.check(_lib.lib().lwg_flow_compose_f32(_ptr(fim, torch.int32), _ptr(wim), B, S, _ptr(map_fn), nf, _ptr(f_uvs2img),
                                                _ptr(uv_img4), Hu, Wu, _ptr(src_f2pts), ns, _ptr(tsf), _ptr(Tst), _ptr(cond),
                                                _ptr(tuv), _stream()), "lwg_flow_compose_f32")
    return tsf, Tst, cond, tuv


def bc_transform(f2pts, fim, wim):
    B, S, _ = fim.shape
    nf = f2pts.shape[1]
    T = torch.empty(B, S, S, 2, device=fim.device, dtype=torch.float32)
    _lib.check(_lib.lib().lwg_bc_transform_f32(_ptr(f2pts), _ptr(fim, torch.int32), _ptr(wim), B, S, nf, _ptr(T), _stream()),
               "lwg_bc_transform_f32")
    return T


def encode_fim(fim, map_fn):
    B, S, _ = fim.shape
    D = map_fn.shape[1]
    out = torch.empty(B, D, S, S, device=fim.device, dtype=torch.float32)
    _lib.check(_lib.lib().lwg_encode_fim_f32(_ptr(fim, torch.int32), _ptr(map_fn), B, S, map_fn.shape[0] - 1, D, _ptr(out),
                                              _stream()), "lwg_encode_fim_f32")
    return out


def head_compose(x, wpk, bg, want_pred=True, want_mask=True, want_img=False, q4=False):
    if q4:
        B, Cq, S, _, four = x.shape
        C = 4 * Cq
        assert four == 4 and x.dtype == torch.float32 and x.is_contiguous()
    else:
        B, S, _, C = x.shape
    dev = x.device
    pred = torch.empty(B, 3, S, S, device=dev, dtype=torch.float32) if want_pred else None
    mask = torch.empty(B, 1, S, S, device=dev, dtype=torch.float32) if want_mask else None
    img = torch.empty(B, 3, S, S, device=dev, dtype=torch.float32) if want_img else None
    bstride = 0
    if bg is not None and bg.shape[0] != 1:
        assert bg.shape[0] == B
        bstride = 3 * S * S
    if x.dtype == torch.bfloat16:
        _lib.check(_lib.lib().lwg_head_compose_bf16(_ptr(x, torch.bfloat16), _ptr(wpk, torch.bfloat16), _ptr(bg), bstride, B, S, C, _ptr(pred),
                                                     _ptr(mask), _ptr(img), _stream()), "lwg_head_compose_bf16")
        return pred, mask, img
    if q4:
        _lib.check(_lib.lib().lwg_head_compose_q4_f32(_ptr(x), _ptr(wpk), _ptr(bg), bstride, B, S, C, _ptr(pred), _ptr(mask), _ptr(img),
                                                       _stream()), "lwg_head_compose_q4_f32")
        return pred, mask, img
    _lib.check(_lib.lib().lwg_head_compose_f32(_ptr(x), _ptr(wpk), _ptr(bg), bstride, B, S, C, _ptr(pred), _ptr(mask), _ptr(img),
                                                _stream()), "lwg_head_compose_f32")
    return pred, mask, img


BF16_UP4_HEAD = True


def up4_head_eligible(x, specs, act):
    s0 = specs[0]
    return (BF16_UP4_HEAD and BF16_UP4 and BF16_HR and x.is_cuda and x.dtype == torch.bfloat16 and len(specs) == 4 and s0.Cin == 128 and s0.N == 64
            and act == ACT_RELU and s0.bias is not None
            and all(s.ntaps == 4 and s.omul == 2 and (s.ooy, s.oox) == (i >> 1, i & 1) for i, s in enumerate(specs)))


def up4_head_compose_bf16(x, specs, head16, bg, want_pred=True, want_mask=True, want_img=False):
    B, H, W, _ = x.shape
    s0 = specs[0]
    dev = x.device
    S2h, S2w = 2 * H, 2 * W
    pred = torch.empty(B, 3, S2h, S2w, device=dev, dtype=torch.float32) if want_pred else None
    mask = torch.empty(B, 1, S2h, S2w, device=dev, dtype=torch.float32) if want_mask else None
    img = torch.empty(B, 3, S2h, S2w, device=dev, dtype=torch.float32) if want_img else None
    bstride = 0
    if bg is not None and bg.shape[0] != 1:
        assert bg.shape[0] == B
        bstride = 3 * S2h * S2w
    a = conv_args(x, s0, torch.empty(0, S2h, S2w, s0.N, device=dev, dtype=torch.bfloat16), act=ACT_RELU, out_hw=(H, W))
    per = H * W * 256
    _fused_transpose_launch(a, s0, _w16up(specs), "lwg_up4_head_compose_bf16", "up4_head",
                            extra=(_ptr(head16, torch.bfloat16), _ptr(bg), bstride, _ptr(pred), _ptr(mask), _ptr(img)),
                            kernels=max(1, -(-B // max(1, (0xC0000000 - 1) // per))))
    return pred, mask, img


def thin_conv(x, wpk, ks):
    B, S, S2, C = x.shape
    assert S == S2 and tuple(wpk.shape) == (ks * ks, C, 4), (x.shape, wpk.shape, ks)
    y = torch.empty(B, S, S, 4, device=x.device, dtype=torch.float32)
    _lib.check(_lib.lib().lwg_thin_conv_f32(_ptr(x), _ptr(wpk), B, S, C, ks, _ptr(y), _stream()), "lwg_thin_conv_f32")
    return y


def nchw_to_nhwc(x, c_pad=None):
    B, C = x.shape[0], x.shape[1]
    H, W = x.shape[2], x.shape[3]
    Cp = C if c_pad is None else c_pad
    y = torch.empty(B, H, W, Cp, device=x.device, dtype=torch.float32)
    _lib.check(_lib.lib().lwg_nchw_to_nhwc_f32(_ptr(x), _ptr(y), B, C, Cp, H * W, _stream()), "lwg_nchw_to_nhwc_f32")
    return y


def nhwc_to_nchw(x, channels=None):
    B, H, W, Cs = x.shape
    C = Cs if channels is None else channels
    y = torch.empty(B, C, H, W, device=x.device, dtype=torch.float32)
    _lib.check(_lib.lib().lwg_nhwc_to_nchw_f32(_ptr(x), _ptr(y), B, C, Cs, H * W, _stream()), "lwg_nhwc_to_nchw_f32")
    return y


def smpl_lbs(model, pose, beta, cam, offsets=None, links=None):
    B = pose.shape[0]
    nv = model["v_template"].shape[0]
    nj = model["J_regressor"].shape[0]
    dev = pose.device
    assert pose.shape[1] == 3 * nj, (pose.shape, nj)
    verts = torch.empty(B, nv, 3, device=dev, dtype=torch.float32)
    j3d = torch.empty(B, nj, 3, device=dev, dtype=torch.float32)
    j2d = torch.empty(B, nj, 2, device=dev, dtype=torch.float32) if cam is not None else None
    ws = torch.empty(_lib.lib().lwg_smpl_lbs_ws_floats(B, nv, nj), device=dev, dtype=torch.float32)
    off_batched = 0
    if offsets is not None:
        off_batched = 1 if offsets.dim() == 3 else 0
        if off_batched:
            assert offsets.shape[0] == B
    nlinks = 0 if links is None else links.shape[0]
    nbeta = beta.shape[1]
    _lib.check(_lib.lib().lwg_smpl_lbs_f32(
        _ptr(pose), pose.shape[1], _ptr(beta), nbeta, nbeta, _ptr(cam), 0 if cam is None else cam.shape[1],
        _ptr(model["v_template"]), _ptr(offsets), off_batched, _ptr(model["shapedirs"]), _ptr(model["posedirs"]),
        _ptr(model["J_regressor"]), _ptr(model["parents"], torch.int32), _ptr(model["lbs_weights"]),
        _ptr(links, torch.int32), nlinks, B, nv, nj, _ptr(verts), _ptr(j3d), _ptr(j2d), _ptr(ws), _stream()),
        "lwg_smpl_lbs_f32")
    return verts, j3d, j2d


MORPH_MODES = {"erode": 0, "dilate": 1, "soft_dilate": 2}


def morph(x, ks, mode="erode"):
    n, c, H, W = x.shape
    assert c == 1
    x = x.contiguous().float()
    out = torch.empty_like(x)
    ws = torch.empty_like(x)
    _lib.check(_lib.lib().lwg_morph_f32(_ptr(x), _ptr(out), n, H, W, int(ks), MORPH_MODES[mode], _ptr(ws), _stream()),
               "lwg_morph_f32")
    return out


def canny_edges(sil, gauss9, sobelx9, low, high):
    import ctypes
    n, c, H, W = sil.shape
    assert c == 1
    sil = sil.contiguous().float()
    edges = torch.empty_like(sil)
    ws = torch.empty(3 * sil.numel(), device=sil.device, dtype=torch.float32)
    g = (ctypes.c_float * 9)(*[float(v) for v in gauss9])
    s = (ctypes.c_float * 9)(*[float(v) for v in sobelx9])
    _lib.check(_lib.lib().lwg_canny_f32(_ptr(sil), n, H, W, g, s, float(low), float(high), _ptr(edges), _ptr(ws), _stream()),
               "lwg_canny_f32")
    return edges


def boundary_fill(src, confidant, outpad, edges, want_top3=False):
    n, _, H, W = src.shape
    src, confidant, outpad, edges = (t.contiguous().float() for t in (src, confidant, outpad, edges))
    out = torch.empty_like(src)
    top3 = torch.empty(n, 3, H, W, device=src.device, dtype=torch.int32) if want_top3 else None
    ws = torch.empty(n * (H * W + 1), device=src.device, dtype=torch.int32)
    _lib.check(_lib.lib().lwg_boundary_fill_f32(_ptr(src), _ptr(confidant), _ptr(outpad), _ptr(edges), n, H, W, _ptr(out),
                                                 _ptr(top3, torch.int32), _ptr(ws, torch.int32), _stream()),
               "lwg_boundary_fill_f32")
    return out, ws[n * H * W:], top3


def grid_sample(img, grid):
    n, Ho, Wo, _ = grid.shape
    nb, C, H, W = img.shape
    assert nb in (1, n)
    img, grid = img.contiguous().float(), grid.contiguous().float()
    out = torch.empty(n, C, Ho, Wo, device=img.device, dtype=torch.float32)
    _lib.check(_lib.lib().lwg_grid_sample_nchw_f32(_ptr(img), 0 if (nb == 1 and n > 1) else C * H * W, _ptr(grid), n, C, H, W,
                                                    Ho, Wo, _ptr(out), _stream()), "lwg_grid_sample_nchw_f32")
    return out


def uv_merge(src_warp, vis):
    ns, _, H, W = src_warp.shape
    out = torch.empty(3, H, W, device=src_warp.device, dtype=torch.float32)
    _lib.check(_lib.lib().lwg_uv_merge_f32(_ptr(src_warp.contiguous()), _ptr(vis.contiguous()), ns, H, W, _ptr(out), _stream()),
               "lwg_uv_merge_f32")
    return out


def uv_merge_parts(uv_imgs, vis):
    n, _, H, W = uv_imgs.shape
    out = torch.empty(1, 3, H, W, device=uv_imgs.device, dtype=torch.float32)
    _lib.check(_lib.lib().lwg_uv_merge_parts_f32(_ptr(uv_imgs.contiguous()), _ptr(vis.contiguous()), n, H, W, _ptr(out), _stream()),
               "lwg_uv_merge_parts_f32")
    return out


def pack_inputs(a, b, mask, c_pad):
    n, Ca, H, W = a.shape
    Cb = 0 if b is None else b.shape[1]
    out = torch.empty(n, H, W, c_pad, device=a.device, dtype=torch.float32)
    _lib.check(_lib.lib().lwg_pack_inputs_f32(_ptr(a.contiguous()), Ca, _ptr(None if b is None else b.contiguous()), Cb,
                                               _ptr(None if mask is None else mask.contiguous()), n, H, W, c_pad, _ptr(out),
                                               _stream()), "lwg_pack_inputs_f32")
    return out


def frames_to_u8(pred, bgr=False):
    B, C, S, S2 = pred.shape
    assert C == 3 and S == S2
    out = torch.empty(B, S, S, 3, device=pred.device, dtype=torch.uint8)
    if B == 0:
        return out
    _lib.check(_lib.lib().lwg_frames_to_u8(_ptr(pred), B, S, 1 if bgr else 0, _ptr(out, torch.uint8), _stream()), "lwg_frames_to_u8")
    return out


def conv2d_wgrad(x0, spec, dy, x1=None, out_hw=None, ycoff=0):
    a = conv_args(x0, spec, dy, x1=x1, out_hw=out_hw, ycoff=ycoff)
    Ktot = spec.ntaps * spec.Cin
    dw = torch.empty(Ktot, spec.N, device=x0.device, dtype=torch.float32)
    ws = torch.empty(_lib.lib().lwg_conv2d_wgrad_ws_floats(Ktot, spec.N, a.M), device=x0.device, dtype=torch.float32)
    _lib.check(_lib.lib().lwg_conv2d_wgrad_nhwc_f32(a, _ptr(dy), _ptr(dw), _ptr(ws), _stream()), "lwg_conv2d_wgrad_nhwc_f32")
    return dw


def conv2d_wgrad_unpacked(x0, spec, dy, dw, transposed, kidx, cin, nout, x1=None, out_hw=None, ycoff=0, db=None):
    a = conv_args(x0, spec, dy, x1=x1, out_hw=out_hw, ycoff=ycoff)
    Ktot = spec.ntaps * spec.Cin
    D0, D1, KH, KW = dw.shape
    assert dw.is_contiguous() and len(kidx) == spec.ntaps
    ws = torch.empty(_lib.lib().lwg_conv2d_wgrad_ws_floats(Ktot, spec.N, a.M), device=x0.device, dtype=torch.float32)
    arr = (ctypes.c_int * spec.ntaps)(*[int(k) for k in kidx])
    if db is not None:
        assert db.is_contiguous() and db.dtype == torch.float32 and db.numel() == nout
    _lib.check(_lib.lib().lwg_conv2d_wgrad_unpacked_f32(a, _ptr(dy), _ptr(ws), _ptr(dw), D0, D1, KH, KW, 1 if transposed else 0, arr, cin, nout,
                                                        None if db is None else _ptr(db), _stream()), "lwg_conv2d_wgrad_unpacked_f32")
    return dw


WGRAD_PRECISION = "direct"


class wgrad_precision(object):

    def __init__(self, mode):
        assert mode in ("direct", "winograd")
        self.mode = mode

    def __enter__(self):
        global WGRAD_PRECISION
        self.prev = WGRAD_PRECISION
        WGRAD_PRECISION = self.mode

    def __exit__(self, *exc):
        global WGRAD_PRECISION
        WGRAD_PRECISION = self.prev


def _wgrad_wino_use(x0, spec, dy, x1=None):
    if not (x0.is_cuda and dy.is_cuda) or x0.dtype != torch.float32 or dy.dtype != torch.float32 or x0.dim() != 4 or dy.dim() != 4:
        return False
    if x1 is not None and (not x1.is_cuda or x1.dtype != torch.float32 or x1.shape[:3] != x0.shape[:3] or x1.shape[3] % 64 != 0):
        return False
    C1 = 0 if x1 is None else x1.shape[3]
    if spec.ntaps != 9 or spec.stride != 1 or spec.omul != 1 or spec.ooy != 0 or spec.oox != 0 or x0.shape[3] % 64 != 0 or spec.N % 64 != 0 or \
            x0.shape[3] + C1 != spec.Cin or list(zip(spec.dy, spec.dx)) != _WINO_TAPS:
        return False
    if tuple(dy.shape) != (x0.shape[0], x0.shape[1], x0.shape[2], spec.N):
        return False
    pix = x0.shape[0] * x0.shape[1] * x0.shape[2]
    return pix * max(x0.shape[3], C1, spec.N) * 4 < 0xC0000000


def conv2d_wgrad_winograd(x0, spec, dy, dw, cin, nout, x1=None):
    a = conv_args(x0, spec, dy, x1=x1)
    assert dw.is_contiguous() and tuple(dw.shape) == (nout, cin, 3, 3)
    nws = _lib.lib().lwg_conv2d_wgrad_winograd_ws_floats(a)
    if nws == 0:
        raise ValueError("launch outside lwg_conv2d_wgrad_winograd_f32's contract (ops._wgrad_wino_use)")
    if CONV_HOOK is not None:
        CONV_HOOK(True, a.M, spec, EPI_NONE, None)
    ws = torch.empty(nws, device=x0.device, dtype=torch.float32)
    _lib.check(_lib.lib().lwg_conv2d_wgrad_winograd_f32(a, _ptr(dy), _ptr(ws), _ptr(dw), cin, nout, _stream()), "lwg_conv2d_wgrad_winograd_f32")
    if CONV_HOOK is not None:
        CONV_HOOK(False, a.M, spec, EPI_NONE, {"kernels": 2, "kind": "wgrad_winograd"})
    return dw


class PanelCache:

    def __init__(self, params=()):
        self.out, self.rows, self.keep, self.table, self.blocks = {}, [], [], None, 0
        params = list(params)
        self.storages = {p.untyped_storage().data_ptr() for p in params}
        self.training_storages = {p.untyped_storage().data_ptr() for p in params if p.requires_grad}
        self.src_of, self.wino, self.wino_rows, self.wino_table, self.wino_blocks = {}, {}, [], None, 0
        self.frozen = []

    def cacheable(self, w):
        return w.untyped_storage().data_ptr() in self.storages

    def get(self, w, transposed, kidx, cin, cin_pad, nout, n_pad):
        key = (w.data_ptr(), tuple(w.shape), bool(transposed), kidx, cin, cin_pad, nout, n_pad)
        hit = self.out.get(key)
        if hit is not None:
            return hit, False
        if self.table is not None and torch.cuda.is_current_stream_capturing() and w.untyped_storage().data_ptr() in self.training_storages:
            raise RuntimeError("PanelCache: a panel was requested for the first time inside a hipGraph capture (the table upload is "
                               "not capturable): run one eager step before capturing")
        D0, D1, KH, KW = w.shape
        Kp = (len(kidx) * cin_pad + 31) // 32 * 32
        out = torch.empty(Kp // 4, n_pad, 4, device=w.device, dtype=torch.float32)
        self.out[key] = out
        self.src_of[out.data_ptr()] = w
        self.keep.append(w)
        if w.untyped_storage().data_ptr() in self.training_storages:
            self.rows.append((w.data_ptr(), out.data_ptr(), D1, KH * KW, 1 if transposed else 0, len(kidx), cin, cin_pad, nout, n_pad, Kp, kidx))
            self.table = None
        else:
            self.frozen.append([w, w._version, key])
        return out, True

    def _repack_stale_frozen(self):
        stale = [f for f in self.frozen if f[0]._version != f[1]]
        if not stale:
            return
        if torch.cuda.is_current_stream_capturing():
            raise RuntimeError("PanelCache: a frozen weight changed (load_state_dict / un-freeze) - its panels cannot be re-packed inside a hipGraph "
                               "capture: call refresh() eagerly once (or invalidate()) before capturing")
        for f in stale:
            w, _, key = f
            _, _, transposed, kidx, cin, cin_pad, nout, n_pad = key
            out = self.out[key]
            D0, D1, KH, KW = w.shape
            arr = (ctypes.c_int * len(kidx))(*kidx)
            _lib.check(_lib.lib().lwg_pack_panel_f32(_ptr(w), D0, D1, KH, KW, 1 if transposed else 0, arr, len(kidx), cin, cin_pad, nout, n_pad,
                                                     _ptr(out), _stream()), "lwg_pack_panel_f32")
            for (pp, tap9), U in self.wino.items():
                if pp == out.data_ptr():
                    arr9 = (ctypes.c_int * 9)(*tap9)
                    _lib.check(_lib.lib().lwg_winograd_panel_f32(_ptr(out), _ptr(U), cin_pad, out.shape[1], arr9, _stream()), "lwg_winograd_panel_f32")
            f[1] = w._version

    def invalidate(self):
        self.out, self.rows, self.keep, self.table, self.blocks, self.frozen = {}, [], [], None, 0, []
        self.src_of, self.wino, self.wino_rows, self.wino_table, self.wino_blocks = {}, {}, [], None, 0

    def refresh(self):
        self._repack_stale_frozen()
        if not self.rows:
            return
        if self.table is None:
            descs = (_lib.LwgPackDesc * len(self.rows))()
            first = 0
            for d, (wp, op, D1, KHW, tr, nt, cin, cp, nout, npad, Kp, kidx) in zip(descs, self.rows):
                d.w, d.out = wp, op
                d.D1, d.KHW, d.transposed, d.ntaps, d.cin, d.cin_pad, d.nout, d.n_pad, d.Kp, d.first_block = D1, KHW, tr, nt, cin, cp, nout, npad, Kp, first
                for i, k in enumerate(kidx):
                    d.kidx[i] = k
                first += ((Kp // 4) * npad + 255) // 256
            raw = torch.frombuffer(bytearray(bytes(descs)), dtype=torch.uint8)
            self.table = raw.to(self.keep[0].device)
            self.blocks = first
        _lib.check(_lib.lib().lwg_pack_panels_f32(self.table.data_ptr(), len(self.rows), self.blocks, _stream()), "lwg_pack_panels_f32")
        if self.wino_rows:
            if self.wino_table is None:
                descs = (_lib.LwgWinoDesc * len(self.wino_rows))()
                first = 0
                for d, (wp, up, cin, N, tap9) in zip(descs, self.wino_rows):
                    d.wpanel, d.upk, d.Cin, d.N, d.first_block = wp, up, cin, N, first
                    for i in range(9):
                        d.tap9[i] = tap9[i]
                    first += ((N + 63) // 64) * ((cin + 15) // 16)
                raw = torch.frombuffer(bytearray(bytes(descs)), dtype=torch.uint8)
                self.wino_table = raw.to(self.keep[0].device)
                self.wino_blocks = first
            _lib.check(_lib.lib().lwg_winograd_panels_f32(self.wino_table.data_ptr(), len(self.wino_rows), self.wino_blocks, _stream()),
                       "lwg_winograd_panels_f32")

    def winograd(self, spec, tap9):
        w = self.src_of.get(spec.w.data_ptr())
        if w is None:
            return None
        key = (spec.w.data_ptr(), tuple(tap9))
        U = self.wino.get(key)
        if U is None:
            trains = w.untyped_storage().data_ptr() in self.training_storages
            if self.wino_table is not None and trains and torch.cuda.is_current_stream_capturing():
                raise RuntimeError("PanelCache: a Winograd panel was requested for the first time inside a hipGraph capture: run one eager step first")
            K4, N, _ = spec.w.shape
            U = torch.empty(16, spec.Cin // 8, 2, N, 4, device=spec.w.device, dtype=torch.float32)
            arr = (ctypes.c_int * 9)(*tap9)
            _lib.check(_lib.lib().lwg_winograd_panel_f32(_ptr(spec.w), _ptr(U), spec.Cin, N, arr, _stream()), "lwg_winograd_panel_f32")
            self.wino[key] = U
            if trains:
                self.wino_rows.append((spec.w.data_ptr(), U.data_ptr(), spec.Cin, N, tuple(tap9)))
                self.wino_table = None
        return U


PANEL_CACHE = None
BRANCH_STREAM = None


def pack_panel(w, transposed, kidx, cin, cin_pad, nout, n_pad):
    w = w.detach()
    assert w.is_cuda and w.dtype == torch.float32 and w.is_contiguous()
    D0, D1, KH, KW = w.shape
    kidx = tuple(int(k) for k in kidx)
    ntaps = len(kidx)
    Kp = (ntaps * cin_pad + 31) // 32 * 32
    if PANEL_CACHE is not None and PANEL_CACHE.cacheable(w):
        out, fresh = PANEL_CACHE.get(w, transposed, kidx, cin, cin_pad, nout, n_pad)
        if not fresh:
            return out
    else:
        out = torch.empty(Kp // 4, n_pad, 4, device=w.device, dtype=torch.float32)
    arr = (ctypes.c_int * ntaps)(*[int(k) for k in kidx])
    _lib.check(_lib.lib().lwg_pack_panel_f32(_ptr(w), D0, D1, KH, KW, 1 if transposed else 0, arr, ntaps, cin, cin_pad, nout, n_pad,
                                             _ptr(out), _stream()), "lwg_pack_panel_f32")
    return out


def unpack_wgrad(dwk, dw, transposed, kidx, cin, cin_pad, nout):
    D0, D1, KH, KW = dw.shape
    ntaps = len(kidx)
    assert dwk.is_contiguous() and dw.is_contiguous() and dwk.shape[0] == ntaps * cin_pad
    arr = (ctypes.c_int * ntaps)(*[int(k) for k in kidx])
    _lib.check(_lib.lib().lwg_unpack_wgrad_f32(_ptr(dwk), D0, D1, KH, KW, 1 if transposed else 0, arr, ntaps, cin, cin_pad, nout,
                                               dwk.shape[1], _ptr(dw), _stream()), "lwg_unpack_wgrad_f32")
    return dw


def maxpool2_fwd(x):
    B, H, W, C = x.shape
    y = torch.empty(B, H // 2, W // 2, C, device=x.device, dtype=torch.float32)
    _lib.check(_lib.lib().lwg_maxpool2_fwd_nhwc_f32(_ptr(x), _ptr(y), B, H, W, C, _stream()), "lwg_maxpool2_fwd_nhwc_f32")
    return y


def maxpool2_bwd(x, dy):
    B, H, W, C = x.shape
    dx = torch.empty_like(x)
    _lib.check(_lib.lib().lwg_maxpool2_bwd_nhwc_f32(_ptr(x), _ptr(dy.contiguous()), _ptr(dx), B, H, W, C, _stream()), "lwg_maxpool2_bwd_nhwc_f32")
    return dx


def colsum(x2d_or_nhwc):
    x = x2d_or_nhwc.contiguous()
    C = x.shape[-1]
    rows = x.numel() // C
    out = torch.empty(C, device=x.device, dtype=torch.float32)
    ws = torch.empty(512 * C, device=x.device, dtype=torch.float32)
    _lib.check(_lib.lib().lwg_colsum_nhwc_f32(_ptr(x), rows, C, _ptr(out), _ptr(ws), _stream()), "lwg_colsum_nhwc_f32")
    return out


def act_bwd(dy, y, act):
    dy, y = dy.contiguous(), y.contiguous()
    out = torch.empty_like(dy)
    _lib.check(_lib.lib().lwg_act_bwd_f32(_ptr(dy), _ptr(y), dy.numel(), act, _ptr(out), _stream()), "lwg_act_bwd_f32")
    return out


def crop_resize(x, box, out_hw, want_valid=True):
    N, C, H, W = x.shape
    OH, OW = out_hw
    x = x.contiguous()
    box = box.contiguous()
    y = x.new_empty(N, C, OH, OW)
    valid = x.new_empty(N) if want_valid else None
    _lib.check(_lib.lib().lwg_crop_resize_bilinear_f32(_ptr(x), _ptr(box, torch.int64), _ptr(y), _ptr(valid), N, C, H, W, OH, OW, _stream()),
               "lwg_crop_resize_bilinear_f32")
    return y, valid


def crop_resize_bwd(dy, box, in_hw):
    N, C, OH, OW = dy.shape
    H, W = in_hw
    dx = dy.new_zeros(N, C, H, W)
    _lib.check(_lib.lib().lwg_crop_resize_bilinear_bwd_f32(_ptr(dy.contiguous()), _ptr(box.contiguous(), torch.int64), _ptr(dx), N, C, H, W, OH, OW,
                                                           _stream()), "lwg_crop_resize_bilinear_bwd_f32")
    return dx


def prelu(x, slope, res=None):
    x = x.contiguous()
    C = x.shape[-1]
    y = torch.empty_like(x)
    _lib.check(_lib.lib().lwg_prelu_f32(_ptr(x), _ptr(slope.contiguous()), None if res is None else _ptr(res.contiguous()), x.numel() // C, C, _ptr(y),
                                        _stream()), "lwg_prelu_f32")
    return y


def prelu_bwd(x, slope, dy):
    x, dy = x.contiguous(), dy.contiguous()
    C = x.shape[-1]
    dx = torch.empty_like(x)
    _lib.check(_lib.lib().lwg_prelu_bwd_f32(_ptr(x), _ptr(slope.contiguous()), _ptr(dy), x.numel() // C, C, _ptr(dx), _stream()), "lwg_prelu_bwd_f32")
    return dx


def _nsplit(hw):
    return max(1, min(64, hw // 64))


def _elem_ptr(t, off):
    return ctypes.c_void_p(t.data_ptr() + 4 * off)


def norm_fwd(x, gamma=None, beta=None, act=ACT_NONE, eps=1e-5, gb=None):
    B, H, W, C = x.shape
    x = x.contiguous()
    mean, rstd = x.new_empty(B, C), x.new_empty(B, C)
    ns = _nsplit(H * W)
    instnorm_stats(x, mean, rstd, x.new_empty(B * C * ns * 3), eps=eps, nsplit=ns)
    y = torch.empty_like(x)
    if gb is not None:
        assert gamma is None and beta is None and gb.is_contiguous() and gb.shape == (B, H, W, 2 * C)
        gp, bp, gs = _ptr(gb), _elem_ptr(gb, C), 2 * C
    else:
        gp, bp, gs = _ptr(None if gamma is None else gamma.contiguous()), _ptr(None if beta is None else beta.contiguous()), 0
    _lib.check(_lib.lib().lwg_norm_fwd_nhwc_f32(_ptr(x), _ptr(mean), _ptr(rstd), gp, bp, gs, B, H * W, C, act, _ptr(y),
                                                 _stream()), "lwg_norm_fwd_nhwc_f32")
    return y, mean, rstd


def _nsplit_bwd(hw, B, C):
    per_image = max(1, 512 // max(1, B * ((C // 4 + 63) // 64)))
    return max(1, min(per_image, hw // 32, 512))


def norm_bwd(dy, y, x, mean, rstd, gamma=None, act=ACT_NONE, gb=None):
    B, H, W, C = x.shape
    dy = dy.contiguous()
    ns = _nsplit_bwd(H * W, B, C)
    dx = torch.empty_like(x)
    ws = x.new_empty(B * (ns + 1) * C * 2)
    if gb is not None:
        dgb = torch.empty_like(gb)
        _lib.check(_lib.lib().lwg_norm_bwd_nhwc_f32(_ptr(dy), _ptr(y), _ptr(x), _ptr(mean), _ptr(rstd), _ptr(gb), 2 * C, B, H * W, C, act, ns,
                                                     _ptr(dx), _ptr(dgb), _elem_ptr(dgb, C), _ptr(ws), _stream()), "lwg_norm_bwd_nhwc_f32")
        return dx, dgb, None
    dg = torch.empty_like(x) if gamma is not None else None
    db = torch.empty_like(x) if gamma is not None else None
    _lib.check(_lib.lib().lwg_norm_bwd_nhwc_f32(_ptr(dy), _ptr(y), _ptr(x), _ptr(mean), _ptr(rstd), _ptr(gamma), 0, B, H * W, C, act, ns,
                                                 _ptr(dx), _ptr(dg), _ptr(db), _ptr(ws), _stream()), "lwg_norm_bwd_nhwc_f32")
    return dx, dg, db


def adam_step_dev(p, g, m, v, lr, beta1, beta2, eps, t_dev):
    _lib.check(_lib.lib().lwg_adam_step_dev_f32(_ptr(p), _ptr(g), _ptr(m), _ptr(v), p.numel(), lr, beta1, beta2, eps, _ptr(t_dev, torch.int32),
                                                _stream()), "lwg_adam_step_dev_f32")


def adam_step(p, g, m, v, lr, beta1, beta2, eps, t):
    _lib.check(_lib.lib().lwg_adam_step_f32(_ptr(p), _ptr(g), _ptr(m), _ptr(v), p.numel(), lr, beta1, beta2, eps, int(t), _stream()),
               "lwg_adam_step_f32")
```

Before: 1324 frames/s.

## Skip storing attention output tiles never read by downstream skip-listed SPADE convs

Builds a per-tile 'need' mask from the fine skip marks of the two SPADE convolutions, so the attention kernel skips writing background tiles that no heavy conv tile reads. It also derives a reduced light list for the shared conv from these unread marks. For the single-wave kernel variant it adds an early background detection pass that bypasses the per-source fold for tiles with no in-image taps. This cuts memory writes and conv work in background regions, at the cost of an extra small mark+scan kernel and more coupling between the attention and conv skip logic.

```diff
diff --git a/include/lwg_hip.h b/include/lwg_hip.h
--- a/include/lwg_hip.h
+++ b/include/lwg_hip.h
@@ -79,6 +79,8 @@
 int lwg_conv2d_winograd4_fine_f32(const LwgConvArgs* args, const LwgConvLists* lists, lwg_stream_t stream);
 int lwg_spade_skip_fine_lists_f32(const float* T, int B, int ns, int h, int w, int d, int* marks, int* heavy, int* light, int* counts, int* fmarks,
                                   int* fheavy, int* flight, int* fcounts, lwg_stream_t stream);
+int lwg_spade_skip_unread_lists(const int* fmarks1, const int* fmarks5, int B, int h, int w, int* need_att, int* lmarks, int* light, int* counts,
+                                lwg_stream_t stream);
 int lwg_winograd4_panel_f32(const float* wpanel, float* upk, int Cin, int N, const int* tap9, lwg_stream_t stream);
 int lwg_conv2d_nhwc_bf16_hr(const LwgConvArgs* args, lwg_stream_t stream);
 int lwg_conv2d_winograd_bf16(const LwgConvArgs* args, lwg_stream_t stream);
@@ -145,6 +147,9 @@
 int lwg_lwb_attention_x_records(int h, int w, int C, int element_size);
 int lwg_lwb_attention_x_f32(const float* x, const float* Kq, const float* kappa, const float* Vs, const float* bv, const float* T,
                             float* out, float* stats, int B, int ns, int h, int w, int C, int src_batched, lwg_stream_t stream);
+int lwg_lwb_attention_x_masked_f32(const float* x, const float* Kq, const float* kappa, const float* Vs, const float* bv, const float* T,
+                                   float* out, float* stats, int B, int ns, int h, int w, int C, int src_batched, const int* need_att,
+                                   lwg_stream_t stream);
 int lwg_lwb_attention_x_bf16(const void* x, const void* Kq, const float* kappa, const void* Vs, const float* bv, const float* T,
                              void* out, float* stats, int B, int ns, int h, int w, int C, int src_batched, lwg_stream_t stream);
 size_t lwg_instnorm_finalize_ws_floats(int B, int C, int nrec);
diff --git a/ipercore_amd/_lib.py b/ipercore_amd/_lib.py
--- a/ipercore_amd/_lib.py
+++ b/ipercore_amd/_lib.py
@@ -66,6 +66,7 @@
     "lwg_spade_skip_lists_f32": (c_i, [c_f, c_i, c_i, c_i, c_i, c_i, c_f, c_f, c_f, c_f, c_f]),
     "lwg_conv2d_winograd4_fine_f32": (c_i, [ctypes.POINTER(LwgConvArgs), ctypes.POINTER(LwgConvLists), c_f]),
     "lwg_spade_skip_fine_lists_f32": (c_i, [c_f, c_i, c_i, c_i, c_i, c_i, c_f, c_f, c_f, c_f, c_f, c_f, c_f, c_f, c_f]),
+    "lwg_spade_skip_unread_lists": (c_i, [c_f, c_f, c_i, c_i, c_i, c_f, c_f, c_f, c_f, c_f]),
     "lwg_winograd4_panel_f32": (c_i, [c_f, c_f, c_i, c_i, ctypes.POINTER(c_i), c_f]),
     "lwg_conv2d_nhwc_bf16_hr": (c_i, [ctypes.POINTER(LwgConvArgs), c_f]),
     "lwg_conv2d_winograd_bf16": (c_i, [ctypes.POINTER(LwgConvArgs), c_f]),
@@ -109,6 +110,7 @@
     "lwg_lwb_fuse_bf16": (c_i, [c_f] * 5 + [c_i] * 7 + [ctypes.c_float, ctypes.c_float, c_f]),
     "lwg_lwb_fuse_bwd_f32": (c_i, [c_f] * 7 + [c_i] * 7 + [ctypes.c_float, ctypes.c_float, c_f]),
     "lwg_lwb_attention_x_f32": (c_i, [c_f] * 8 + [c_i] * 6 + [c_f]),
+    "lwg_lwb_attention_x_masked_f32": (c_i, [c_f] * 8 + [c_i] * 6 + [c_f, c_f]),
     "lwg_lwb_attention_x_bf16": (c_i, [c_f] * 8 + [c_i] * 6 + [c_f]),
     "lwg_lwb_attention_x_records": (c_i, [c_i, c_i, c_i, c_i]),
     "lwg_instnorm_finalize_ws_floats": (ctypes.c_size_t, [c_i, c_i, c_i]),
diff --git a/ipercore_amd/csrc/lwb_attn_x.hip b/ipercore_amd/csrc/lwb_attn_x.hip
--- a/ipercore_amd/csrc/lwb_attn_x.hip
+++ b/ipercore_amd/csrc/lwb_attn_x.hip
@@ -1,5 +1,6 @@
 #include "lwg_common.h"
 #include "lwg_conv_args.h"
+#include "lwg_conv_wino.h"
 #include "lwg_lwb_taps.h"
 
 typedef unsigned int uintx4 __attribute__((ext_vector_type(4)));
@@ -49,7 +50,7 @@
                                                                  const float* __restrict__ kappa, const ST* __restrict__ Vs,
                                                                  const float* __restrict__ bv, const float* __restrict__ T,
                                                                  ST* __restrict__ out, float* __restrict__ stats, int B, int ns, int h, int w,
-                                                                 int src_batched) {
+                                                                 int src_batched, const int* __restrict__ need) {
     using TR = AttnXTraits<ST>;
     constexpr int CPL = TR::CPL;
     constexpr int C = CPL * LPP;
@@ -143,6 +144,12 @@
         }
     };
     auto taps_of = [&](const float2 t, float (&wt)[4], int& tx0, int& ty0) { lwb_taps_of(t, w, h, wt, tx0, ty0); };
+    auto has_tap = [&](const float2 t) -> bool {
+        float wt[4];
+        int tx0, ty0;
+        taps_of(t, wt, tx0, ty0);
+        return lwb_tap_in_image(tx0, ty0, w, h);
+    };
     auto fold = [&](const float (&ka)[CPL], const float (&va)[CPL], float kap, const float (&xv)[CPL], float& mrun, float& lrun, float (&o)[CPL]) {
         float dot = 0.f;
 #pragma unroll
@@ -184,14 +191,11 @@
             const int ptile = it * PPP + wq * PPW + pg;
 #pragma unroll
             for (int s = 0; s < 2; ++s) {
-                const float2 t = Tl[s * 64 + ptile];
-                float wt[4];
-                int tx0, ty0;
-                taps_of(t, wt, tx0, ty0);
-                mine |= live && lwb_tap_in_image(tx0, ty0, w, h);
+                mine |= live && has_tap(Tl[s * 64 + ptile]);
             }
         }
         if (__syncthreads_or(mine ? 1 : 0) == 0) {
+            const bool store = !need || __builtin_amdgcn_readfirstlane(need[cw4f_of_pixel(cw_grid(B, h, w, CW_NB, 32, 16, CW_NB), b, tx * 8, ty * 8)]) != 0;
 #pragma unroll 1
             for (int it = 0; it < NIT; ++it) {
                 int yc, xc;
@@ -203,7 +207,7 @@
                     float o[CPL];
 #pragma unroll
                     for (int k = 0; k < CPL; ++k) o[k] = 0.f;
-                    finish(((long)b * h + yc) * w + xc, 2.f, o);
+                    if (store) finish(((long)b * h + yc) * w + xc, 2.f, o);
                 }
             }
         } else {
@@ -271,6 +275,16 @@
             }
         }
     } else {
+    bool bg = false, store = true;
+    if (PW == 1) {
+        bool mine = false;
+        for (int i = threadIdx.x; i < ns * 64; i += 256) {
+            const int p = i & 63;
+            mine |= ty * 8 + (p >> 3) < h && tx * 8 + (p & 7) < w && has_tap(Tl[i]);
+        }
+        bg = __syncthreads_or(mine ? 1 : 0) == 0;
+        if (bg && need != nullptr) store = __builtin_amdgcn_readfirstlane(need[cw4f_of_pixel(cw_grid(B, h, w, CW_NB, 32, 16, CW_NB), b, tx * 8, ty * 8)]) != 0;
+    }
 #pragma unroll 1
     for (int it = 0; it < NIT; ++it) {
         const int pass = it * PW + pl;
@@ -285,6 +299,10 @@
         float o[CPL];
 #pragma unroll
         for (int k = 0; k < CPL; ++k) o[k] = 0.f;
+        if (bg) {
+            if (live && store) finish(gp, 1.f, o);
+            continue;
+        }
 
         auto source = [&](int s, const float2 t) {
             float wt[4];
@@ -422,7 +440,7 @@
 
 template <typename ST>
 static int lwg_attnx_launch(const ST* x, const ST* Kq, const float* kappa, const ST* Vs, const float* bv, const float* T, ST* out, float* stats,
-                            int B, int ns, int h, int w, int C, int src_batched, hipStream_t stream) {
+                            int B, int ns, int h, int w, int C, int src_batched, const int* need, hipStream_t stream) {
     if (!x || !Kq || !kappa || !Vs || !bv || !T || !out || B <= 0 || ns <= 0 || ns > 64 || h <= 0 || w <= 0) return (int)hipErrorInvalidValue;
     const unsigned long long nsrc = (unsigned long long)(src_batched ? B * ns : ns);
     if (nsrc * (unsigned long long)h * w * (unsigned long long)C * sizeof(ST) >= 0xC0000000ull) return (int)hipErrorInvalidValue;
@@ -442,7 +460,8 @@
             const hipError_t e = lwg_allow_dynamic_lds(reinterpret_cast<const void*>(kern), lds, lds_ok);                            \
             if (e != hipSuccess) return (int)e;                                                                                      \
         }                                                                                                                            \
-        hipLaunchKernelGGL(kern, grid, dim3(256 * PW), lds, stream, x, Kq, kappa, Vs, bv, T, out, stats, B, ns, h, w, src_batched);   \
+        hipLaunchKernelGGL(kern, grid, dim3(256 * PW), lds, stream, x, Kq, kappa, Vs, bv, T, out, stats, B, ns, h, w, src_batched,    \
+                           (PW) == 1 ? need : nullptr);                       \
     }
 #define LWG_ATTNX_PW(LPP, ST_, NSU)                                                                                                  \
     {                                                                                                                                \
@@ -472,14 +491,20 @@
 extern "C" int lwg_lwb_attention_x_f32(const float* x, const float* Kq, const float* kappa, const float* Vs, const float* bv, const float* T,
                                        float* out, float* stats, int B, int ns, int h, int w, int C, int src_batched, lwg_stream_t stream_) {
     if (C != 32 && C != 64 && C != 128 && C != 256) return (int)hipErrorInvalidValue;
-    return lwg_attnx_launch<float>(x, Kq, kappa, Vs, bv, T, out, stats, B, ns, h, w, C, src_batched, reinterpret_cast<hipStream_t>(stream_));
+    return lwg_attnx_launch<float>(x, Kq, kappa, Vs, bv, T, out, stats, B, ns, h, w, C, src_batched, nullptr, reinterpret_cast<hipStream_t>(stream_));
+}
+extern "C" int lwg_lwb_attention_x_masked_f32(const float* x, const float* Kq, const float* kappa, const float* Vs, const float* bv, const float* T,
+                                              float* out, float* stats, int B, int ns, int h, int w, int C, int src_batched, const int* need_att,
+                                              lwg_stream_t stream_) {
+    if (C != 32 && C != 64 && C != 128 && C != 256) return (int)hipErrorInvalidValue;
+    return lwg_attnx_launch<float>(x, Kq, kappa, Vs, bv, T, out, stats, B, ns, h, w, C, src_batched, need_att, reinterpret_cast<hipStream_t>(stream_));
 }
 
 extern "C" int lwg_lwb_attention_x_bf16(const void* x, const void* Kq, const float* kappa, const void* Vs, const float* bv, const float* T,
                                         void* out, float* stats, int B, int ns, int h, int w, int C, int src_batched, lwg_stream_t stream_) {
     if (C != 64 && C != 128 && C != 256) return (int)hipErrorInvalidValue;
     return lwg_attnx_launch<__bf16>(static_cast<const __bf16*>(x), static_cast<const __bf16*>(Kq), kappa, static_cast<const __bf16*>(Vs), bv, T,
-                                    static_cast<__bf16*>(out), stats, B, ns, h, w, C, src_batched, reinterpret_cast<hipStream_t>(stream_));
+                                    static_cast<__bf16*>(out), stats, B, ns, h, w, C, src_batched, nullptr, reinterpret_cast<hipStream_t>(stream_));
 }
 
 __global__ __launch_bounds__(1024) void lwg_in_stats_merge_seg(const float* __restrict__ ws, int C, int nrec, int nseg, float eps,
diff --git a/ipercore_amd/csrc/lwg_conv_wino.h b/ipercore_amd/csrc/lwg_conv_wino.h
--- a/ipercore_amd/csrc/lwg_conv_wino.h
+++ b/ipercore_amd/csrc/lwg_conv_wino.h
@@ -132,6 +132,30 @@
     const int p = py * 32 + px;
     py = p / CW4F_SX, px = p - py * CW4F_SX;
 }
+CW_FN void cw4f_grid_pos(const CwGrid& g, int u, int& b, int& sx, int& sy) {
+    const int t = u / CW4F_NS, s = u - t * CW4F_NS;
+    b = cw_image(g, t);
+    const int ti = t - b * g.bx * g.by;
+    sx = (ti % g.bx) * CW4F_NSX + s % CW4F_NSX, sy = (ti / g.bx) * (CW4F_NS / CW4F_NSX) + s / CW4F_NSX;
+}
+CW_FN int cw4f_grid_id(const CwGrid& g, int b, int sx, int sy) {
+    const int t = (b * g.by + sy / (CW4F_NS / CW4F_NSX)) * g.bx + sx / CW4F_NSX;
+    return t * CW4F_NS + (sy % (CW4F_NS / CW4F_NSX)) * CW4F_NSX + sx % CW4F_NSX;
+}
+CW_FN int cw4f_of_pixel(const CwGrid& g, int b, int x, int y) { return cw4f_grid_id(g, b, x / CW4F_SX, y / CW4F_SY); }
+CW_FN bool cw4f_near_heavy(const int* fmarks, const CwGrid& g, int u) {
+    int b, sx, sy;
+    cw4f_grid_pos(g, u, b, sx, sy);
+    bool any = false;
+    if (fmarks[u] == 2) return false;
+    for (int dy = -1; dy <= 1; ++dy)
+        for (int dx = -1; dx <= 1; ++dx) {
+            const int nx = sx + dx, ny = sy + dy;
+            if (nx >= 0 && nx < g.bx * CW4F_NSX && ny >= 0 && ny < g.by * (CW4F_NS / CW4F_NSX)) any |= fmarks[cw4f_grid_id(g, b, nx, ny)] == 1;
+        }
+    return any;
+}
+CW_FN int cw4f_unread_mark(int m, bool near5) { return m == 1 ? 1 : m == 0 && near5 ? 0 : 2; }
 
 #define CW_NO_OUT_BUFFER (-1ll)
 CW_FN bool cw_contract_ok(const LwgConvArgs& a, unsigned long long pair_bytes, long long out_slack) {
diff --git a/ipercore_amd/csrc/spade_skip.hip b/ipercore_amd/csrc/spade_skip.hip
--- a/ipercore_amd/csrc/spade_skip.hip
+++ b/ipercore_amd/csrc/spade_skip.hip
@@ -113,8 +113,10 @@
     }
     int hv = ph[tid] - ch, lt = pl[tid] - cl;
     sk_for_marks(j.marks, i0, i1, vec, [&](int i, int m) {
-        if (m == 1) j.heavy[hv++] = i;
-        else if (m == 0) j.light[lt++] = i;
+        if (m == 1) {
+            if (j.heavy) j.heavy[hv] = i;
+            ++hv;
+        } else if (m == 0) j.light[lt++] = i;
     });
     if (tid == 1023) {
         j.counts[0] = ph[1023];
@@ -135,6 +137,27 @@
     return (int)hipGetLastError();
 }
 
+__global__ __launch_bounds__(256) void lwg_spade_skip_unread_mark_kernel(const int* __restrict__ fm1, const int* __restrict__ fm5, int B, int h, int w, int n,
+                                                                         int* __restrict__ need_att, int* __restrict__ lmarks) {
+    const int u = blockIdx.x * 256 + threadIdx.x;
+    if (u >= n) return;
+    const CwGrid g = cw_grid(B, h, w, CW_NB, SK_EX, SK_EY, CW_NB);
+    need_att[u] = cw4f_near_heavy(fm1, g, u) ? 1 : 0;
+    lmarks[u] = cw4f_unread_mark(fm1[u], cw4f_near_heavy(fm5, g, u));
+}
+
+extern "C" int lwg_spade_skip_unread_lists(const int* fmarks1, const int* fmarks5, int B, int h, int w, int* need_att, int* lmarks, int* light, int* counts,
+                                           lwg_stream_t stream_) {
+    if (!fmarks1 || !fmarks5 || !need_att || !lmarks || !light || !counts || B <= 0 || h <= 0 || w <= 0) return (int)hipErrorInvalidValue;
+    const long long tiles = cw_total_blocks(B, h, w, CW_NB, SK_EX, SK_EY, CW_NB);
+    if (tiles * CW4F_NS >= (1ll << 30)) return (int)hipErrorInvalidValue;
+    hipStream_t stream = reinterpret_cast<hipStream_t>(stream_);
+    const int n = (int)tiles * CW4F_NS;
+    hipLaunchKernelGGL(lwg_spade_skip_unread_mark_kernel, dim3((unsigned)((n + 255) / 256)), dim3(256), 0, stream, fmarks1, fmarks5, B, h, w, n, need_att, lmarks);
+    hipLaunchKernelGGL(lwg_spade_skip_scan2_kernel, dim3(1), dim3(1024), 0, stream, SkScanJob{lmarks, n, nullptr, light, counts}, SkScanJob{});
+    return (int)hipGetLastError();
+}
+
 extern "C" int lwg_spade_skip_lists_f32(const float* T, int B, int ns, int h, int w, int d, int* marks, int* heavy, int* light, int* counts,
                                         lwg_stream_t stream_) {
     if (!T || !marks || !heavy || !light || !counts || B <= 0 || ns <= 0 || h <= 0 || w <= 0 || d < 0 || d > 64) return (int)hipErrorInvalidValue;
diff --git a/ipercore_amd/networks/generator.py b/ipercore_amd/networks/generator.py
--- a/ipercore_amd/networks/generator.py
+++ b/ipercore_amd/networks/generator.py
@@ -280,15 +280,20 @@
         if tuple(flow.shape[2:4]) != (h, w):
             raise NotImplementedError("the attention block takes flows resized to its feature size: non-square feature maps are not built "
                                       "(image_size is one number throughout the reference)")
-        att = ops.lwb_attention_x(tsf_x, kv[0], kv[2], kv[1], st["bv"], flow, torch.empty_like(tsf_x), stats=ws,
-                                  src_batched=batched)
+        att, actv, out = torch.empty_like(tsf_x), tsf_x.new_empty(B, h, w, st["shared"].N), torch.empty_like(tsf_x)
+        l1 = l5 = s1 = s5 = need = None
+        if ops.conv2d_lists_apply(att, st["shared"], actv, act=ops.ACT_RELU):
+            s1 = scratch.lists(flow, ops.SPADE_SKIP_D[0])
+            l1 = _skip_lists(s1, spade_calibration(st, tsf_x)[0])
+        if ops.conv2d_lists_apply(actv, st["gb"], out, epi=ops.EPI_SPADE, xn=tsf_x, mean=mean, rstd=rstd):
+            s5 = scratch.lists(flow, ops.SPADE_SKIP_D[1])
+            l5 = _skip_lists(s5, spade_calibration(st, tsf_x)[1])
+        if ops.SPADE_SKIP_UNREAD and s1 is not None and s5 is not None and isinstance(s1, ops.SkipLists) and isinstance(s5, ops.SkipLists) and \
+                s1.fine is not None and s5.fine is not None and ops.spade_skip_fine_apply(att) and ops.spade_skip_fine_apply(actv):
+            need, light, counts = scratch.unread(flow, s1, s5)
+            l1 = l1 + ((light, counts),)
+        att = ops.lwb_attention_x(tsf_x, kv[0], kv[2], kv[1], st["bv"], flow, att, stats=ws, src_batched=batched, **({} if need is None else {"need_att": need}))
         ops.instnorm_finalize(ws, B, C, nrec, mean, rstd, eps=1e-5)
-        actv, out = tsf_x.new_empty(B, h, w, st["shared"].N), torch.empty_like(tsf_x)
-        l1 = l5 = None
-        if ops.conv2d_lists_apply(att, st["shared"], actv, act=ops.ACT_RELU):
-            l1 = _skip_lists(scratch.lists(flow, ops.SPADE_SKIP_D[0]), spade_calibration(st, tsf_x)[0])
-        if ops.conv2d_lists_apply(actv, st["gb"], out, epi=ops.EPI_SPADE, xn=tsf_x, mean=mean, rstd=rstd):
-            l5 = _skip_lists(scratch.lists(flow, ops.SPADE_SKIP_D[1]), spade_calibration(st, tsf_x)[1])
         ops.conv2d(att, st["shared"], actv, act=ops.ACT_RELU, **({} if l1 is None else {"lists": l1}))
         return ops.conv2d(actv, st["gb"], out, epi=ops.EPI_SPADE, xn=tsf_x, mean=mean, rstd=rstd, **({} if l5 is None else {"lists": l5}))
 
@@ -505,6 +510,12 @@
             self.flows[key] = ops.spade_skip_lists(flow, d)
         return self.flows[key]
 
+    def unread(self, flow, s1, s5):
+        key = ("unread", flow.shape[2], flow.shape[3], flow.data_ptr())
+        if key not in self.flows:
+            self.flows[key] = ops.spade_skip_unread(s1, s5, flow.shape[0], flow.shape[2], flow.shape[3])
+        return self.flows[key]
+
     def get(self, n, device):
         if self.buf is None or self.buf.numel() < n or self.buf.device != device:
             self.buf = torch.empty(max(n, 1 << 16), device=device, dtype=torch.float32)
diff --git a/ipercore_amd/ops.py b/ipercore_amd/ops.py
--- a/ipercore_amd/ops.py
+++ b/ipercore_amd/ops.py
@@ -295,11 +295,14 @@
 
 SPADE_SKIP_FINE = True
 
+SPADE_SKIP_UNREAD = True
+
 _LISTS_APPLY = {}
 
 
 class SkipLists(tuple):
     fine = None
+    fmarks = None
 
 
 def spade_skip_fine_apply(x0):
@@ -320,7 +323,19 @@
                                                         _stream()), "lwg_spade_skip_fine_lists_f32")
     out = SkipLists((heavy, light, counts))
     out.fine = (fheavy, flight, fcounts)
-    return out
+    out.fmarks = fmarks
+    return out
+
+
+def spade_skip_unread(l1, l5, B, h, w):
+    n = l1.fmarks.numel()
+    assert l5.fmarks.numel() == n == 4 * B * ((h + 15) // 16) * ((w + 31) // 32)
+    buf = torch.empty(3 * n + 4, device=l1.fmarks.device, dtype=torch.int32)
+    need, lmarks, light, counts = buf[:n], buf[n:2 * n], buf[2 * n:3 * n], buf[3 * n:3 * n + 2]
+    i32 = torch.int32
+    _lib.check(_lib.lib().lwg_spade_skip_unread_lists(_ptr(l1.fmarks, i32), _ptr(l5.fmarks, i32), B, h, w, _ptr(need, i32), _ptr(lmarks, i32),
+                                                      _ptr(light, i32), _ptr(counts, i32), _stream()), "lwg_spade_skip_unread_lists")
+    return need, light, counts
 
 
 def conv2d_lists_apply(x0, spec, y, epi=EPI_NONE, act=ACT_NONE, xn=None, mean=None, rstd=None):
@@ -419,11 +434,11 @@
             kind = "winograd4"
             if lists is not None:
                 i32 = torch.int32
-                fine = len(lists) == 2 and isinstance(lists[0], SkipLists)
+                fine = len(lists) in (2, 3) and isinstance(lists[0], SkipLists)
                 if fine:
-                    sl, cal = lists
+                    sl, cal = lists[:2]
                     fine = sl.fine is not None and spade_skip_fine_apply(x0)
-                    lists = tuple(sl.fine if fine else sl) + (cal,)
+                    lists = ((sl.fine[0],) + tuple(lists[2]) if fine and len(lists) == 3 else tuple(sl.fine if fine else sl)) + (cal,)
                 ld = _lib.LwgConvLists(_ptr(lists[0], i32), _ptr(lists[1], i32), _ptr(lists[2], i32), _ptr(lists[3]))
                 if fine:
                     _lib.check(_lib.lib().lwg_conv2d_winograd4_fine_f32(a, ctypes.byref(ld), _stream()), "lwg_conv2d_winograd4_fine_f32")
@@ -630,7 +645,7 @@
     return n
 
 
-def lwb_attention_x(x, Kq, kappa, Vs, bv, T, out, stats=None, src_batched=False):
+def lwb_attention_x(x, Kq, kappa, Vs, bv, T, out, stats=None, src_batched=False, need_att=None):
     B, h, w, C = x.shape
     ns = T.shape[1]
     nsrc = B * ns if src_batched else ns
@@ -638,6 +653,12 @@
     assert tuple(Kq.shape) == (nsrc, h, w, C) and tuple(Vs.shape) == (nsrc, h, w, C) and tuple(kappa.shape) == (nsrc, h, w)
     assert Kq.dtype == x.dtype and Vs.dtype == x.dtype and out.dtype == x.dtype and kappa.dtype == torch.float32
     assert stats is None or stats.numel() >= B * attn_records(h, w, C, x.dtype) * C * 3
+    if need_att is not None:
+        assert x.dtype == torch.float32 and need_att.dtype == torch.int32 and need_att.numel() == 4 * B * ((h + 15) // 16) * ((w + 31) // 32)
+        _lib.check(_lib.lib().lwg_lwb_attention_x_masked_f32(_ptr(x), _ptr(Kq), _ptr(kappa), _ptr(Vs), _ptr(bv), _ptr(T), _ptr(out), _ptr(stats), B, ns,
+                                                              h, w, C, 1 if src_batched else 0, _ptr(need_att, torch.int32), _stream()),
+                   "lwg_lwb_attention_x_masked_f32")
+        return out
     if x.dtype == torch.bfloat16:
         bf = torch.bfloat16
         _lib.check(_lib.lib().lwg_lwb_attention_x_bf16(_ptr(x, bf), _ptr(Kq, bf), _ptr(kappa), _ptr(Vs, bf), _ptr(bv), _ptr(T), _ptr(out, bf),
```

Result: no change. 1331 frames/s (median of 6 runs) (+0.6%).
